# VatsalSy/gerris-fft-particles

Measured on AMD Instinct MI355X. Metric: Mcell-steps/s (projection+advection), 3D 256^3 uniform, higher is better.
Workload: dtype f64; 1 GPU; 3-D periodic Taylor-Green, 256^3 per GPU, default projection/advection parameters (SURVEY 8d config C); relax_mode=exact, parallelism=1 box, rccl_world_size=0

## Files before the change

### gerris-fft-particles_amd/csrc/domain.hip

```cpp
#include "gfship_internal.hpp"

namespace gfship {

static thread_local char g_error[1024] = "";

void set_error (const char * fmt, ...)
{
  va_list ap;
  va_start (ap, fmt);
  vsnprintf (g_error, sizeof (g_error), fmt, ap);
  va_end (ap);
}

int hip_fail (hipError_t e, const char * what, const char * file, int line)
{
  set_error ("HIP error %d (%s) in %s at %s:%d", (int) e, hipGetErrorString (e), what, file, line);
  return e == hipErrorOutOfMemory ? GFSHIP_ENOMEM : GFSHIP_EHIP;
}

Field * get_field (gfship_domain * dom, gfship_field f)
{
  if (!dom || f < 0 || (size_t) f >= dom->fields.size () || !dom->fields[f].used) {
    set_error ("invalid field handle %d", f);
    return nullptr;
  }
  return &dom->fields[f];
}

}

using namespace gfship;

extern "C" {

const char * gfship_last_error (void) { return g_error; }
int gfship_version (void) { return GFSHIP_VERSION; }

int gfship_device_count (void)
{
  int n = 0;
  if (hipGetDeviceCount (&n) != hipSuccess)
    return 0;
  return n;
}

int gfship_domain_create (gfship_domain ** out, int dim, int depth, const int side[6], int device)
{
  GFSHIP_CHECK (out != nullptr, GFSHIP_EINVAL, "null output pointer");
  *out = nullptr;
  GFSHIP_CHECK (dim == 2 || dim == 3, GFSHIP_EINVAL, "dim must be 2 or 3 (got %d)", dim);
  GFSHIP_CHECK (depth >= 0 && depth <= GFSHIP_MAXLEVEL, GFSHIP_EINVAL,
		"depth must be in [0,%d] (got %d)", GFSHIP_MAXLEVEL, depth);
  int ndev = gfship_device_count ();
  GFSHIP_CHECK (ndev > 0, GFSHIP_ENODEVICE,
		"no HIP device: libgfship has no CPU fallback");
  GFSHIP_CHECK (device >= 0 && device < ndev, GFSHIP_EINVAL, "device %d out of range (%d devices)",
		device, ndev);
  GFSHIP_HIP (hipSetDevice (device));
  gfship_domain * dom = new gfship_domain;
  dom->dim = dim;
  dom->depth = depth;
  dom->device = device;
  for (int d = 0; d < 6; d++) {
    dom->side[d] = side ? side[d] : GFSHIP_SIDE_BOUNDARY;
    if (d < 2*dim && (dom->side[d] < 0 || dom->side[d] > GFSHIP_SIDE_EXTERNAL)) {
      delete dom;
      set_error ("invalid side kind %d for direction %d", side[d], d);
      return GFSHIP_EINVAL;
    }
  }
  for (int d = 0; d < 2*dim; d += 2)
    if ((dom->side[d] == GFSHIP_SIDE_PERIODIC) != (dom->side[d + 1] == GFSHIP_SIDE_PERIODIC)) {
      delete dom;
      set_error ("periodic sides must come in pairs (directions %d,%d)", d, d + 1);
      return GFSHIP_EINVAL;
    }
  for (int d = 0; d < 2*dim; d++)
    if (dom->side[d] == GFSHIP_SIDE_EXTERNAL)
      dom->has_external = true;
  for (int l = 0; l <= depth; l++) {
    Layout & L = dom->lay[l];
    L.n = 1 << l;
    L.dim = dim;
    L.rows = L.n + 2;
    L.xo = 1;
    L.px = L.n + 4;
    L.sy = L.px;
    L.sz = dim == 3 ? (long) L.px*L.rows : 0;
    L.total = (size_t) L.px*L.rows*(dim == 3 ? L.rows : 1);
  }
  hipError_t e = hipStreamCreateWithFlags (&dom->stream, hipStreamNonBlocking);
  if (e == hipSuccess) e = hipEventCreate (&dom->ev0);
  if (e == hipSuccess) e = hipEventCreate (&dom->ev1);
  if (e == hipSuccess) e = hipStreamCreateWithFlags (&dom->side_stream, hipStreamNonBlocking);
  if (e == hipSuccess) e = hipEventCreateWithFlags (&dom->side_fork, hipEventDisableTiming);
  dom->scratch_doubles = 5*8192 + 64;
  if (e == hipSuccess) e = hipMalloc ((void **) &dom->d_scratch, dom->scratch_doubles*sizeof (double));
  if (e == hipSuccess) e = hipHostMalloc ((void **) &dom->h_pinned, 64*sizeof (double), hipHostMallocDefault);
  if (e == hipSuccess) memset (dom->h_pinned, 0, 64*sizeof (double));
  if (e != hipSuccess) {
    int r = hip_fail (e, "domain resources", __FILE__, __LINE__);
    gfship_domain_destroy (dom);
    return r;
  }
  dom->sw = read_switches ();
  *out = dom;
  return GFSHIP_OK;
}

void gfship_domain_destroy (gfship_domain * dom)
{
  if (!dom) return;
  (void) hipSetDevice (dom->device);
  if (dom->stream) (void) hipStreamSynchronize (dom->stream);
  if (dom->side_stream) (void) hipStreamSynchronize (dom->side_stream);
  for (size_t f = 0; f < dom->fields.size (); f++)
    if (dom->fields[f].used)
      gfship_field_free (dom, (gfship_field) f);
  comm_free (dom);
  mpi_order_free (dom);
  skew_free (dom);
  if (dom->d_scratch) (void) hipFree (dom->d_scratch);
  if (dom->cfl_partial) (void) hipFree (dom->cfl_partial);
  for (int d = 0; d < 6; d++) {
    if (dom->gfv_send[d]) (void) hipFree (dom->gfv_send[d]);
    if (dom->gfv_recv[d]) (void) hipFree (dom->gfv_recv[d]);
  }
  if (dom->lat_res) (void) hipFree (dom->lat_res);
  if (dom->lat_xch) (void) hipFree (dom->lat_xch);
  if (dom->lat_bar) (void) hipFree (dom->lat_bar);
  if (dom->h_pinned) (void) hipHostFree (dom->h_pinned);
  if (dom->ev0) (void) hipEventDestroy (dom->ev0);
  if (dom->ev1) (void) hipEventDestroy (dom->ev1);
  if (dom->side_fork) (void) hipEventDestroy (dom->side_fork);
  if (dom->side_stream) (void) hipStreamDestroy (dom->side_stream);
  if (dom->stream) (void) hipStreamDestroy (dom->stream);
  delete dom;
}

int gfship_domain_set_relax_mode (gfship_domain * dom, int mode)
{
  GFSHIP_CHECK (dom != nullptr, GFSHIP_EINVAL, "null domain");
  GFSHIP_CHECK (mode == GFSHIP_RELAX_EXACT || mode == GFSHIP_RELAX_REDBLACK ||
		mode == GFSHIP_RELAX_EXACT_HYPERPLANE || mode == GFSHIP_RELAX_EXACT_PER_SWEEP,
		GFSHIP_EINVAL, "unknown relax mode %d", mode);
  dom->force_hyperplane = (mode == GFSHIP_RELAX_EXACT_HYPERPLANE);
  dom->no_fused_loop = (mode == GFSHIP_RELAX_EXACT_PER_SWEEP);
  dom->no_fused_godunov = (mode == GFSHIP_RELAX_EXACT_PER_SWEEP);
  dom->relax_mode = mode == GFSHIP_RELAX_REDBLACK ? GFSHIP_RELAX_REDBLACK : GFSHIP_RELAX_EXACT;
  return GFSHIP_OK;
}

int gfship_domain_set_overlap (gfship_domain * dom, int overlap)
{
  GFSHIP_CHECK (dom != nullptr, GFSHIP_EINVAL, "null domain");
  dom->overlap = overlap != 0;
  return GFSHIP_OK;
}

int gfship_domain_set_exchange (gfship_domain * dom, gfship_exchange_fn fn, void * ctx)
{
  GFSHIP_CHECK (dom != nullptr, GFSHIP_EINVAL, "null domain");
  dom->exchange = fn;
  dom->exchange_ctx = ctx;
  return GFSHIP_OK;
}

int gfship_domain_set_reduce (gfship_domain * dom, gfship_reduce_fn fn, void * ctx)
{
  GFSHIP_CHECK (dom != nullptr, GFSHIP_EINVAL, "null domain");
  dom->reduce = fn;
  dom->reduce_ctx = ctx;
  return GFSHIP_OK;
}

int gfship_domain_set_gather (gfship_domain * dom, gfship_gather_fn fn, void * ctx, int rank,
			      int nboxes, const int lattice[3])
{
  GFSHIP_CHECK (dom && lattice, GFSHIP_EINVAL, "null argument");
  GFSHIP_CHECK (nboxes >= 1 && rank >= 0 && rank < nboxes &&
		(long) lattice[0]*lattice[1]*lattice[2] == nboxes, GFSHIP_EINVAL,
		"box %d of %d on a lattice of %d x %d x %d", rank, nboxes, lattice[0], lattice[1], lattice[2]);
  for (int d = 0; d < 2*dom->dim; d++)
    GFSHIP_CHECK (lattice[d/2] == 1 || dom->side[d] == GFSHIP_SIDE_EXTERNAL, GFSHIP_EINVAL,
		  "side %d faces another box of the lattice: it must be GFSHIP_SIDE_EXTERNAL", d);
  dom->gather = fn;
  dom->gather_ctx = ctx;
  dom->lat_rank = rank; dom->lat_n = nboxes;
  for (int c = 0; c < 3; c++) dom->lat_b[c] = lattice[c];
  return GFSHIP_OK;
}

int gfship_domain_path_counts (gfship_domain * dom, unsigned long long * lattice_cycles,
			       unsigned long long * fused_mpi_launches)
{
  GFSHIP_CHECK (dom != nullptr, GFSHIP_EINVAL, "null domain");
  if (lattice_cycles) *lattice_cycles = dom->n_lattice_cycles;
  if (fused_mpi_launches) *fused_mpi_launches = dom->n_fused_mpi;
  return GFSHIP_OK;
}

int gfship_domain_kernel_counts (gfship_domain * dom, unsigned long long * counts, int n)
{
  GFSHIP_CHECK (dom != nullptr && counts != nullptr && n >= 0, GFSHIP_EINVAL, "null argument");
  for (int k = 0; k < n && k < GFSHIP_KC_COUNT; k++)
    counts[k] = dom->kc[k];
  return GFSHIP_OK;
}

int gfship_domain_synchronize (gfship_domain * dom)
{
  GFSHIP_CHECK (dom != nullptr, GFSHIP_EINVAL, "null domain");
  GFSHIP_HIP (hipStreamSynchronize (dom->stream));
  return GFSHIP_OK;
}

void * gfship_domain_stream (gfship_domain * dom)
{
  return dom ? (void *) dom->stream : nullptr;
}

gfship_field gfship_field_alloc (gfship_domain * dom, int component)
{
  GFSHIP_CHECK (dom != nullptr, GFSHIP_EINVAL, "null domain");
  GFSHIP_CHECK (component >= -1 && component < dom->dim, GFSHIP_EINVAL,
		"component %d out of range", component);
  size_t slot = dom->fields.size ();
  for (size_t f = 0; f < dom->fields.size (); f++)
    if (!dom->fields[f].used) { slot = f; break; }
  if (slot == dom->fields.size ())
    dom->fields.emplace_back ();
  Field nf;
  nf.used = true;
  nf.component = component;
  size_t total = 0;
  for (int l = 0; l <= dom->depth; l++)
    total += (dom->lay[l].total + 31) & ~(size_t) 31;
  double * base = nullptr;
  GFSHIP_HIP (hipMalloc ((void **) &base, total*sizeof (double)));
  GFSHIP_HIP (hipMemsetAsync (base, 0, total*sizeof (double), dom->stream));
  size_t o = 0;
  for (int l = dom->depth; l >= 0; l--) {
    nf.lev[l] = base + o;
    nf.zero[l] = true;
    o += (dom->lay[l].total + 31) & ~(size_t) 31;
  }
  dom->fields[slot] = nf;
  return (gfship_field) slot;
}

int gfship_field_free (gfship_domain * dom, gfship_field f)
{
  Field * F = get_field (dom, f);
  if (!F) return GFSHIP_EINVAL;
  GFSHIP_HIP (hipStreamSynchronize (dom->stream));
  GFSHIP_HIP (hipFree (F->lev[dom->depth]));
  for (int d = 0; d < 6; d++)
    if (F->bcval[d]) GFSHIP_HIP (hipFree (F->bcval[d]));
  *F = Field ();
  return GFSHIP_OK;
}

int gfship_field_set_bc (gfship_domain * dom, gfship_field f, int d, int type, const double * val)
{
  Field * F = get_field (dom, f);
  if (!F) return GFSHIP_EINVAL;
  GFSHIP_CHECK (d >= 0 && d < 2*dom->dim, GFSHIP_EINVAL, "direction %d out of range", d);
  GFSHIP_CHECK (type >= GFSHIP_BC_SYMMETRY && type <= GFSHIP_BC_NEUMANN, GFSHIP_EINVAL,
		"unknown bc type %d", type);
  F->bc[d] = type;
  if (F->bcval[d]) {
    GFSHIP_HIP (hipStreamSynchronize (dom->stream));
    GFSHIP_HIP (hipFree (F->bcval[d]));
    F->bcval[d] = nullptr;
  }
  if (val) {
    int n = dom->lay[dom->depth].n;
    size_t m = dom->dim == 3 ? (size_t) n*n : (size_t) n;
    GFSHIP_HIP (hipMalloc ((void **) &F->bcval[d], m*sizeof (double)));
    GFSHIP_HIP (hipMemcpy (F->bcval[d], val, m*sizeof (double), hipMemcpyHostToDevice));
  }
  return GFSHIP_OK;
}

static int check_level (gfship_domain * dom, int level)
{
  GFSHIP_CHECK (level >= 0 && level <= dom->depth, GFSHIP_EINVAL, "level %d out of [0,%d]", level,
		dom->depth);
  return GFSHIP_OK;
}

}

namespace gfship {
int coarse_flush (gfship_domain * dom, Field * F, int level, bool leaf_write)
{
  if (!F->coarse_stale || (level >= dom->depth && !leaf_write)) return GFSHIP_OK;
  F->coarse_stale = false;
  Field * one[1] = { F };
  return launch_coarse_init (dom, one, 1);
}
}

extern "C" {

int gfship_field_upload (gfship_domain * dom, gfship_field f, int level, const double * host)
{
  Field * F = get_field (dom, f);
  if (!F) return GFSHIP_EINVAL;
  GFSHIP_CHECK (host != nullptr, GFSHIP_EINVAL, "null host pointer");
  int r = check_level (dom, level);
  if (r) return r;
  if ((r = before_write (dom))) return r;
  if ((r = coarse_flush (dom, F, level, true))) return r;
  const Layout & L = dom->lay[level];
  size_t rows = (size_t) L.rows*(dom->dim == 3 ? L.rows : 1);
  GFSHIP_HIP (hipMemcpy2DAsync (F->lev[level] + L.xo, L.px*sizeof (double),
				host, L.rows*sizeof (double),
				L.rows*sizeof (double), rows, hipMemcpyHostToDevice, dom->stream));
  GFSHIP_HIP (hipStreamSynchronize (dom->stream));
  F->zero[level] = false;
  if (level < dom->depth) F->coarse_valid = true;
  return GFSHIP_OK;
}

int gfship_field_download (gfship_domain * dom, gfship_field f, int level, double * host)
{
  Field * F = get_field (dom, f);
  if (!F) return GFSHIP_EINVAL;
  GFSHIP_CHECK (host != nullptr, GFSHIP_EINVAL, "null host pointer");
  int r = check_level (dom, level);
  if (r) return r;
  if ((r = coarse_flush (dom, F, level))) return r;
  const Layout & L = dom->lay[level];
  size_t rows = (size_t) L.rows*(dom->dim == 3 ? L.rows : 1);
  GFSHIP_HIP (hipMemcpy2DAsync (host, L.rows*sizeof (double),
				F->lev[level] + L.xo, L.px*sizeof (double),
				L.rows*sizeof (double), rows, hipMemcpyDeviceToHost, dom->stream));
  GFSHIP_HIP (hipStreamSynchronize (dom->stream));
  return GFSHIP_OK;
}

// ... 51 lines not shown
```

### gerris-fft-particles_amd/csrc/gfship_internal.hpp

```cpp
#pragma once

#include <hip/hip_runtime.h>
#include <cstdio>
#include <cstdarg>
#include <cstring>
#include <vector>
#include <deque>
#include <string>
#include <type_traits>
#include "gfship.h"
#include "switches.hpp"
#include "cell_update.hpp"

namespace gfship {

struct Layout {
  int n = 0;
  int px = 0;
  int xo = 1;
  int rows = 0;
  int dim = 3;
  long sy = 0;
  long sz = 0;
  size_t total = 0;
  __host__ __device__ inline long idx (int i, int j, int k) const {
    return xo + i + sy*j + sz*k;
  }
};

struct Field {
  bool used = false;
  int component = -1;
  double * lev[GFSHIP_MAXLEVEL + 1] = {};
  int bc[6] = {0, 0, 0, 0, 0, 0};
  double * bcval[6] = {};
  bool zero[GFSHIP_MAXLEVEL + 1] = {};
  bool coarse_stale = false;
  bool coarse_valid = false;
};

struct SkewPlan {
  int ntj = 0, RT = 0;
  size_t hb_words = 0;
  double * us = nullptr, * rs = nullptr, * ds = nullptr;
  double * ws[6] = {};
  unsigned long ws_stamp = 0;
  void * hb = nullptr;
  void * hbf = nullptr;
  bool rs_ready = false;
  int cur_set = 0;
  size_t armed[2] = { 0, 0 };
  unsigned * arm_cum = nullptr;
  hipEvent_t arm_ev = nullptr;
  bool arm_wait = false;
  bool loop_checked = false;
  void * stats_loop = nullptr;
  void * ctl = nullptr;
  unsigned long long * stats = nullptr;
  unsigned short * order = nullptr;
  unsigned short * xorder = nullptr;
};

struct RelaxOp {
  int kind = 0;
  double w = 1., h2 = 1.;
  const double * wf[6] = {};
};

inline W6 op_weights (const RelaxOp * op)
{
  W6 wf;
  for (int d = 0; d < 6; d++) wf.p[d] = op ? op->wf[d] : nullptr;
  return wf;
}

struct BcDesc {
  int side[6];
  int type[6];
  const double * val[6];
  int component;
  int homogeneous;
};

}

struct gfship_domain {
  int dim = 3, depth = 0, device = 0;
  int side[6] = {1, 1, 1, 1, 1, 1};
  int relax_mode = GFSHIP_RELAX_EXACT;
  gfship::Switches sw;
  gfship::Layout lay[GFSHIP_MAXLEVEL + 1];
  std::deque<gfship::Field> fields;
  hipStream_t stream = nullptr;
  hipEvent_t ev0 = nullptr, ev1 = nullptr;
  hipStream_t side_stream = nullptr;
  hipEvent_t side_fork = nullptr;
  int (* before_write) (void *) = nullptr;
  void * before_write_ctx = nullptr;
  double * d_scratch = nullptr;
  size_t scratch_doubles = 0;
  double * h_pinned = nullptr;
  gfship_exchange_fn exchange = nullptr; void * exchange_ctx = nullptr;
  gfship_reduce_fn reduce = nullptr;     void * reduce_ctx = nullptr;
  bool has_external = false;
  void * comm = nullptr;
  int overlap = 0;
  int lat_rank = -1, lat_n = 0, lat_b[3] = { 1, 1, 1 };
  gfship_gather_fn gather = nullptr; void * gather_ctx = nullptr;
  double * lat_res = nullptr, * lat_xch = nullptr;
  unsigned * lat_bar = nullptr;
  size_t lat_res_doubles = 0, lat_xch_doubles = 0;
  double * gfv_send[6] = {}, * gfv_recv[6] = {};
  double src[3] = { 0., 0., 0. };
  unsigned long long n_lattice_cycles = 0, n_fused_mpi = 0;
  unsigned long long kc[GFSHIP_KC_COUNT] = {};
  bool lattice_attr_set = false;
  void * mpi_plan[GFSHIP_MAXLEVEL + 1] = {};
  gfship_field dp_cache = -1;
  int skew_resident = -1;
  int patch_resident = 0;
  bool no_fused_godunov = false;
  bool no_fused_loop = false;
  bool force_hyperplane = false;
  bool unit_weights = false;
  bool weighted = false;
  unsigned long weights_stamp = 0;
  gfship_field wf[6] = {-1, -1, -1, -1, -1, -1};
  gfship::SkewPlan skew[GFSHIP_MAXLEVEL + 1];
  double diff_w[GFSHIP_MAXLEVEL + 1] = {};
  double * cfl_partial = nullptr;
  size_t cfl_nblocks = 0, cfl_used = 0;
  bool cfl_dirty = false;
  bool coarse_attr_set = false;
  gfship_field res_cache = -1;
  bool diff_ready = false;
  int diff_kind = 1;
  int patch_call = -1;
};

namespace gfship {

void set_error (const char * fmt, ...);
int  hip_fail (hipError_t e, const char * what, const char * file, int line);

inline int before_write (gfship_domain * dom)
{
  return dom->before_write ? dom->before_write (dom->before_write_ctx) : GFSHIP_OK;
}

#define GFSHIP_HIP(call) do { hipError_t e_ = (call); \
    if (e_ != hipSuccess) return gfship::hip_fail (e_, #call, __FILE__, __LINE__); } while (0)

inline hipError_t stream_wait_spin (hipStream_t st)
{
  hipError_t e;
  while ((e = hipStreamQuery (st)) == hipErrorNotReady)
    ;
  return e;
}

template <class F> inline void with_bools (F && f) { f (); }
template <class F, class... B> inline void with_bools (F && f, bool b0, B... rest)
{
  if (b0) with_bools ([&] (auto... r) { f (std::true_type {}, r...); }, rest...);
  else    with_bools ([&] (auto... r) { f (std::false_type {}, r...); }, rest...);
}

template <class F, class... B> inline void with_kind (F && f, int kind, B... bools)
{
  auto k = [&] (auto K) { with_bools ([&] (auto... r) { f (K, r...); }, bools...); };
  if (kind == 3)      k (std::integral_constant<int, 3> {});
  else if (kind == 2) k (std::integral_constant<int, 2> {});
  else if (kind)      k (std::integral_constant<int, 1> {});
  else                k (std::integral_constant<int, 0> {});
}

#define GFSHIP_CHECK(cond, code, ...) do { if (!(cond)) { \
    gfship::set_error (__VA_ARGS__); return (code); } } while (0)

Field * get_field (gfship_domain * dom, gfship_field f);
int coarse_flush (gfship_domain * dom, Field * F, int level, bool leaf_write = false);
inline long ncells (const Layout & L) {
  return L.dim == 3 ? (long) L.n*L.n*L.n : (long) L.n*L.n;
}

int launch_bc (gfship_domain * dom, Field * v, Field * v1, int level, int homogeneous);
bool all_sides_periodic (const gfship_domain * dom);

__device__ __forceinline__ void periodic_images (const Layout & L, double * __restrict__ a, int i, int j, int k,
						  double v)
{
  const int n = L.n;
  if (i == 1) a[L.idx (n + 1, j, k)] = v;
  if (i == n) a[L.idx (0, j, k)] = v;
  if (j == 1) a[L.idx (i, n + 1, k)] = v;
  if (j == n) a[L.idx (i, 0, k)] = v;
  if (k == 1) a[L.idx (i, j, n + 1)] = v;
  if (k == n) a[L.idx (i, j, 0)] = v;
}
int call_exchange (gfship_domain * dom, double * ptr, int level, int kind);
int bc_mpi_begin (gfship_domain * dom, Field * v1, int level);
int bc_mpi_end (gfship_domain * dom, Field * v, Field * v1, int level, int homogeneous);
int call_reduce (gfship_domain * dom, double * vals, int n, int op);
int call_reduce_norm (gfship_domain * dom, double * sums, int nsum, double * mx);
int comm_exchange (gfship_domain * dom, double * a, int level, int kind);
int comm_exchange_raw (gfship_domain * dom, double * const send[6], double * const recv[6], size_t count);
int comm_migrate (gfship_domain * dom, int rs, const int nsend[6], const double * const send[6],
		  int nrecv[6], std::vector<double> recv[6]);
int comm_allgather (gfship_domain * dom, const double * send, double * recv, size_t count);
int multi_buffers (gfship_domain * dom);
int launch_bc_multi (gfship_domain * dom, Field * const * v, int nf, int level, int homogeneous);
int call_gather (gfship_domain * dom, const double * send, double * recv, size_t count);
int comm_exchange_begin (gfship_domain * dom, double * a, int level);
int comm_exchange_end (gfship_domain * dom, double * a, int level);
int comm_reduce (gfship_domain * dom, double * sums, int nsum, double * maxs, int nmax,
		 double * mins, int nmin);
void comm_free (gfship_domain * dom);
int launch_relax_exact (gfship_domain * dom, unsigned dimension, int level, double omega,
			double * u, const double * rhs, const double * dia,
			const RelaxOp * op = nullptr);
int launch_relax_mpi_first (gfship_domain * dom, unsigned dimension, int level, double omega,
			    double * u, const double * rhs, const double * dia, const RelaxOp * op,
			    int (* after_shell) (void *), void * ctx);
void mpi_order_free (gfship_domain * dom);
int launch_relax_loop_small (gfship_domain * dom, unsigned dimension, int level, double omega,
			     Field * dp, Field * ubc, const double * rhs, const double * dia,
			     unsigned nrelax, bool * done, const RelaxOp * op = nullptr);
int coarse_cycle_top (gfship_domain * dom, int minlevel);
int lattice_cycle_top (gfship_domain * dom, int minlevel, Field * dia);
int lattice_check_error (gfship_domain * dom);
int launch_lattice_cycle (gfship_domain * dom, unsigned dimension, double omega, int lmin, int ltop,
			  const unsigned * nrelax, Field * dp, Field * ubc, Field * res);
int launch_coarse_cycle (gfship_domain * dom, unsigned dimension, double omega, int lmin, int ltop,
			 const unsigned * nrelax, Field * dp, Field * ubc, Field * res, Field * dia);
int launch_relax_redblack (gfship_domain * dom, unsigned dimension, int level, double omega,
			   double * u, const double * rhs, const double * dia);
int launch_residual (gfship_domain * dom, int level, const double * u, const double * rhs,
		     const double * dia, double * res);
int launch_residual_weighted (gfship_domain * dom, int level, const double * u, const double * rhs,
			      const double * dia, double * res);
int launch_poisson_weights (gfship_domain * dom, double * const alpha[3]);
int launch_diffusion_weights (gfship_domain * dom, double * const D[3], double cdt);
int alloc_weights (gfship_domain * dom);
RelaxOp weighted_op (gfship_domain * dom, int level);
int launch_restrict (gfship_domain * dom, unsigned dimension, int level_coarse, double * v_coarse,
		     const double * v_fine);
int launch_prolongate (gfship_domain * dom, int level_coarse, const double * v_coarse,
		       double * v_fine);
int launch_correct (gfship_domain * dom, int level, double * u, const double * dp);
int launch_fill (gfship_domain * dom, int level, double * a, double value);
int launch_residual_norm (gfship_domain * dom, int level, const double * u, const double * rhs,
			  const double * dia, double * res, double scale, double weight,
			  double * out , bool dia_zero = false);
int launch_norm_async (gfship_domain * dom, int level, const double * a, double scale, double weight);
int launch_norm (gfship_domain * dom, int level, const double * a, double scale, double weight,
		 double out[5] );

int launch_face_interp_un (gfship_domain * dom, double * const u[3], double * const un[3]);
int launch_divergence (gfship_domain * dom, double * const un[3], double * div, double dt);
int launch_correct_un (gfship_domain * dom, const double * p, double * const un[3], double dt);
int launch_centered_gradient (gfship_domain * dom, const double * p, double * const g[3]);
int launch_correct_centered (gfship_domain * dom, double * const u[3], double * const g[3], double dt);
int launch_correct_centered_coarse (gfship_domain * dom, double * const u[3], double * const g[3],
				    double dt, double * const uc[3]);
int launch_coarse_init_from (gfship_domain * dom, Field * const * v, int nf, int top);
int launch_coarse_init_levels (gfship_domain * dom, Field * const * v, int nf, int top, int bottom);
int launch_advected_face_values (gfship_domain * dom, const double * v, double * const u[3],
				 double * const un[3], double dt, int use_centered, int gradient,
				 double * const fv[6], int cmask, double visc = 0., double gsrc = 0.,
				 const double * msrc = nullptr );
int launch_variable_mac_source (gfship_domain * dom, const double * v, double * const D[3],
				const double * alpha, double * out);
int launch_mac_source_fields (gfship_domain * dom, int c, const double * F, bool add_out, double * out);
int launch_centered_source_fields (gfship_domain * dom, double * v, const double * F, double gsrc, double dt);
int launch_face_bc (gfship_domain * dom, Field * v, double * const fv[6], int cmask);
int launch_predict_un (gfship_domain * dom, int cc, const double * uc, double * const fv[6],
		       double * unc);
int launch_flux_update (gfship_domain * dom, bool velocity, double * v, double * const un[3],
			double * const fv[6], const double * gm, const double * gc, double dt,
			double gsrc = 0.);
int launch_cfl (gfship_domain * dom, double * const u[3], double * const un[3],
		const double visc[3], double * cfl2,
		double * const msrc[3] = nullptr );
int launch_coarse_init (gfship_domain * dom, Field * const * v, int nf);
int launch_velocity_divergence (gfship_domain * dom, double * const u[3], double * out);
bool godunov_fused_supported (const gfship_domain * dom);
bool godunov_fused_mpi_supported (const gfship_domain * dom);
int launch_project_correct (gfship_domain * dom, const double * p, double * const un[3],
			    double * const g[3], double * const u[3], double dt, bool want_max,
			    bool * ghosts_done = nullptr);
int launch_cfl_from_max (gfship_domain * dom, double * cfl2);
int launch_face_interp_div (gfship_domain * dom, double * const u[3], double * const un[3] ,
			    double * div, double dt);
int launch_project_correct_weighted (gfship_domain * dom, const double * p, double * const un[3],
				     double * const g[3], double * const u[3], double dt);
int launch_project_correct_lazy (gfship_domain * dom, const double * p, double * const u[3],
				 double * const g[3], double * const uo[3], double dt,
				 bool * ghosts_done = nullptr);
int launch_predict_un_fused (gfship_domain * dom, double * const u[3], double dt, int gradient,
			     const double visc[3], double * const un[3], double * div = nullptr,
			     double div_dt = 0., bool * div_done = nullptr);
int launch_advect3_fused (gfship_domain * dom, double * const v[3], double * const out[3],
			  double * const un[3], double * const gm[3], double * const gc[3],
			  double dt, int gradient, double corr_dt = 0., double * const uc[3] = nullptr);
int launch_advect_fused (gfship_domain * dom, bool velocity, const double * v, double * out,
			 double * const un[3], const double * gm, const double * gc, double dt,
			 int gradient, double visc, double gsrc = 0.);
int launch_advect_diffuse_fused (gfship_domain * dom, const double * v, double * out, double * const un[3],
				 double dt, int gradient, double D, double w, double beta);

bool skew_supported (const gfship_domain * dom, int level);
int  launch_relax_loop_skew (gfship_domain * dom, int level, Field * dp, Field * ubc,
			     const double * rhs, const double * dia, bool dia_zero,
			     unsigned nrelax, bool bc, double * correct_into = nullptr,
			     const double * prolong_from = nullptr, const RelaxOp * op = nullptr);
void skew_free (gfship_domain * dom);
bool skew_loop_supported (gfship_domain * dom, int level, unsigned nrelax, bool bc);
struct LoopGhosts;
int  skew_loop_run (gfship_domain * dom, int level, SkewPlan * S, double * u_nat, bool has_dia,
		    unsigned nrelax, float * ms = nullptr, const Field * ubc = nullptr,
		    const RelaxOp * op = nullptr, LoopGhosts * ghosts = nullptr);
int  skew_time_loop (gfship_domain * dom, int level, Field * u, const double * rhs,
		     const double * dia, bool dia_zero, unsigned nrelax, int reps,
		     double * ms_per_loop, int * fused, double * ms_inclusive = nullptr);
int  skew_check_error (gfship_domain * dom);
int  skew_arm_ahead (gfship_domain * dom, int level, unsigned nrelax);
int  patch_resident_per_cu (const gfship_domain * dom);
bool prolongation_fused (gfship_domain * dom, unsigned dimension, int level, unsigned nrelax);
bool prolongation_fusable (gfship_domain * dom, unsigned dimension, int level, unsigned nrelax);
bool line_prolongation_fused (gfship_domain * dom, unsigned dimension, int level, unsigned nrelax);
bool line_prolongation_fusable (gfship_domain * dom, unsigned dimension, int level, unsigned nrelax);
inline bool patch_level (const gfship_domain * dom, int level)
{
  const bool per_cell_weights = dom->patch_call < 0 ? dom->weighted : dom->patch_call == 0;
  return dom->sw.patch () && !per_cell_weights && dom->lay[level].n >= dom->sw.patch_min_n;
}
int  patch_pack (gfship_domain * dom, int level, SkewPlan * S, const double * u, const double * rhs,
		 const double * dia, const double * coarse = nullptr);
int  patch_unpack (gfship_domain * dom, int level, SkewPlan * S, double * u, double * add_into,
		   const LoopGhosts * ghosts = nullptr);
int  patch_restrict_pack (gfship_domain * dom, int level, SkewPlan * S, const double * res,
			  double * res_coarse, SkewPlan * Sc, unsigned dimension);
int  launch_restrict_pack (gfship_domain * dom, unsigned dimension, int level, Field * res,
			   bool coarse_fused);
void skew_dump_stats (gfship_domain * dom, int level);
int  skew_time_sweeps (gfship_domain * dom, int level, Field * u, const double * rhs,
		       const double * dia, bool dia_zero, int reps, double * ms_per_sweep);

}
```

### gerris-fft-particles_amd/csrc/poisson.hip

```cpp
#include "gfship_internal.hpp"
#include <cmath>
#include <cfloat>
#include <cstdlib>

using namespace gfship;

#define GFSHIP_CHECK_DIMENSION(dom, d) \
  GFSHIP_CHECK ((d) == (unsigned) (dom)->dim, GFSHIP_EUNSUPPORTED, \
		"dimension %u on a %d-D domain: only the dimension of the domain is implemented", (d), (dom)->dim)

namespace gfship {

static bool weighted_pipelinable (gfship_domain * dom, unsigned dimension, int level)
{
  return dom->relax_mode == GFSHIP_RELAX_EXACT && dimension == 3 && dom->dim == 3 &&
    skew_supported (dom, level) && !dom->force_hyperplane;
}

static bool weighted_pipelined (gfship_domain * dom, unsigned dimension, int level)
{
  return dom->sw.weighted_pipelined && weighted_pipelinable (dom, dimension, level);
}

static int relax_level (gfship_domain * dom, unsigned dimension, int level, double omega,
// ... 137 lines not shown
  int r;
  double w = (double) ncells (L);
  if (dom->has_external) {
    double sums[5] = { s[0], s[1], s[2], w, s[4] }, mx[1] = { s[3] };
    if ((r = call_reduce_norm (dom, sums, 5, mx))) return r;
    s[0] = sums[0]; s[1] = sums[1]; s[2] = sums[2]; w = sums[3]; s[3] = mx[0]; s[4] = sums[4];
  }
  gfship_norm n;
  n.bias = s[0]; n.first = s[1]; n.second = s[2]; n.infty = s[3]; n.w = w;
  if (n.w > 0.) {
    n.bias /= n.w;
    n.first /= n.w;
    n.second = sqrt (n.second/n.w);
  }
  else
    n.infty = 0.;
  dt *= dt;
  n.bias = s[4]*dt;
  n.first *= dt;
  n.second *= dt;
  n.infty *= dt;
  *out = n;
  return GFSHIP_OK;
}

}

extern "C" {

void gfship_multilevel_params_init (gfship_multilevel_params * par, int dim)
{
  memset (par, 0, sizeof (*par));
  par->tolerance = 1e-3;
  par->nrelax    = 4;
  par->erelax    = 1;
  par->minlevel  = 0;
  par->nitermax  = 100;
  par->nitermin  = 1;
  par->dimension = dim;
  par->weighted  = 0;
  par->beta      = 1.;
  par->omega     = 1.;
  par->function  = 0;
}

int gfship_poisson_coefficients_alpha (gfship_domain * dom, const gfship_field alpha[3])
{
  GFSHIP_CHECK (dom != nullptr, GFSHIP_EINVAL, "null domain");
  if (!alpha)
    return gfship_poisson_coefficients (dom);
  double * a[3] = { nullptr, nullptr, nullptr };
  for (int c = 0; c < dom->dim; c++) {
    Field * F = get_field (dom, alpha[c]);
    if (!F) return GFSHIP_EINVAL;
    a[c] = F->lev[dom->depth];
  }
  int r = alloc_weights (dom);
  if (r) return r;
  if ((r = launch_poisson_weights (dom, a))) return r;
  dom->weighted = true;
  dom->weights_stamp++;
  dom->unit_weights = true;
  return GFSHIP_OK;
}

int gfship_poisson_weights (gfship_domain * dom, int d, gfship_field * w)
{
  GFSHIP_CHECK (dom && w, GFSHIP_EINVAL, "null argument");
  GFSHIP_CHECK (d >= 0 && d < 2*dom->dim, GFSHIP_EINVAL, "direction %d out of range", d);
  GFSHIP_CHECK (dom->wf[d] >= 0 && (dom->weighted || (dom->diff_ready && dom->diff_kind == 3)), GFSHIP_EINVAL,
		"call gfship_poisson_coefficients_alpha or gfship_diffusion_coefficients_faces first");
  *w = dom->wf[d];
  return GFSHIP_OK;
}

int gfship_poisson_coefficients (gfship_domain * dom)
{
  GFSHIP_CHECK (dom != nullptr, GFSHIP_EINVAL, "null domain");
  dom->weighted = false;
  dom->unit_weights = true;
  return GFSHIP_OK;
}

int gfship_relax (gfship_domain * dom, unsigned d, int level, double omega,
		  gfship_field u, gfship_field rhs, gfship_field dia)
{
  Field * U = get_field (dom, u), * R = get_field (dom, rhs), * D = get_field (dom, dia);
  if (!U || !R || !D) return GFSHIP_EINVAL;
  GFSHIP_CHECK (level >= 0 && level <= dom->depth, GFSHIP_EINVAL, "level %d out of range", level);
  GFSHIP_CHECK (d == 2 || d == 3, GFSHIP_EINVAL, "dimension must be 2 or 3");
  GFSHIP_CHECK_DIMENSION (dom, d);
  GFSHIP_CHECK (dom->unit_weights, GFSHIP_EINVAL, "call gfship_poisson_coefficients first");
  { int r = before_write (dom); if (r) return r; }
  for (Field * F : { U, R, D })
    if (int r = coarse_flush (dom, F, level)) return r;
  return relax_level (dom, d, level, omega, U, R, D);
}

int gfship_residual (gfship_domain * dom, unsigned d, int level,
		     gfship_field u, gfship_field rhs, gfship_field dia, gfship_field res)
{
  Field * U = get_field (dom, u), * R = get_field (dom, rhs), * D = get_field (dom, dia),
    * S = get_field (dom, res);
  if (!U || !R || !D || !S) return GFSHIP_EINVAL;
  GFSHIP_CHECK (level >= 0 && level <= dom->depth, GFSHIP_EINVAL, "level %d out of range", level);
  GFSHIP_CHECK (d == 2 || d == 3, GFSHIP_EINVAL, "dimension must be 2 or 3");
  GFSHIP_CHECK_DIMENSION (dom, d);
  GFSHIP_CHECK (dom->unit_weights, GFSHIP_EINVAL, "call gfship_poisson_coefficients first");
  { int r = before_write (dom); if (r) return r; }
  for (Field * F : { U, R, D, S })
    if (int r = coarse_flush (dom, F, level)) return r;
  S->zero[level] = false;
  if (dom->weighted)
    return launch_residual_weighted (dom, level, U->lev[level], R->lev[level], D->lev[level],
				     S->lev[level]);
  return launch_residual (dom, level, U->lev[level], R->lev[level], D->lev[level], S->lev[level]);
}

int gfship_norm_residual (gfship_domain * dom, double dt, gfship_field res, gfship_norm * out)
{
  Field * S = get_field (dom, res);
  if (!S || !out) return GFSHIP_EINVAL;
  return norm_residual (dom, dt, S, out);
}

int gfship_norm_variable (gfship_domain * dom, gfship_field v, gfship_norm * out)
{
  Field * V = get_field (dom, v);
  if (!V || !out) return GFSHIP_EINVAL;
  const Layout & L = dom->lay[dom->depth];
  double size = 1./L.n;
  double vol = dom->dim == 3 ? size*size*size : size*size;
  double s[5];
  int r = launch_norm (dom, dom->depth, V->lev[dom->depth], 1., vol, s);
  if (r) return r;
  gfship_norm n;
  double wv = vol*(double) ncells (L);
  if (dom->has_external) {
    double sums[4] = { s[0], s[1], s[2], wv }, mx[1] = { s[3] };
    if ((r = call_reduce_norm (dom, sums, 4, mx))) return r;
    s[0] = sums[0]; s[1] = sums[1]; s[2] = sums[2]; wv = sums[3]; s[3] = mx[0];
  }
  n.bias = s[0]; n.first = s[1]; n.second = s[2]; n.infty = s[3];
  n.w = wv;
  if (n.w > 0.) {
    n.bias /= n.w;
    n.first /= n.w;
    n.second = sqrt (n.second/n.w);
  }
  else
    n.infty = 0.;
  *out = n;
  return GFSHIP_OK;
}

}

static int poisson_cycle (gfship_domain * dom, gfship_multilevel_params * p,
			  gfship_field u, gfship_field rhs, gfship_field dia, gfship_field res,
			  double dt, gfship_norm * norm)
{
  GFSHIP_CHECK (dom && p, GFSHIP_EINVAL, "null argument");
  GFSHIP_CHECK (p->dimension == 2 || p->dimension == 3, GFSHIP_EINVAL, "dimension must be 2 or 3");
  GFSHIP_CHECK_DIMENSION (dom, p->dimension);
  GFSHIP_CHECK (p->nrelax > 0 && p->erelax > 0, GFSHIP_EINVAL, "nrelax and erelax must be non zero");
  GFSHIP_CHECK (dom->unit_weights, GFSHIP_EINVAL, "call gfship_poisson_coefficients first");
  if (dom->dp_cache < 0)
    dom->dp_cache = gfship_field_alloc (dom, -1);
  gfship_field dpf = dom->dp_cache;
  if (dpf < 0) return dpf;
  Field * U = get_field (dom, u), * R = get_field (dom, rhs), * D = get_field (dom, dia),
    * S = get_field (dom, res), * DP = get_field (dom, dpf);
  int r = GFSHIP_OK;
  bool corrected = false;
  if (!U || !R || !D || !S) return GFSHIP_EINVAL;
  const int L = dom->depth;
  unsigned minlevel = p->minlevel;
  if (minlevel > (unsigned) L) minlevel = L;
  p->depth = L;

#define TRY(x) do { if ((r = (x)) != GFSHIP_OK) goto done; } while (0)
  for (int l = 0; l <= L; l++)
    S->zero[l] = U->zero[l] = false;
  {
    unsigned nrl[GFSHIP_MAXLEVEL + 1];
    {
      unsigned nr = p->nrelax;
      for (int l = L; l >= 0; l--) {
	nrl[l] = nr;
	if (l > (int) minlevel) nr *= p->erelax;
      }
    }
    for (int l = 0; l <= L; l++)
      DP->zero[l] = false;
    const int ctop = dom->weighted ? -1 : coarse_cycle_top (dom, (int) minlevel);
    const int ltop = ctop >= 0 ? -1 : lattice_cycle_top (dom, (int) minlevel, D);
    for (int l = L - 1; l >= (ctop >= 0 ? ctop + 1 : ltop >= 0 ? ltop : 0); l--) {
      if (dom->relax_mode == GFSHIP_RELAX_EXACT && p->dimension == 3 && !dom->weighted &&
	  !dom->force_hyperplane && skew_supported (dom, l + 1))
	TRY (skew_arm_ahead (dom, l + 1, nrl[l + 1]));
      const bool rp = !dom->skew[l + 1].rs_ready && prolongation_fused (dom, p->dimension, l + 1, nrl[l + 1]);
      if (rp) dom->kc[dom->sw.fused_restriction ? GFSHIP_KC_RESTRICTION_FUSED : GFSHIP_KC_RESTRICTION_DECLINED]++;
      if (dom->sw.fused_restriction && rp)
	TRY (launch_restrict_pack (dom, p->dimension, l + 1, S,
				   l > (int) minlevel && prolongation_fused (dom, p->dimension, l, nrl[l])));
      else
	TRY (launch_restrict (dom, p->dimension, l, S->lev[l], S->lev[l + 1]));
    }
    unsigned first = minlevel;
    if (ltop >= 0) {
      TRY (launch_lattice_cycle (dom, p->dimension, p->omega, (int) minlevel, ltop, nrl, DP, U, S));
      first = ltop + 1;
    }
    else if (ctop >= 0) {
      TRY (launch_coarse_cycle (dom, p->dimension, p->omega, (int) minlevel, ctop, nrl, DP, U, S, D));
      first = ctop + 1;
    }
    else {
      TRY (launch_fill (dom, minlevel, DP->lev[minlevel], 0.));
      TRY (relax_loop (dom, DP, U, p->dimension, minlevel, p->omega, S, D, nrl[minlevel]));
      first = minlevel + 1;
      dom->kc[GFSHIP_KC_COARSE_END_BY_LEVEL]++;
    }
    for (unsigned l = first; l <= p->depth; l++) {
      const bool fp = prolongation_fused (dom, p->dimension, (int) l, nrl[l]) ||
	line_prolongation_fused (dom, p->dimension, (int) l, nrl[l]);
      if (fp) dom->kc[GFSHIP_KC_PROLONGATION_FUSED]++;
      else if (prolongation_fusable (dom, p->dimension, (int) l, nrl[l]) ||
	       line_prolongation_fusable (dom, p->dimension, (int) l, nrl[l]))
	dom->kc[GFSHIP_KC_PROLONGATION_DECLINED]++;
      if (!fp)
	TRY (launch_prolongate (dom, l - 1, DP->lev[l - 1], DP->lev[l]));
      TRY (relax_loop (dom, DP, U, p->dimension, l, p->omega, S, D, nrl[l],
		       (int) l == L ? U->lev[L] : nullptr, &corrected, fp ? DP->lev[l - 1] : nullptr));
    }
  }
  if (!corrected)
    TRY (launch_correct (dom, L, U->lev[L], DP->lev[L]));
  if (!(corrected && all_sides_periodic (dom)))
    TRY (launch_bc (dom, U, U, L, 0));
  if (norm)
    TRY (residual_and_norm (dom, dt, U, R, D, S, norm));
  else if (dom->weighted)
    TRY (launch_residual_weighted (dom, L, U->lev[L], R->lev[L], D->lev[L], S->lev[L]));
  else
    TRY (launch_residual (dom, L, U->lev[L], R->lev[L], D->lev[L], S->lev[L]));
#undef TRY
 done:
  for (int l = 0; l <= L; l++)
    dom->skew[l].rs_ready = false;
  return r;
}

extern "C" {

int gfship_poisson_cycle (gfship_domain * dom, gfship_multilevel_params * p,
			  gfship_field u, gfship_field rhs, gfship_field dia, gfship_field res)
{
  GFSHIP_CHECK (dom != nullptr, GFSHIP_EINVAL, "null domain");
  int r = before_write (dom);
  if (r) return r;
  return poisson_cycle (dom, p, u, rhs, dia, res, 1., nullptr);
}

int gfship_poisson_solve (gfship_domain * dom, gfship_multilevel_params * par,
			  gfship_field lhs, gfship_field rhs, gfship_field res,
			  gfship_field dia, double dt)
{
  GFSHIP_CHECK (dom && par, GFSHIP_EINVAL, "null argument");
  Field * U = get_field (dom, lhs), * R = get_field (dom, rhs), * D = get_field (dom, dia),
    * S = get_field (dom, res);
  if (!U || !R || !D || !S) return GFSHIP_EINVAL;
  GFSHIP_CHECK (par->dimension == 2 || par->dimension == 3, GFSHIP_EINVAL, "dimension must be 2 or 3");
  GFSHIP_CHECK_DIMENSION (dom, par->dimension);
  GFSHIP_CHECK (dom->unit_weights, GFSHIP_EINVAL, "call gfship_poisson_coefficients first");
  { int r = before_write (dom); if (r) return r; }
  int r;
  const int L = dom->depth;
  if ((r = coarse_flush (dom, U, L, true))) return r;
  unsigned minlevel = par->minlevel;
  par->depth = L;
  par->niter = 0;

  bool deferred = par->nitermin >= 1 && par->nitermax >= 1;
  if (deferred) {
    const Layout & Ly = dom->lay[L];
    double size = 1./Ly.n;
    S->zero[L] = false;
    if (dom->weighted) {
      if ((r = launch_residual_weighted (dom, L, U->lev[L], R->lev[L], D->lev[L], S->lev[L]))) return r;
      if ((r = launch_norm_async (dom, L, S->lev[L], 1.*size*size, 1.))) return r;
    }
    else if ((r = launch_residual_norm (dom, L, U->lev[L], R->lev[L], D->lev[L], S->lev[L], 1.*size*size,
					1., nullptr, D->zero[L])))
      return r;
  }
  else {
    if ((r = residual_and_norm (dom, dt, U, R, D, S, &par->residual))) return r;
    par->residual_before = par->residual;
  }

  double res_max_before = par->residual.infty;

  while (par->niter < par->nitermin ||
	 (par->residual.infty > par->tolerance && par->niter < par->nitermax)) {
    if ((r = poisson_cycle (dom, par, lhs, rhs, dia, res, dt, &par->residual))) {
      if (deferred) {
	deferred = false;
	double s0[5];
	if (hipStreamSynchronize (dom->stream) == hipSuccess) {
	  memcpy (s0, dom->h_pinned + 8, sizeof (s0));
	  if (norm_residual_finish (dom, dt, s0, &par->residual_before) == GFSHIP_OK)
	    par->residual = par->residual_before;
	}
	else
	  memset (&par->residual_before, 0, sizeof (par->residual_before)),
	    memset (&par->residual, 0, sizeof (par->residual));
      }
      break;
    }
    if (deferred) {
      deferred = false;
      double s0[5];
      memcpy (s0, dom->h_pinned + 8, sizeof (s0));
      if ((r = norm_residual_finish (dom, dt, s0, &par->residual_before))) break;
      res_max_before = par->residual_before.infty;
    }
    if (par->residual.infty == res_max_before)
      break;
    if (par->residual.infty > res_max_before/1.1 && par->minlevel < par->depth)
      par->minlevel++;
    res_max_before = par->residual.infty;
    par->niter++;
  }

  par->minlevel = minlevel;
  if (r == GFSHIP_OK)
    r = skew_check_error (dom);
  if (r == GFSHIP_OK)
    r = lattice_check_error (dom);
  return r;
}

int gfship_time_relax (gfship_domain * dom, unsigned d, int level, gfship_field u,
		       gfship_field rhs, gfship_field dia, int reps, double * ms_per_sweep)
{
  Field * U = get_field (dom, u), * R = get_field (dom, rhs), * D = get_field (dom, dia);
  if (!U || !R || !D || !ms_per_sweep || reps <= 0) return GFSHIP_EINVAL;
  GFSHIP_CHECK (level >= 0 && level <= dom->depth, GFSHIP_EINVAL, "level %d out of range", level);
  int r;
  if (dom->relax_mode == GFSHIP_RELAX_EXACT && d == 3 && skew_supported (dom, level) &&
      !dom->force_hyperplane) {
    U->zero[level] = false;
    r = skew_time_sweeps (dom, level, U, R->lev[level], D->lev[level], D->zero[level], reps,
			  ms_per_sweep);
    if (r == GFSHIP_OK && dom->sw.skew_stats)
      skew_dump_stats (dom, level);
    return r;
  }
  if ((r = relax_level (dom, d, level, 1., U, R, D))) return r;
  GFSHIP_HIP (hipEventRecord (dom->ev0, dom->stream));
  for (int q = 0; q < reps; q++)
    if ((r = relax_level (dom, d, level, 1., U, R, D))) return r;
  GFSHIP_HIP (hipEventRecord (dom->ev1, dom->stream));
  GFSHIP_HIP (hipEventSynchronize (dom->ev1));
  float ms = 0.f;
  GFSHIP_HIP (hipEventElapsedTime (&ms, dom->ev0, dom->ev1));
  *ms_per_sweep = (double) ms/reps;
  if (dom->sw.skew_stats)
    skew_dump_stats (dom, level);
  return GFSHIP_OK;
}

int gfship_time_relax_loop (gfship_domain * dom, int level, gfship_field u, gfship_field rhs,
			    gfship_field dia, unsigned nrelax, int reps, double * ms_per_loop,
			    int * fused)
{
  return gfship_time_relax_loop_inclusive (dom, level, u, rhs, dia, nrelax, reps, ms_per_loop, fused,
					   nullptr);
}

int gfship_time_relax_loop_inclusive (gfship_domain * dom, int level, gfship_field u, gfship_field rhs,
				      gfship_field dia, unsigned nrelax, int reps,
				      double * ms_per_loop, int * fused, double * ms_inclusive)
{
  Field * U = get_field (dom, u), * R = get_field (dom, rhs), * D = get_field (dom, dia);
  if (!U || !R || !D || !ms_per_loop || !fused || reps <= 0 || nrelax == 0) return GFSHIP_EINVAL;
  GFSHIP_CHECK (level >= 0 && level <= dom->depth, GFSHIP_EINVAL, "level %d out of range", level);
  GFSHIP_CHECK (dom->relax_mode == GFSHIP_RELAX_EXACT && skew_supported (dom, level) &&
		!dom->force_hyperplane, GFSHIP_EUNSUPPORTED,
		"the pipelined sweep does not run on this level / in this mode");
  U->zero[level] = false;
  int r = skew_time_loop (dom, level, U, R->lev[level], D->lev[level], D->zero[level], nrelax,
			  reps, ms_per_loop, fused, ms_inclusive);
  if (r == GFSHIP_OK)
    r = skew_check_error (dom);
  return r;
}

}
```

### gerris-fft-particles_amd/csrc/relax_patch_loop.hip

```cpp
#include "relax_skew.hpp"
#include <cstdlib>
#include <vector>

#ifndef PK_D
#define PK_D 9
#endif
#ifndef PK_DH
#define PK_DH 3
#endif
#ifndef PK_KO
#define PK_KO 0
#endif
#define PK_NTHREADS 192
#define PK_SKEW 14

namespace gfship {

typedef double d2 __attribute__((ext_vector_type(2)));

__device__ __forceinline__ void patch_arm_other_set (const SkewLoopArgs & A, int tile, int tid, int nt)
{
  if (A.arm_pairs == 0) return;
  typedef unsigned long long ull2 __attribute__((ext_vector_type(2)));
  const unsigned long long W = A.arm_cum[A.ntj*A.ntj];
// ... 843 lines not shown
  __shared__ double cbuf[10][10][PR_W];
  const int Ilo = R0 - PK_SKEW > 0 ? R0 - PK_SKEW : 0;
  const int cx0 = Ilo >> 1;
  {
    const int jb = n/2 - 8*P - 8, kb = n/2 - 8*Q - 8;
    const int xmax = A.Lc.n + 1;
    for (int e = threadIdx.x; e < 100*PR_W; e += 64*PR_WAVES) {
      const int line = e / PR_W, ix = e % PR_W;
      const int jl = line % 10, kl = line / 10;
      int cx = cx0 + ix;
      if (cx > xmax) cx = xmax;
      cbuf[kl][jl][ix] = vc[A.Lc.idx (cx, jb + jl, kb + kl)];
    }
  }
  __syncthreads ();
  const double * const cl = &cbuf[8 - PB][8 - PA][0] - cx0;
  constexpr int lsy = PR_W, lsz = 10*PR_W;
#endif
  if (r0 >= n + PK_SKEW) return;
  const int j0 = n - (SK_T*P + 2*PA), k0 = n - (SK_T*Q + 2*PB);
  const bool side_j[2] = { j0 == n, j0 - 1 == 1 }, side_k[2] = { k0 == n, k0 - 1 == 1 };
  int cur_m = -1;
  double pv = 0., qx = 0., qy = 0., qz = 0.;
  const int r1 = r0 + PR_ROWS;
  for (int rho = r0; rho < r1; rho++) {
    const int I = rho - s;
    if ((unsigned) I >= (unsigned) n) continue;
    const int m = I >> 1;
    if (m != cur_m) {
      cur_m = m;
#if PR_LDS
      const double * const q = cl + (m + 1);
      pv = q[0];
      {
	const double g1 = q[1] - 1.*pv, g2 = q[-1] - 1.*pv;
	qx = 0.25*((g1 - g2)/2.);
      }
      {
	const double g1 = q[lsy] - 1.*pv, g2 = q[-lsy] - 1.*pv;
	qy = 0.25*((g1 - g2)/2.);
      }
      {
	const double g1 = q[lsz] - 1.*pv, g2 = q[-lsz] - 1.*pv;
	qz = 0.25*((g1 - g2)/2.);
      }
#else
      const long p = cline + (m + 1);
      pv = vc[p];
      {
	const double g1 = vc[p + 1] - 1.*pv, g2 = vc[p - 1] - 1.*pv;
	qx = 0.25*((g1 - g2)/2.);
      }
      {
	const double g1 = vc[p + csy] - 1.*pv, g2 = vc[p - csy] - 1.*pv;
	qy = 0.25*((g1 - g2)/2.);
      }
      {
	const double g1 = vc[p + csz] - 1.*pv, g2 = vc[p - csz] - 1.*pv;
	qz = 0.25*((g1 - g2)/2.);
      }
#endif
    }
    const double bx = pv + ((I & 1) ? qx : - qx);
    d2 o01, o23;
    {
      const double by0 = bx + qy, by1 = bx + (- qy);
      o01.x = by0 + qz;     o01.y = by1 + qz;
      o23.x = by0 + (- qz); o23.y = by1 + (- qz);
    }
    double * const row = dst + (long) rho*SK_NL;
    *(d2 *) row = o01;
    *(d2 *) (row + 128) = o23;
    if (__builtin_expect (I == 0 || I == n - 1 || side_j[0] || side_j[1] || side_k[0] || side_k[1], 0)) {
      const bool ends = I == 0 || I == n - 1;
      const double vv[4] = { o01.x, o01.y, o23.x, o23.y };
#pragma unroll
      for (int q = 0; q < 4; q++)
	if (ends || side_j[q & 1] || side_k[q >> 1]) {
	  A.nat[A.L.idx (I + 1, j0 - (q & 1), k0 - (q >> 1))] = vv[q];
	  if (A.periodic) periodic_images (A.L, A.nat, I + 1, j0 - (q & 1), k0 - (q >> 1), vv[q]);
	}
    }
  }
}

#ifndef PP_ROWS
#define PP_ROWS 16
#endif
#define PP_SPAN (PP_ROWS + 7)
#ifndef PPR_ROWS
#define PPR_ROWS 64
#endif
#define PPR_SPAN (PPR_ROWS + 7)
#ifndef PPU_ROWS
#define PPU_ROWS 64
#endif
#define PPU_SPAN (PPU_ROWS + 7)

__global__ void __launch_bounds__(256)
patch_pack_kernel (PatchPackArgs A)
{
  __shared__ double buf[3][32][PP_SPAN + 1];
  const int tid = threadIdx.x;
  const int tile = blockIdx.z, PB = blockIdx.y, r0 = blockIdx.x*PP_ROWS;
  const int P = tile % A.ntj, Q = tile / A.ntj;
  const int n = A.L.n;
  const long tbase = (long) tile*(A.RT + 2*SK_FP)*SK_NL + SK_FP*SK_NL;
  const int I0 = r0 - 7 - PB;
  for (int e = tid; e < 32*PP_SPAN; e += 256) {
    const int line = e / PP_SPAN, di = e % PP_SPAN;
    const int a = line & 15, db = line >> 4;
    const int I = I0 + di;
    if (I >= 0 && I < n) {
      const int j = n - (SK_T*P + a), k = n - (SK_T*Q + 2*PB + db);
      const long nidx = A.L.idx (I + 1, j, k);
      int q0 = 0;
      if (A.coarse) {
	const double v = patch_prolong (A.Lc, A.coarse, I + 1, j, k);
	buf[0][line][di] = v;
	if (I == 0 || I == n - 1 || j == 1 || j == n || k == 1 || k == n)
	  A.nat[nidx] = v;
	q0 = 1;
      }
      for (int q = q0; q < A.narr; q++)
	buf[q][line][di] = A.src[q][nidx];
    }
  }
  __syncthreads ();
  for (int e = tid; e < PP_ROWS*32; e += 256) {
    const int row = e / 32, col = e % 32;
    const int PA = col >> 2, p = col & 3;
    const int a = 2*PA + (p & 1), db = p >> 1;
    const int rho = r0 + row;
    const int I = rho - PA - PB;
    if (I >= 0 && I < n) {
      const long sidx = tbase + (long) rho*SK_NL + 128*(p >> 1) + 2*(PA + 8*PB) + (p & 1);
      for (int q = 0; q < A.narr; q++)
	A.dst[q][sidx] = buf[q][a + 16*db][I - I0];
    }
  }
}

struct PatchRestrictArgs {
  Layout L, Lc;
  int ntj, RT;
  const double * src;
  double * dst;
  double * cnat;
  double * cskew;
  int cntj, cRT;
  unsigned dimension;
};

__global__ void __launch_bounds__(256)
patch_restrict_pack_kernel (PatchRestrictArgs A)
{
  __shared__ double buf[32][PPR_SPAN + 2];
  const int tid = threadIdx.x;
  const int tile = blockIdx.z, PB = blockIdx.y, r0 = blockIdx.x*PPR_ROWS;
  const int P = tile % A.ntj, Q = tile / A.ntj;
  const int n = A.L.n;
  const long tbase = (long) tile*(A.RT + 2*SK_FP)*SK_NL + SK_FP*SK_NL;
  const int I0 = r0 - 7 - PB;
  for (int e = tid; e < 32*(PPR_SPAN + 1); e += 256) {
    const int line = e / (PPR_SPAN + 1), di = e % (PPR_SPAN + 1);
    const int a = line & 15, db = line >> 4;
    const int I = I0 + di;
    if (I >= 0 && I < n) {
      const int j = n - (SK_T*P + a), k = n - (SK_T*Q + 2*PB + db);
      buf[line][di] = A.src[A.L.idx (I + 1, j, k)];
    }
  }
  __syncthreads ();
  for (int e = tid; e < PPR_ROWS*32; e += 256) {
    const int row = e / 32, col = e % 32;
    const int PA = col >> 2, p = col & 3;
    const int a = 2*PA + (p & 1), db = p >> 1;
    const int rho = r0 + row;
    const int I = rho - PA - PB;
    if (I >= 0 && I < n)
      A.dst[tbase + (long) rho*SK_NL + 128*(p >> 1) + 2*(PA + 8*PB) + (p & 1)] = buf[a + 16*db][I - I0];
  }
  for (int e = tid; e < 8*(PPR_ROWS/2); e += 256) {
    const int PA = e / (PPR_ROWS/2), mi = e % (PPR_ROWS/2);
    const int par = (PA + PB + r0) & 1;
    const int row = 2*mi + par;
    const int I = r0 + row - PA - PB;
    if (I >= 0 && I < n) {
      const int di = I - I0;
      double val = 0.;
#pragma unroll
      for (int id = 0; id < 8; id++)
	val += buf[2*PA + ((id >> 1) & 1) + 16*(id >> 2)][di + (id & 1)];
      const double v = A.dimension == 2 ? val : val/2.;
      const int m = I >> 1;
      const int pj = (n - SK_T*P - 2*PA) >> 1, pk = (n - SK_T*Q - 2*PB) >> 1;
      A.cnat[A.Lc.idx (m + 1, pj, pk)] = v;
      if (A.cskew) {
	const int ca = 8*(P & 1) + PA, cb = 8*(Q & 1) + PB;
	const long ctile = (P >> 1) + (long) A.cntj*(Q >> 1);
	A.cskew[ctile*(A.cRT + 2*SK_FP)*SK_NL + SK_FP*SK_NL +
		(long) (m + (ca >> 1) + (cb >> 1))*SK_NL + 128*(cb & 1) + 2*((ca >> 1) + 8*(cb >> 1)) + (ca & 1)] = v;
      }
    }
  }
}

__global__ void __launch_bounds__(256)
patch_unpack_kernel (PatchPackArgs A, LoopGhosts G)
{
  if ((int) blockIdx.z >= A.ntj*A.ntj) {
    loop_ghost_blocks (G, A.ntj*A.ntj);
    return;
  }
  __shared__ double buf[32][PPU_SPAN + 1];
  const int tid = threadIdx.x;
  const int tile = blockIdx.z, PB = blockIdx.y, r0 = blockIdx.x*PPU_ROWS;
  const int P = tile % A.ntj, Q = tile / A.ntj;
  const int n = A.L.n;
  const long tbase = (long) tile*(A.RT + 2*SK_FP)*SK_NL + SK_FP*SK_NL;
  const int I0 = r0 - 7 - PB;
  for (int e = tid; e < PPU_ROWS*32; e += 256) {
    const int row = e / 32, col = e % 32;
    const int PA = col >> 2, p = col & 3;
    const int a = 2*PA + (p & 1), db = p >> 1;
    const int rho = r0 + row;
    const int I = rho - PA - PB;
    if (I >= 0 && I < n)
      buf[a + 16*db][I - I0] = A.src[0][tbase + (long) rho*SK_NL + 128*(p >> 1) + 2*(PA + 8*PB) + (p & 1)];
  }
  __syncthreads ();
  for (int e = tid; e < 32*PPU_SPAN; e += 256) {
    const int line = e / PPU_SPAN, di = e % PPU_SPAN;
    const int a = line & 15, db = line >> 4;
    const int I = I0 + di;
    const int rho = I + (a >> 1) + PB;
    if (I >= 0 && I < n && rho >= r0 && rho < r0 + PPU_ROWS) {
      const int j = n - (SK_T*P + a), k = n - (SK_T*Q + 2*PB + db);
      const long c = A.L.idx (I + 1, j, k);
      if (A.add) {
	const double v = A.add[c] + buf[line][di];
	A.add[c] = v;
	if (A.periodic && (I == 0 || I == n - 1 || j == 1 || j == n || k == 1 || k == n))
	  periodic_images (A.L, A.add, I + 1, j, k, v);
      }
      else
	A.dst[0][c] = buf[line][di];
    }
  }
}

int patch_resident_per_cu (const gfship_domain * dom)
{
  int per_cu = 0;
  hipError_t e = dom->sw.patch_regs ?
    hipOccupancyMaxActiveBlocksPerMultiprocessor (&per_cu, relax_patch_loop_kernel<true>, PK_NTHREADS, 0) :
    hipOccupancyMaxActiveBlocksPerMultiprocessor (&per_cu, relax_ring_loop_kernel<true, 0>, RK_NTHREADS, 0);
  int per_cu1 = 0;
  if (e == hipSuccess)
    e = hipOccupancyMaxActiveBlocksPerMultiprocessor (&per_cu1, relax_ring_loop_kernel<true, 1>, RK_NTHREADS, 0);
  if (per_cu1 < per_cu) per_cu = per_cu1;
  return e == hipSuccess ? per_cu : 0;
}

int patch_pack (gfship_domain * dom, int level, SkewPlan * S, const double * u, const double * rhs,
		const double * dia, const double * coarse)
{
  PatchPackArgs A;
  A.add = nullptr;
  A.coarse = coarse;
  A.periodic = all_sides_periodic (dom);
  A.nat = const_cast<double *> (u);
  A.Lc = dom->lay[level > 0 ? level - 1 : 0];
  A.L = dom->lay[level]; A.ntj = S->ntj; A.RT = S->RT;
  A.narr = 0;
  A.src[A.narr] = u;   A.dst[A.narr++] = S->us;
  if (rhs) { A.src[A.narr] = rhs; A.dst[A.narr++] = S->rs; }
  if (dia) { A.src[A.narr] = dia; A.dst[A.narr++] = S->ds; }
  const int rows = A.L.n + PK_SKEW + 1;
  const bool old_pack = coarse && dom->sw.old_prolong_pack;
  if (coarse) dom->kc[old_pack ? GFSHIP_KC_PROLONG_PACK_OLD : GFSHIP_KC_PROLONG_PACK_NEW]++;
  if (coarse && !old_pack) {
    PatchPackArgs Pr = A;
    Pr.narr = 1;
    dim3 pgrid ((rows + PR_ROWS*PR_WAVES - 1)/(PR_ROWS*PR_WAVES), S->ntj*S->ntj);
    hipLaunchKernelGGL (patch_prolong_kernel, pgrid, dim3 (64*PR_WAVES), 0, dom->stream, Pr);
    GFSHIP_HIP (hipGetLastError ());
    if (A.narr == 1)
      return GFSHIP_OK;
    for (int q = 1; q < A.narr; q++) { A.src[q - 1] = A.src[q]; A.dst[q - 1] = A.dst[q]; }
    A.narr--;
    A.coarse = nullptr;
  }
  dim3 grid ((rows + PP_ROWS - 1)/PP_ROWS, 8, S->ntj*S->ntj);
  hipLaunchKernelGGL (patch_pack_kernel, grid, dim3 (256), 0, dom->stream, A);
  GFSHIP_HIP (hipGetLastError ());
  return GFSHIP_OK;
}

int patch_restrict_pack (gfship_domain * dom, int level, SkewPlan * S, const double * res,
			 double * res_coarse, SkewPlan * Sc, unsigned dimension)
{
  PatchRestrictArgs A;
  A.L = dom->lay[level]; A.Lc = dom->lay[level - 1];
  A.ntj = S->ntj; A.RT = S->RT;
  A.src = res; A.dst = S->rs;
  A.cnat = res_coarse;
  A.cskew = Sc ? Sc->rs : nullptr;
  A.cntj = Sc ? Sc->ntj : 0; A.cRT = Sc ? Sc->RT : 0;
  A.dimension = dimension;
  const int rows = A.L.n + PK_SKEW + 1;
  dim3 grid ((rows + PPR_ROWS - 1)/PPR_ROWS, 8, S->ntj*S->ntj);
  hipLaunchKernelGGL (patch_restrict_pack_kernel, grid, dim3 (256), 0, dom->stream, A);
  GFSHIP_HIP (hipGetLastError ());
  return GFSHIP_OK;
}

int patch_unpack (gfship_domain * dom, int level, SkewPlan * S, double * u, double * add_into,
		  const LoopGhosts * ghosts)
{
  PatchPackArgs A;
  A.coarse = nullptr; A.nat = nullptr; A.Lc = dom->lay[level];
  A.periodic = all_sides_periodic (dom);
  A.L = dom->lay[level]; A.ntj = S->ntj; A.RT = S->RT;
  A.narr = 1;
  A.src[0] = S->us; A.dst[0] = u; A.add = add_into;
  const int rows = A.L.n + PK_SKEW + 1;
  dim3 grid ((rows + PPU_ROWS - 1)/PPU_ROWS, 8, S->ntj*S->ntj);
  const LoopGhosts G = ghosts ? *ghosts : LoopGhosts ();
  grid.z += loop_ghost_planes (G, grid.x, grid.y);
  hipLaunchKernelGGL (patch_unpack_kernel, grid, dim3 (256), 0, dom->stream, A, G);
  GFSHIP_HIP (hipGetLastError ());
  return GFSHIP_OK;
}

int patch_loop_launch (gfship_domain * dom, const SkewLoopArgs & A, int ntiles, bool has_dia,
		       unsigned nrelax, float * ms, LoopGhosts * ghosts)
{
  if (ms) GFSHIP_HIP (hipEventRecord (dom->ev0, dom->stream));
  if (A.op == 1)
    hipLaunchKernelGGL ((relax_ring_loop_kernel<true, 1>), dim3 (ntiles), dim3 (RK_NTHREADS), 0, dom->stream, A);
  else if (dom->sw.patch_regs) {
    if (has_dia)
      hipLaunchKernelGGL (relax_patch_loop_kernel<true>, dim3 (ntiles), dim3 (PK_NTHREADS), 0, dom->stream, A);
    else
      hipLaunchKernelGGL (relax_patch_loop_kernel<false>, dim3 (ntiles), dim3 (PK_NTHREADS), 0, dom->stream, A);
  }
  else if (has_dia)
    hipLaunchKernelGGL ((relax_ring_loop_kernel<true, 0>), dim3 (ntiles), dim3 (RK_NTHREADS), 0, dom->stream, A);
  else
    hipLaunchKernelGGL ((relax_ring_loop_kernel<false, 0>), dim3 (ntiles), dim3 (RK_NTHREADS), 0, dom->stream, A);
  GFSHIP_HIP (hipGetLastError ());
  if (ms) {
    GFSHIP_HIP (hipEventRecord (dom->ev1, dom->stream));
    GFSHIP_HIP (hipEventSynchronize (dom->ev1));
    GFSHIP_HIP (hipEventElapsedTime (ms, dom->ev0, dom->ev1));
  }
  if (nrelax >= 2 && ghosts)
    *ghosts = loop_ghosts_of (A, true);
  else if (nrelax >= 2) {
    const Layout & L = A.L;
    int block = L.n >= 256 ? 256 : L.n >= 128 ? 128 : 64;
    hipLaunchKernelGGL (patch_loop_ghosts_kernel, dim3 ((L.n + block - 1)/block, L.n, 4), dim3 (block),
			0, dom->stream, A);
    GFSHIP_HIP (hipGetLastError ());
  }
  return GFSHIP_OK;
}

}
```

### gerris-fft-particles_amd/csrc/relax_skew.hip

```cpp
#include "relax_skew.hpp"
#include <cstdlib>

namespace gfship {

template <bool HAS_DIA>
__global__ void __launch_bounds__(SK_NL)
relax_skew_kernel (SkewArgs A)
{
  constexpr int XS = SK_T + 1;
  __shared__ double X[2][XS*XS];
  __shared__ double Y[2][XS*XS];
  __shared__ unsigned s_tile;

  const int tid = threadIdx.x;
  const int a = tid & (SK_T - 1), b = tid >> 4;
  const int n = A.L.n;
  const int ntj = A.ntj;
  const long tstride = (long) (A.RT + 2*SK_FP)*SK_NL;
  const long hstride = (long) SK_HROWS (n)*SK_T;

  if (tid == 0)
    s_tile = A.order[atomicAdd (A.ticket, 1u)];
  __syncthreads ();
  const int tile = s_tile;
// ... 200 lines not shown
    const int di = m - lo;
    if (m <= 2*SK_T - 2 && di >= 0 && di < SK_T) {
      long sidx = tbase + (long) (I0 + m + b)*SK_NL + lo + SK_T*b;
      for (int q = 0; q < A.narr; q++)
	A.dst[q][sidx] = tile_[q][lo][di];
    }
  }
}

__global__ void __launch_bounds__(SK_NL)
skew_prolong_pack_kernel (PackArgs A)
{
  __shared__ double tile_[3][SK_T][SK_T + 1];
  const int tid = threadIdx.x;
  const int lo = tid & (SK_T - 1), hi = tid >> 4;
  const int tile = blockIdx.z;
  const int b = blockIdx.y;
  const int I0 = blockIdx.x*SK_T;
  const int P = tile % A.ntj, Q = tile / A.ntj;
  const int n = A.L.n;
  const int k = n - (SK_T*Q + b);
  const long tbase = (long) tile*(A.RT + 2*SK_FP)*SK_NL + SK_FP*SK_NL;
  {
    const int i = I0 + lo + 1, j = n - (SK_T*P + hi);
    const long nidx = A.L.idx (i, j, k);
    const double v = patch_prolong (A.Lc, A.coarse, i, j, k);
    tile_[0][hi][lo] = v;
    if (i == 1 || i == n || j == 1 || j == n || k == 1 || k == n) {
      A.nat[nidx] = v;
      periodic_images (A.L, A.nat, i, j, k, v);
    }
    for (int q = 1; q < A.narr; q++)
      tile_[q][hi][lo] = A.src[q][nidx];
  }
  __syncthreads ();
#pragma unroll
  for (int pass = 0; pass < 2; pass++) {
    const int m = hi + SK_T*pass;
    const int di = m - lo;
    if (m <= 2*SK_T - 2 && di >= 0 && di < SK_T) {
      long sidx = tbase + (long) (I0 + m + b)*SK_NL + lo + SK_T*b;
      for (int q = 0; q < A.narr; q++)
	A.dst[q][sidx] = tile_[q][lo][di];
    }
  }
}

__global__ void __launch_bounds__(SK_NL)
skew_unpack_kernel (PackArgs A, LoopGhosts G)
{
  if ((int) blockIdx.z >= A.ntj*A.ntj) {
    loop_ghost_blocks (G, A.ntj*A.ntj);
    return;
  }
  __shared__ double tile_[SK_T][SK_T + 1];
  const int tid = threadIdx.x;
  const int lo = tid & (SK_T - 1), hi = tid >> 4;
  const int tile = blockIdx.z;
  const int b = blockIdx.y;
  const int I0 = blockIdx.x*SK_T;
  const int P = tile % A.ntj, Q = tile / A.ntj;
  const int n = A.L.n;
  const int k = n - (SK_T*Q + b);
  const long tbase = (long) tile*(A.RT + 2*SK_FP)*SK_NL + SK_FP*SK_NL;
#pragma unroll
  for (int pass = 0; pass < 2; pass++) {
    const int m = hi + SK_T*pass;
    const int di = m - lo;
    if (m <= 2*SK_T - 2 && di >= 0 && di < SK_T)
      tile_[lo][di] = A.src[0][tbase + (long) (I0 + m + b)*SK_NL + lo + SK_T*b];
  }
  __syncthreads ();
  const int j = n - (SK_T*P + hi);
  const long c = A.L.idx (I0 + lo + 1, j, k);
  if (A.add) {
    const double v = A.add[c] + tile_[hi][lo];
    A.add[c] = v;
    if (A.periodic) periodic_images (A.L, A.add, I0 + lo + 1, j, k, v);
  }
  else
    A.dst[0][c] = tile_[hi][lo];
}

bool skew_supported (const gfship_domain * dom, int level)
{
  if (dom->dim != 3) return false;
  int n = dom->lay[level].n;
  if (n < 2*SK_T) return false;
  return true;
}

static unsigned * skew_err_word (gfship_domain * dom, int level)
{
  return (unsigned *) (dom->h_pinned + 32) + level;
}

static int skew_plan (gfship_domain * dom, int level, SkewPlan ** out)
{
  SkewPlan & S = dom->skew[level];
  if (!S.us) {
    const Layout & L = dom->lay[level];
    S.ntj = L.n/SK_T;
    S.RT = L.n + SK_PAD;
    int ntiles = S.ntj*S.ntj;
    size_t doubles = (size_t) ntiles*(S.RT + 2*SK_FP)*SK_NL + 64;
    S.hb_words = (size_t) ntiles*SK_HROWS (L.n)*SK_T;
    GFSHIP_HIP (hipMalloc ((void **) &S.us, doubles*sizeof (double)));
    GFSHIP_HIP (hipMalloc ((void **) &S.rs, doubles*sizeof (double)));
    GFSHIP_HIP (hipMalloc ((void **) &S.ds, doubles*sizeof (double)));
    GFSHIP_HIP (hipMalloc ((void **) &S.hb, 2*S.hb_words*sizeof (u64)));
    GFSHIP_HIP (hipMalloc ((void **) &S.ctl, 64));
    if (dom->sw.skew_stats)
      GFSHIP_HIP (hipMalloc ((void **) &S.stats, (size_t) ntiles*4*sizeof (u64)));
    std::vector<unsigned short> order;
    for (int d = 0; d <= 2*(S.ntj - 1); d++)
      for (int Q = 0; Q < S.ntj; Q++) {
	int P = d - Q;
	if (P >= 0 && P < S.ntj)
	  order.push_back ((unsigned short) (P + S.ntj*Q));
      }
    GFSHIP_HIP (hipMalloc ((void **) &S.order, order.size ()*sizeof (unsigned short)));
    GFSHIP_HIP (hipMemcpy (S.order, order.data (), order.size ()*sizeof (unsigned short),
			   hipMemcpyHostToDevice));
    if (ntiles >= 8 && S.ntj % 4 == 0) {
      int bw = S.ntj/2, bh = S.ntj/4;
      std::vector<unsigned short> xo;
      for (int x = 0; x < 8; x++)
	for (unsigned short t : order) {
	  int P = t % S.ntj, Q = t / S.ntj;
	  if ((P/bw) + 2*(Q/bh) == x) xo.push_back (t);
	}
      GFSHIP_HIP (hipMalloc ((void **) &S.xorder, xo.size ()*sizeof (unsigned short)));
      GFSHIP_HIP (hipMemcpy (S.xorder, xo.data (), xo.size ()*sizeof (unsigned short),
			     hipMemcpyHostToDevice));
    }
    GFSHIP_HIP (hipMemsetAsync (S.ctl, 0, 64, dom->stream));
  }
  *out = &S;
  return GFSHIP_OK;
}

void skew_free (gfship_domain * dom)
{
  for (int l = 0; l <= GFSHIP_MAXLEVEL; l++) {
    SkewPlan & S = dom->skew[l];
    if (S.us) (void) hipFree (S.us);
    if (S.rs) (void) hipFree (S.rs);
    if (S.ds) (void) hipFree (S.ds);
    for (int d = 0; d < 6; d++) if (S.ws[d]) (void) hipFree (S.ws[d]);
    if (S.hb) (void) hipFree (S.hb);
    if (S.hbf) (void) hipFree (S.hbf);
    if (S.arm_cum) (void) hipFree (S.arm_cum);
    if (S.arm_ev) (void) hipEventDestroy (S.arm_ev);
    if (S.stats_loop) (void) hipFree (S.stats_loop);
    if (S.ctl) (void) hipFree (S.ctl);
    if (S.stats) (void) hipFree (S.stats);
    if (S.order) (void) hipFree (S.order);
    if (S.xorder) (void) hipFree (S.xorder);
    S = SkewPlan ();
  }
}

static int skew_pack (gfship_domain * dom, int level, SkewPlan * S, const double * u,
		      const double * rhs, const double * dia, const double * coarse = nullptr)
{
  if (patch_level (dom, level))
    return patch_pack (dom, level, S, u, rhs, dia, coarse);
  PackArgs A;
  A.add = nullptr; A.periodic = false;
  A.coarse = coarse; A.nat = const_cast<double *> (u);
  A.Lc = dom->lay[level > 0 ? level - 1 : 0];
  A.L = dom->lay[level]; A.ntj = S->ntj; A.RT = S->RT;
  A.narr = 0;
  A.src[A.narr] = u;   A.dst[A.narr++] = S->us;
  A.src[A.narr] = rhs; A.dst[A.narr++] = S->rs;
  if (dia) { A.src[A.narr] = dia; A.dst[A.narr++] = S->ds; }
  dim3 grid (A.L.n/SK_T, SK_T, S->ntj*S->ntj);
  if (coarse)
    hipLaunchKernelGGL (skew_prolong_pack_kernel, grid, dim3 (SK_NL), 0, dom->stream, A);
  else
    hipLaunchKernelGGL (skew_pack_kernel, grid, dim3 (SK_NL), 0, dom->stream, A);
  GFSHIP_HIP (hipGetLastError ());
  return GFSHIP_OK;
}

static int skew_pack_weights (gfship_domain * dom, int level, SkewPlan * S, const RelaxOp * op)
{
  if (S->ws[0] && S->ws_stamp == dom->weights_stamp)
    return GFSHIP_OK;
  const size_t doubles = (size_t) S->ntj*S->ntj*(S->RT + 2*SK_FP)*SK_NL + 64;
  for (int d = 0; d < 6; d++)
    if (!S->ws[d]) {
      GFSHIP_HIP (hipMalloc ((void **) &S->ws[d], doubles*sizeof (double)));
      GFSHIP_HIP (hipMemsetAsync (S->ws[d], 0, doubles*sizeof (double), dom->stream));
    }
  for (int h = 0; h < 2; h++) {
    PackArgs A;
    A.add = nullptr; A.periodic = false;
    A.coarse = nullptr; A.nat = nullptr; A.Lc = dom->lay[level];
    A.L = dom->lay[level]; A.ntj = S->ntj; A.RT = S->RT;
    A.narr = 3;
    for (int q = 0; q < 3; q++) { A.src[q] = op->wf[3*h + q]; A.dst[q] = S->ws[3*h + q]; }
    dim3 grid (A.L.n/SK_T, SK_T, S->ntj*S->ntj);
    hipLaunchKernelGGL (skew_pack_kernel, grid, dim3 (SK_NL), 0, dom->stream, A);
    GFSHIP_HIP (hipGetLastError ());
  }
  S->ws_stamp = dom->weights_stamp;
  return GFSHIP_OK;
}

static int skew_unpack (gfship_domain * dom, int level, SkewPlan * S, double * u,
			double * add_into = nullptr, const LoopGhosts * ghosts = nullptr)
{
  if (patch_level (dom, level))
    return patch_unpack (dom, level, S, u, add_into, ghosts);
  PackArgs A;
  A.L = dom->lay[level]; A.ntj = S->ntj; A.RT = S->RT;
  A.narr = 1;
  A.src[0] = S->us; A.dst[0] = u; A.add = add_into;
  A.coarse = nullptr; A.nat = nullptr; A.Lc = dom->lay[level];
  A.periodic = all_sides_periodic (dom);
  dim3 grid (A.L.n/SK_T, SK_T, S->ntj*S->ntj);
  const LoopGhosts G = ghosts ? *ghosts : LoopGhosts ();
  grid.z += loop_ghost_planes (G, grid.x, grid.y);
  hipLaunchKernelGGL (skew_unpack_kernel, grid, dim3 (SK_NL), 0, dom->stream, A, G);
  GFSHIP_HIP (hipGetLastError ());
  return GFSHIP_OK;
}

static int skew_launch (gfship_domain * dom, int level, SkewPlan * S, double * u_nat, bool has_dia)
{
  SkewArgs A;
  A.L = dom->lay[level]; A.ntj = S->ntj; A.RT = S->RT;
  A.us = S->us; A.rs = S->rs; A.ds = has_dia ? S->ds : nullptr;
  A.un = u_nat;
  A.hbJ = (u64 *) S->hb; A.hbK = (u64 *) S->hb + S->hb_words;
  A.order = S->order;
  A.ticket = (unsigned *) S->ctl;
  A.err = skew_err_word (dom, level);
  A.dummy = (const u64 *) S->ctl + 2;
  A.stats = S->stats;
  int ntiles = S->ntj*S->ntj;
  if (has_dia)
    hipLaunchKernelGGL (relax_skew_kernel<true>, dim3 (ntiles), dim3 (SK_NL), 0, dom->stream, A);
  else
    hipLaunchKernelGGL (relax_skew_kernel<false>, dim3 (ntiles), dim3 (SK_NL), 0, dom->stream, A);
  GFSHIP_HIP (hipGetLastError ());
  return GFSHIP_OK;
}

static int skew_sweep (gfship_domain * dom, int level, SkewPlan * S, double * u_nat, bool has_dia,
		       const RelaxOp * op = nullptr)
{
  if (!dom->sw.skew_old || (op && op->kind))
    return skew_loop_run (dom, level, S, u_nat, has_dia, 1, nullptr, nullptr, op);
  GFSHIP_HIP (hipMemsetAsync (S->ctl, 0, sizeof (unsigned), dom->stream));
  if (S->ntj > 1)
    GFSHIP_HIP (hipMemsetAsync (S->hb, 0xFF, 2*S->hb_words*sizeof (u64), dom->stream));
  return skew_launch (dom, level, S, u_nat, has_dia);
}

static int skew_loop_trial (gfship_domain * dom, int level, SkewPlan * S, unsigned nrelax, bool bc)
{
  int r;
  if (!dom->no_fused_loop && !S->loop_checked && skew_loop_supported (dom, level, nrelax, bc)) {
    S->loop_checked = true;
    const Layout & L = dom->lay[level];
    size_t doubles = (size_t) S->ntj*S->ntj*(S->RT + 2*SK_FP)*SK_NL;
    double * zero_nat = nullptr;
    GFSHIP_HIP (hipMalloc ((void **) &zero_nat, L.total*sizeof (double)));
    GFSHIP_HIP (hipMemsetAsync (zero_nat, 0, L.total*sizeof (double), dom->stream));
    GFSHIP_HIP (hipMemsetAsync (S->us, 0, doubles*sizeof (double), dom->stream));
    GFSHIP_HIP (hipMemsetAsync (S->rs, 0, doubles*sizeof (double), dom->stream));
    r = skew_loop_run (dom, level, S, zero_nat, false, 2);
    if (r == GFSHIP_OK)
      GFSHIP_HIP (hipStreamSynchronize (dom->stream));
    (void) hipFree (zero_nat);
    if (r != GFSHIP_OK) return r;
    if (*skew_err_word (dom, level)) {
      dom->no_fused_loop = true;
      *skew_err_word (dom, level) = 0;
    }
  }
  return GFSHIP_OK;
}

bool prolongation_fused (gfship_domain * dom, unsigned dimension, int level, unsigned nrelax)
{
  return dom->sw.fused_prolongation && prolongation_fusable (dom, dimension, level, nrelax);
}

bool prolongation_fusable (gfship_domain * dom, unsigned dimension, int level, unsigned nrelax)
{
  if (dom->weighted || level < 1) return false;
  if (dom->relax_mode != GFSHIP_RELAX_EXACT || dimension != 3 || dom->force_hyperplane) return false;
  if (dom->has_external && dom->overlap && nrelax > 1) return false;
  return skew_supported (dom, level) && patch_level (dom, level);
}

bool line_prolongation_fusable (gfship_domain * dom, unsigned dimension, int level, unsigned nrelax)
{
  (void) nrelax;
  if (dom->weighted || level < 1) return false;
  if (dom->relax_mode != GFSHIP_RELAX_EXACT || dimension != 3 || dom->force_hyperplane) return false;
  return all_sides_periodic (dom) && skew_supported (dom, level) && !patch_level (dom, level);
}

bool line_prolongation_fused (gfship_domain * dom, unsigned dimension, int level, unsigned nrelax)
{
  return dom->sw.fused_prolongation && line_prolongation_fusable (dom, dimension, level, nrelax);
}

static bool prolong_images (gfship_domain * dom, int level)
{
  return all_sides_periodic (dom) && (!patch_level (dom, level) || !dom->sw.old_prolong_pack);
}

int launch_relax_loop_skew (gfship_domain * dom, int level, Field * dp, Field * ubc,
			    const double * rhs, const double * dia, bool dia_zero,
			    unsigned nrelax, bool bc, double * correct_into, const double * prolong_from,
			    const RelaxOp * op)
{
  SkewPlan * S;
  int r;
  if ((r = skew_plan (dom, level, &S))) return r;
  double * u = dp->lev[level];
  if ((r = skew_loop_trial (dom, level, S, nrelax, bc))) return r;
  if (op && op->kind >= 2) {
    if ((r = skew_pack_weights (dom, level, S, op))) return r;
    dia_zero = false;
  }
  const bool fusedp = prolong_from != nullptr && bc && (patch_level (dom, level) || all_sides_periodic (dom));
  const double * rhs_pack = S->rs_ready && patch_level (dom, level) ? nullptr : rhs;
  S->rs_ready = false;
  if (prolong_from && !fusedp)
    if ((r = launch_prolongate (dom, level - 1, prolong_from, u))) return r;
  if (fusedp && (r = skew_pack (dom, level, S, u, rhs_pack, dia_zero ? nullptr : dia, prolong_from))) return r;
  if (bc &&!(fusedp && prolong_images (dom, level)) && (r = launch_bc (dom, ubc, dp, level, 1))) return r;
  if (!fusedp && (r = skew_pack (dom, level, S, u, rhs_pack, dia_zero ? nullptr : dia))) return r;
  if (!dom->no_fused_loop && skew_loop_supported (dom, level, nrelax, bc)) {
    LoopGhosts G;
    const bool defer = all_sides_periodic (dom) && !op;
    if ((r = skew_loop_run (dom, level, S, u, !dia_zero, nrelax, nullptr, ubc, op, defer ? &G : nullptr))) return r;
    if (correct_into) G.active = false;
    return skew_unpack (dom, level, S, u, correct_into, &G);
  }
  for (unsigned q = 0; q < nrelax; q++) {
    if ((r = skew_sweep (dom, level, S, u, !dia_zero, op))) return r;
    if (bc && q + 1 < nrelax && (r = launch_bc (dom, ubc, dp, level, 1))) return r;
  }
  return skew_unpack (dom, level, S, u, correct_into);
}

int launch_restrict_pack (gfship_domain * dom, unsigned dimension, int level, Field * res, bool coarse_fused)
{
  SkewPlan * S, * Sc = nullptr;
  int r;
  if ((r = skew_plan (dom, level, &S))) return r;
  if ((r = skew_loop_trial (dom, level, S, 4, true))) return r;
  if (coarse_fused) {
    if ((r = skew_plan (dom, level - 1, &Sc))) return r;
    if ((r = skew_loop_trial (dom, level - 1, Sc, 4, true))) return r;
  }
  res->zero[level - 1] = false;
  if ((r = patch_restrict_pack (dom, level, S, res->lev[level], res->lev[level - 1], Sc, dimension))) return r;
  S->rs_ready = true;
  if (Sc) Sc->rs_ready = true;
  return GFSHIP_OK;
}

void skew_dump_stats (gfship_domain * dom, int level)
{
  SkewPlan & S = dom->skew[level];
  if (!S.stats) return;
  (void) hipStreamSynchronize (dom->stream);
  int nt = S.ntj*S.ntj;
  std::vector<u64> h (4*nt);
  (void) hipMemcpy (h.data (), S.stats, h.size ()*sizeof (u64), hipMemcpyDeviceToHost);
  u64 t0 = ~0ull;
  for (int q = 0; q < nt; q++) if (h[4*q] < t0) t0 = h[4*q];
  for (int Q = 0; Q < S.ntj; Q++)
    for (int P = 0; P < S.ntj; P++) {
      int q = P + S.ntj*Q;
      if (P == Q || P == 0 || Q == 0 || P == S.ntj - 1)
	fprintf (stderr, "tile (%2d,%2d) start %8.2f us  dur %8.2f us  spins %6llu slow %5llu\n", P, Q,
		 (h[4*q] - t0)/100., (h[4*q + 1] - h[4*q])/100., h[4*q + 2], h[4*q + 3]);
    }
}

int skew_time_sweeps (gfship_domain * dom, int level, Field * u, const double * rhs,
		      const double * dia, bool dia_zero, int reps, double * ms_per_sweep)
{
  SkewPlan * S;
  int r;
  if ((r = skew_plan (dom, level, &S))) return r;
  if ((r = skew_pack (dom, level, S, u->lev[level], rhs, dia_zero ? nullptr : dia))) return r;
  if ((r = skew_sweep (dom, level, S, u->lev[level], !dia_zero))) return r;
  float total = 0.f;
  for (int q = 0; q < reps; q++) {
    float ms = 0.f;
    if (!dom->sw.skew_old) {
      if ((r = skew_loop_run (dom, level, S, u->lev[level], !dia_zero, 1, &ms))) return r;
    }
    else {
      GFSHIP_HIP (hipMemsetAsync (S->ctl, 0, sizeof (unsigned), dom->stream));
      if (S->ntj > 1)
	GFSHIP_HIP (hipMemsetAsync (S->hb, 0xFF, 2*S->hb_words*sizeof (u64), dom->stream));
      GFSHIP_HIP (hipEventRecord (dom->ev0, dom->stream));
      if ((r = skew_launch (dom, level, S, u->lev[level], !dia_zero))) return r;
      GFSHIP_HIP (hipEventRecord (dom->ev1, dom->stream));
      GFSHIP_HIP (hipEventSynchronize (dom->ev1));
      GFSHIP_HIP (hipEventElapsedTime (&ms, dom->ev0, dom->ev1));
    }
    total += ms;
  }
  *ms_per_sweep = total/reps;
  return skew_unpack (dom, level, S, u->lev[level]);
}

int skew_time_loop (gfship_domain * dom, int level, Field * u, const double * rhs,
		    const double * dia, bool dia_zero, unsigned nrelax, int reps,
		    double * ms_per_loop, int * fused, double * ms_inclusive)
{
  SkewPlan * S;
  int r;
  if ((r = skew_plan (dom, level, &S))) return r;
  double * un = u->lev[level];
  bool fuse = !dom->no_fused_loop && skew_loop_supported (dom, level, nrelax, true);
  *fused = fuse;
  double total = 0., total_incl = 0.;
  hipEvent_t e0 = nullptr, e1 = nullptr;
  double * target = nullptr;
  const bool vcycle_like = ms_inclusive && fuse && level >= 1 && patch_level (dom, level);
  if (ms_inclusive) {
    GFSHIP_HIP (hipEventCreate (&e0));
    GFSHIP_HIP (hipEventCreate (&e1));
  }
  if (vcycle_like) {
    GFSHIP_HIP (hipMalloc ((void **) &target, dom->lay[level].total*sizeof (double)));
    GFSHIP_HIP (hipMemsetAsync (target, 0, dom->lay[level].total*sizeof (double), dom->stream));
    if ((r = skew_pack (dom, level, S, un, rhs, dia_zero ? nullptr : dia))) return r;
  }
  for (int q = -1; q < reps; q++) {
    float ms = 0.f;
    if (vcycle_like) {
      if (S->hbf) {
        if ((r = skew_arm_ahead (dom, level, nrelax))) return r;
        GFSHIP_HIP (hipStreamSynchronize (dom->side_stream));
      }
      GFSHIP_HIP (hipEventRecord (e0, dom->stream));
      if ((r = skew_pack (dom, level, S, un, nullptr, nullptr, u->lev[level - 1]))) return r;
      if ((r = launch_bc (dom, u, u, level, 1))) return r;
      if ((r = skew_loop_run (dom, level, S, un, !dia_zero, nrelax, &ms, u))) return r;
      if ((r = skew_unpack (dom, level, S, un, target))) return r;
    }
    else {
      if (e0) GFSHIP_HIP (hipEventRecord (e0, dom->stream));
      if ((r = launch_bc (dom, u, u, level, 1))) return r;
      if ((r = skew_pack (dom, level, S, un, rhs, dia_zero ? nullptr : dia))) return r;
      if (fuse) {
	if ((r = skew_loop_run (dom, level, S, un, !dia_zero, nrelax, &ms, u))) return r;
      }
      else
	for (unsigned w = 0; w < nrelax; w++) {
	  float m1 = 0.f;
	  if (!dom->sw.skew_old) {
	    if ((r = skew_loop_run (dom, level, S, un, !dia_zero, 1, &m1))) return r;
	  }
	  else {
	    GFSHIP_HIP (hipMemsetAsync (S->ctl, 0, sizeof (unsigned), dom->stream));
	    if (S->ntj > 1)
	      GFSHIP_HIP (hipMemsetAsync (S->hb, 0xFF, 2*S->hb_words*sizeof (u64), dom->stream));
	    GFSHIP_HIP (hipEventRecord (dom->ev0, dom->stream));
	    if ((r = skew_launch (dom, level, S, un, !dia_zero))) return r;
	    GFSHIP_HIP (hipEventRecord (dom->ev1, dom->stream));
	    GFSHIP_HIP (hipEventSynchronize (dom->ev1));
	    GFSHIP_HIP (hipEventElapsedTime (&m1, dom->ev0, dom->ev1));
	  }
	  ms += m1;
	  if (w + 1 < nrelax && (r = launch_bc (dom, u, u, level, 1))) return r;
	}
      if ((r = skew_unpack (dom, level, S, un))) return r;
    }
    if (e0) {
      float mi = 0.f;
      GFSHIP_HIP (hipEventRecord (e1, dom->stream));
      GFSHIP_HIP (hipEventSynchronize (e1));
      GFSHIP_HIP (hipEventElapsedTime (&mi, e0, e1));
      if (q >= 0) total_incl += mi;
    }
    if (q >= 0) total += ms;
  }
  *ms_per_loop = total/reps;
  if (ms_inclusive) {
    *ms_inclusive = total_incl/reps;
    (void) hipEventDestroy (e0);
    (void) hipEventDestroy (e1);
  }
  if (target) {
    GFSHIP_HIP (hipStreamSynchronize (dom->stream));
    (void) hipFree (target);
  }
  return GFSHIP_OK;
}

int skew_check_error (gfship_domain * dom)
{
  for (int l = 0; l <= dom->depth; l++)
    if (dom->skew[l].ctl && *skew_err_word (dom, l) != 0) {
      *skew_err_word (dom, l) = 0;
      dom->skew[l].armed[0] = dom->skew[l].armed[1] = 0;
      dom->no_fused_loop = true;
      set_error ("relax_skew_kernel: a hand-off wait timed out on level %d (CUs held by another "
		 "process or stream?); this solve failed, the domain falls back to one launch "
		 "per sweep", l);
      return GFSHIP_EHIP;
    }
  return GFSHIP_OK;
}

// ... 2 lines not shown
```

### gerris-fft-particles_amd/csrc/simulation.hip

```cpp
#include "gfship_internal.hpp"
#include <cmath>
#include <cfloat>
#include <cstdlib>

using namespace gfship;

#define G_MAXINT 2147483647

struct gfship_sim {
  gfship_domain * dom = nullptr;
  gfship_field p = -1, pmac = -1, u[3] = {-1, -1, -1}, g[3] = {-1, -1, -1}, gmac[3] = {-1, -1, -1};
  std::vector<gfship_field> tracers;
  std::vector<int> tracer_gradient;
  std::vector<int> tracer_scheme;
  std::vector<double> tracer_D;
  std::deque<gfship_multilevel_params> tracer_diffusion_params;
  bool tracer_diffusion_fused = true;
  unsigned long long tracer_diffusion_counts[2] = { 0, 0 };
  gfship_field un[3] = {-1, -1, -1};
  gfship_field fv[6] = {-1, -1, -1, -1, -1, -1};
  gfship_field dia = -1, div = -1, res = -1, tmp = -1;
  gfship_multilevel_params projection_params, approx_projection_params;
  gfship_advection_params advection_params;
  double t = 0., end = DBL_MAX, dtmax = DBL_MAX, tnext = 0.;
// ... 800 lines not shown
      TRY (variable_sources (s, t, s->drhs, gradient, false, dt, nullptr, nullptr, D));
    TRY (gfship_diffusion_rhs (dom, t, s->drhs, s->rhoc, par->beta));
    s->tracer_diffusion_counts[1]++;
  }
  TRY (gfship_diffusion (dom, par, t, s->drhs, s->rhoc));
  return GFSHIP_OK;
}

int gfship_sim_set_tracer_diffusion (gfship_sim * s, int t, double D)
{
  GFSHIP_CHECK (s != nullptr, GFSHIP_EINVAL, "null simulation");
  GFSHIP_CHECK (t >= 0 && (size_t) t < s->tracers.size (), GFSHIP_EINVAL, "no tracer %d", t);
  GFSHIP_CHECK (D >= 0., GFSHIP_EINVAL, "the diffusion coefficient must be positive");
  GFSHIP_CHECK (D == 0. || !s->dom->has_external, GFSHIP_EUNSUPPORTED,
		"GfsSourceDiffusion on a tracer on a box with GfsBoundaryMpi sides is not supported");
  s->tracer_D[t] = D;
  return GFSHIP_OK;
}

gfship_multilevel_params * gfship_sim_tracer_diffusion_params (gfship_sim * s, int t)
{ return (s && t >= 0 && (size_t) t < s->tracers.size ()) ? &s->tracer_diffusion_params[t] : nullptr; }

int gfship_sim_set_tracer_scheme (gfship_sim * s, int t, int scheme)
{
  GFSHIP_CHECK (s != nullptr, GFSHIP_EINVAL, "null simulation");
  GFSHIP_CHECK (t >= 0 && (size_t) t < s->tracers.size (), GFSHIP_EINVAL, "no tracer %d", t);
  GFSHIP_CHECK (scheme == GFSHIP_SCHEME_GODUNOV || scheme == GFSHIP_SCHEME_NONE, GFSHIP_EINVAL,
		"scheme: GFSHIP_SCHEME_GODUNOV or GFSHIP_SCHEME_NONE");
  s->tracer_scheme[t] = scheme;
  return GFSHIP_OK;
}

int gfship_sim_tracer_diffusion_path (gfship_sim * s, int fused)
{
  GFSHIP_CHECK (s != nullptr, GFSHIP_EINVAL, "null simulation");
  GFSHIP_CHECK (fused == 0 || fused == 1, GFSHIP_EINVAL, "path: 1 the fused pass where it applies, 0 composed");
  s->tracer_diffusion_fused = fused != 0;
  return GFSHIP_OK;
}

int gfship_sim_tracer_diffusion_counts (gfship_sim * s, unsigned long long counts[2])
{
  GFSHIP_CHECK (s && counts, GFSHIP_EINVAL, "null argument");
  counts[0] = s->tracer_diffusion_counts[0];
  counts[1] = s->tracer_diffusion_counts[1];
  return GFSHIP_OK;
}

static int cfl_full (gfship_sim * s, double * const u[3], double * const un[3], double * c2)
{
  double * msrc[3] = { nullptr, nullptr, nullptr };
  for (int c = 0; c < s->dom->dim; c++) {
    const double * m;
    TRY (mac_source_array (s, c, &m));
    msrc[c] = const_cast<double *> (m);
  }
  return launch_cfl (s->dom, u, un, s->visc, c2, msrc);
}

static int domain_cfl (gfship_sim * s, double * cfl, bool cached)
{
  double * u[3], * un[3];
  ptrs3 (s, s->u, u);
  ptrs3 (s, s->un, un);
  double c2;
  if (cached && s->cfl_ready)
    TRY (launch_cfl_from_max (s->dom, &c2));
  else {
    TRY (materialize_un (s));
    TRY (cfl_full (s, u, un, &c2));
  }
  s->cfl_ready = false;
  *cfl = sqrt (c2);
  return GFSHIP_OK;
}

int gfship_domain_cfl (gfship_sim * s, double * cfl)
{
  GFSHIP_CHECK (s && cfl, GFSHIP_EINVAL, "null argument");
  double * u[3], * un[3];
  ptrs3 (s, s->u, u);
  ptrs3 (s, s->un, un);
  double c2;
  s->cfl_ready = false;
  TRY (materialize_un (s));
  TRY (cfl_full (s, u, un, &c2));
  *cfl = sqrt (c2);
  return GFSHIP_OK;
}

static int set_timestep (gfship_sim * s, bool cached)
{
  double t = s->t;
  double cfl = s->advection_params.cfl;
  if (cfl < DBL_MAX) {
    double dcfl;
    TRY (domain_cfl (s, &dcfl, cached));
    s->advection_params.dt = cfl*dcfl;
  }
  else
    s->advection_params.dt = G_MAXINT;
  if (s->advection_params.dt > s->dtmax)
    s->advection_params.dt = s->dtmax;

  double tnext = G_MAXINT;
  if (s->next_event)
    tnext = s->next_event (s->next_event_ctx, t, s->i);
  if (s->end < tnext)
    tnext = s->end;

  double n = ceil ((tnext - t)/s->advection_params.dt);
  if (n > 0. && n < G_MAXINT) {
    s->advection_params.dt = (tnext - t)/n;
    if (n == 1.)
      s->tnext = tnext;
    else
      s->tnext = t + s->advection_params.dt;
  }
  else
    s->tnext = t + s->advection_params.dt;

  if (s->advection_params.dt < 1e-9)
    s->advection_params.dt = 1e-9;
  return GFSHIP_OK;
}

int gfship_set_timestep (gfship_sim * s)
{
  GFSHIP_CHECK (s != nullptr, GFSHIP_EINVAL, "null simulation");
  return set_timestep (s, false);
}

static void sim_variables (gfship_sim * s, std::vector<Field *> & v)
{
  gfship_domain * dom = s->dom;
  v.push_back (get_field (dom, s->p));
  v.push_back (get_field (dom, s->pmac));
  for (int c = 0; c < dom->dim; c++)
    v.push_back (get_field (dom, s->u[c]));
  for (gfship_field t : s->tracers)
    v.push_back (get_field (dom, t));
}

int gfship_sim_set_tracer_gradient (gfship_sim * s, int t, int gradient)
{
  GFSHIP_CHECK (s != nullptr, GFSHIP_EINVAL, "null simulation");
  GFSHIP_CHECK (t >= 0 && (size_t) t < s->tracers.size (), GFSHIP_EINVAL, "no tracer %d", t);
  GFSHIP_CHECK (gradient >= 0 && gradient <= 4, GFSHIP_EINVAL,
		"gradient: 0 centred, 1 van Leer, 2 minmod, 3 superbee, 4 sweby");
  s->tracer_gradient[t] = gradient;
  return GFSHIP_OK;
}

static int coarse_init (gfship_sim * s, bool u_done);

int gfship_coarse_init (gfship_sim * s)
{
  GFSHIP_CHECK (s != nullptr, GFSHIP_EINVAL, "null simulation");
  return coarse_init (s, false);
}

static int coarse_init (gfship_sim * s, bool u_done)
{
  std::vector<Field *> v;
  sim_variables (s, v);
  Field * pmac = get_field (s->dom, s->pmac);
  std::vector<Field *> now, vel;
  for (Field * F : v) {
    bool is_u = false;
    for (int c = 0; c < s->dom->dim; c++)
      if (F == get_field (s->dom, s->u[c])) is_u = true;
    if (F == pmac) F->coarse_stale = true;
    else {
      F->coarse_stale = false;
      F->coarse_valid = true;
      if (u_done && is_u) vel.push_back (F); else now.push_back (F);
    }
  }
  if (vel.empty ())
    return launch_coarse_init (s->dom, now.data (), (int) now.size ());
  TRY (launch_coarse_init_levels (s->dom, now.data (), (int) now.size (), s->dom->depth - 1, s->dom->depth - 1));
  now.insert (now.end (), vel.begin (), vel.end ());
  if (s->dom->depth >= 2)
    TRY (launch_coarse_init_levels (s->dom, now.data (), (int) now.size (), s->dom->depth - 2, 0));
  return GFSHIP_OK;
}

int gfship_sim_start (gfship_sim * s)
{
  GFSHIP_CHECK (s != nullptr, GFSHIP_EINVAL, "null simulation");
  GFSHIP_CHECK (s->advection_params.gc, GFSHIP_EUNSUPPORTED, "gc = 0 is not supported");
  TRY (bc_leaf (s, s->p));
  TRY (bc_leaf (s, s->pmac));
  for (int c = 0; c < s->dom->dim; c++)
    TRY (bc_leaf (s, s->u[c]));
  for (gfship_field t : s->tracers)
    TRY (bc_leaf (s, t));
  TRY (gfship_coarse_init (s));

  TRY (gfship_set_timestep (s));
  if (s->i == 0) {
    TRY (gfship_approximate_projection (s, &s->approx_projection_params, s->advection_params.dt,
					s->p, s->g));
    TRY (set_timestep (s, true));
    TRY (advance_tracers (s, s->advection_params.dt/2.));
  }
  else {
    double * gp[3];
    ptrs3 (s, s->g, gp);
    if (s->has_alpha) {
      TRY (gfship_poisson_coefficients_alpha (s->dom, s->alpha));
      TRY (launch_project_correct_weighted (s->dom, leaf (s, s->p), nullptr, gp, nullptr, 0.));
    }
    else {
      TRY (gfship_poisson_coefficients (s->dom));
      TRY (launch_centered_gradient (s->dom, leaf (s, s->p), gp));
    }
    for (int c = 0; c < s->dom->dim; c++)
      TRY (bc_leaf (s, s->g[c]));
  }
  return GFSHIP_OK;
}

int gfship_sim_restart (gfship_sim * s, double t, unsigned i)
{
  GFSHIP_CHECK (s != nullptr, GFSHIP_EINVAL, "null simulation");
  s->t = s->tnext = t;
  s->i = i;
  return GFSHIP_OK;
}

int gfship_sim_advection_step (gfship_sim * s)
{
  GFSHIP_CHECK (s != nullptr, GFSHIP_EINVAL, "null simulation");
  TRY (materialize_un (s));
  TRY (gfship_coarse_init (s));
  TRY (set_timestep (s, false));
  TRY (advance_tracers (s, s->advection_params.dt));
  s->t = s->tnext;
  s->i++;
  return GFSHIP_OK;
}

int gfship_sim_step (gfship_sim * s)
{
  GFSHIP_CHECK (s != nullptr, GFSHIP_EINVAL, "null simulation");
  gfship_domain * dom = s->dom;
  const gfship_field * gc = s->g;

  TRY (predicted_face_velocities (s, s->advection_params.dt/2.));

  {
    Field * P = get_field (dom, s->p), * PM = get_field (dom, s->pmac);
    std::swap (P->lev, PM->lev);
    int r = mac_projection (s, &s->projection_params, s->advection_params.dt/2., s->p, s->gmac);
    std::swap (P->lev, PM->lev);
    if (r != GFSHIP_OK) return r;
  }

  bool u_coarse = false, corrected = false;
  TRY (centered_velocity_advection (s, s->gmac, s->i > 0 ? gc : s->gmac, - s->advection_params.dt,
				    &corrected, &u_coarse));
  if (!corrected)
    TRY (correct_centered_velocities (s, s->i > 0 ? gc : s->gmac, - s->advection_params.dt, &u_coarse));

  TRY (coarse_init (s, u_coarse));

  TRY (mac_projection (s, &s->approx_projection_params, s->advection_params.dt, s->p, s->g, true, true));
  s->t = s->tnext;
  s->i++;

  TRY (set_timestep (s, true));
  TRY (advance_tracers (s, s->advection_params.dt));
  return GFSHIP_OK;
}

int gfship_divergence_norm (gfship_sim * s, gfship_norm * out)
{
  GFSHIP_CHECK (s && out, GFSHIP_EINVAL, "null argument");
  double * u[3];
  ptrs3 (s, s->u, u);
  TRY (launch_velocity_divergence (s->dom, u, leaf (s, s->div)));
  return gfship_norm_variable (s->dom, s->div, out);
}

int gfship_sim_download_un (gfship_sim * s, int c, double * host)
{
  GFSHIP_CHECK (s && host, GFSHIP_EINVAL, "null argument");
  GFSHIP_CHECK (c >= 0 && c < s->dom->dim, GFSHIP_EINVAL, "component %d out of range", c);
  TRY (materialize_un (s));
  return gfship_field_download (s->dom, s->un[c], s->dom->depth, host);
}

}
```

### gerris-fft-particles_amd/csrc/timestep_kernels.hip

```cpp
#include "gfship_internal.hpp"
#include "cell_loop.hpp"
#include <cfloat>

namespace gfship {

#define EXT_PROLOGUE(L)							\
  int i = blockIdx.x*blockDim.x + threadIdx.x;				\
  int j = blockIdx.y;							\
  int k = (L).dim == 3 ? blockIdx.z : 0;				\
  if (i > (L).n) return;						\
  long c = (L).idx (i, j, k)

static inline void ext_grid (const Layout & L, dim3 * grid, dim3 * block)
{
  int b = L.n >= 256 ? 256 : L.n >= 128 ? 128 : 64;
  *block = dim3 (b);
  *grid = dim3 ((L.n + 1 + b - 1)/b, L.n + 1, L.dim == 3 ? L.n + 1 : 1);
}

struct Ptr3  { double * p[3]; };
struct CPtr3 { const double * p[3]; };
struct Ptr6  { double * p[6]; };
struct CPtr6 { const double * p[6]; };
struct Visc3 { double d[3]; double g[3]; };
// ... 2509 lines not shown
    vn[q] = u.p[q][col + plane (kb + 1)];
  }
  for (int p = kb; p <= kb + SWZ + 1; p++) {
#pragma unroll
    for (int q = 0; q < 3; q++) {
      vm[q] = v0[q]; v0[q] = vp[q]; vp[q] = vn[q];
      vn[q] = u.p[q][col + plane (p + 2)];
      S_.V[q][ty + 1][tx + 1] = v0[q];
    }
    __syncthreads ();
    const int rp = p & 1, ro = rp ^ 1;
    FacePair F[3];
    double uxpn, uypn;
    {
      Stencil7 W;
      W.v0 = v0[0];
      W.m[0] = S_.V[0][ty + 1][tx];  W.p[0] = S_.V[0][ty + 1][tx + 2];
      W.m[1] = S_.V[0][ty][tx + 1];  W.p[1] = S_.V[0][ty + 2][tx + 1];
      W.m[2] = vm[0];                W.p[2] = vp[0];
      uxpn = W.p[0];
      F[0] = cen_face_values_s<0, VL, VS> (W, v0, dt, n, visc.d[0], visc.g[0]);
      S_.FRx[rp][ty][tx] = F[0].r;
      W.v0 = v0[1];
      W.m[0] = S_.V[1][ty + 1][tx];  W.p[0] = S_.V[1][ty + 1][tx + 2];
      W.m[1] = S_.V[1][ty][tx + 1];  W.p[1] = S_.V[1][ty + 2][tx + 1];
      W.m[2] = vm[1];                W.p[2] = vp[1];
      uypn = W.p[1];
      F[1] = cen_face_values_s<1, VL, VS> (W, v0, dt, n, visc.d[1], visc.g[1]);
      S_.FRy[rp][ty][tx] = F[1].r;
      W.v0 = v0[2];
      W.m[0] = S_.V[2][ty + 1][tx];  W.p[0] = S_.V[2][ty + 1][tx + 2];
      W.m[1] = S_.V[2][ty][tx + 1];  W.p[1] = S_.V[2][ty + 2][tx + 1];
      W.m[2] = vm[2];                W.p[2] = vp[2];
      F[2] = cen_face_values_s<2, VL, VS> (W, v0, dt, n, visc.d[2], visc.g[2]);
      if (MPI) {
	if (zlo && p == 0) F[2].l = G.r[5][fpos];
	if (zhi && p == n + 1) F[2].r = G.r[4][fpos];
      }
    }
    double unv[3] = { 0., 0., 0. };
    if (p > kb) {
      const int o = p - 1, co = col + plane (o);
      unv[0] = upwinded (face_interp (vm[0], uxp), flo[0], S_.FRx[ro][ty][tx + 1]);
      unv[1] = upwinded (face_interp (vm[1], uyp), flo[1], S_.FRy[ro][ty + 1][tx]);
      unv[2] = upwinded (face_interp (vm[2], v0[2]), flo[2], F[2].r);
      if (o >= 1 && o <= n) {
	un.p[0][co] = unv[0];
	un.p[1][co] = unv[1];
	un.p[2][co] = unv[2];
	if (i == n && !xmpi) un.p[0][co - n] = unv[0];
	if (j == n && !ympi) un.p[1][co - n*sy] = unv[1];
	if (o == n && !zlo) un.p[2][co - n*sz] = unv[2];
      }
      else if (MPI && zlo && o == 0)
	un.p[2][co] = unv[2];
      if (DIV) {
	S_.UOx[ty][tx + 1] = unv[0];
	S_.UOy[ty + 1][tx] = unv[1];
      }
    }
    __syncthreads ();
    if (p > kb) {
      if (DIV && p > kb + 1) {
	const int co = col + plane (p - 1);
	const double h = 1./n;
	double d_ = 0.;
	d_ += 1.*unv[0]*1.;
	d_ += -1.*S_.UOx[ty][tx]*1.;
	d_ += 1.*unv[1]*1.;
	d_ += -1.*S_.UOy[ty][tx]*1.;
	d_ += 1.*unv[2]*1.;
	d_ += -1.*unzo*1.;
	const double w_ = d_*h;
	div[co] = w_/div_dt;
      }
      unzo = unv[2];
    }
#pragma unroll
    for (int d = 0; d < 3; d++)
      flo[d] = F[d].l;
    uxp = uxpn; uyp = uypn;
  }
}

template <int DIM>
__global__ void __launch_bounds__(256)
cfl_partial_kernel (Layout L, CPtr3 u, CPtr3 un, Visc3 visc, CPtr3 msrc, double * __restrict__ partial)
{
  const int n = L.n;
  const double length = 1./n;
  const long r = n + 1;
  const long next = DIM == 3 ? r*r*r : r*r;
  const long off[3] = { 1, L.sy, L.sz };
  double m = DBL_MAX;
  for (long q = (long) blockIdx.x*blockDim.x + threadIdx.x; q < next;
       q += (long) gridDim.x*blockDim.x) {
    int i = q % r, j = (q / r) % r, k = DIM == 3 ? q / (r*r) : 0;
    long c = L.idx (i, j, k);
#pragma unroll
    for (int cc = 0; cc < DIM; cc++)
      if (face_valid<DIM> (n, cc, i, j, k)) {
	double unf = un.p[cc][c];
	if (unf != 0.) {
	  double cflu = length/fabs (unf);
	  m = fmin (m, cflu*cflu);
	}
      }
    if (i >= 1 && j >= 1 && (DIM == 2 || k >= 1)) {
#pragma unroll
      for (int cc = 0; cc < DIM; cc++) {
	double uv = u.p[cc][c];
	if (uv != 0.) {
	  double cflu = length/fabs (1.*uv);
	  m = fmin (m, cflu*cflu);
	}
	if ((visc.d[cc] != 0. || visc.g[cc] != 0. || msrc.p[cc]) && i <= n && j <= n && (DIM == 2 || k <= n)) {
	  double g = 0.;
	  if (msrc.p[cc]) g += msrc.p[cc][c];
	  else if (visc.d[cc] != 0.) g += source_diffusion_value<DIM> (u.p[cc], c, off, visc.d[cc], n);
	  if (visc.g[cc] != 0.) g += visc.g[cc];
	  if (g != 0.) {
	    double cflg = 2.*length/fabs (1.*g);
	    m = fmin (m, cflg);
	  }
	}
      }
    }
  }
  __shared__ double sh[4];
  m = wave_min (m);
  if ((threadIdx.x & 63) == 0) sh[threadIdx.x >> 6] = m;
  __syncthreads ();
  if (threadIdx.x == 0) {
    double rmin = sh[0];
    for (int q = 1; q < (int) (blockDim.x >> 6); q++) rmin = fmin (rmin, sh[q]);
    partial[blockIdx.x] = rmin;
  }
}

__global__ void __launch_bounds__(256)
min_final_kernel (const double * __restrict__ partial, int nblocks, double * __restrict__ out)
{
  double m = DBL_MAX;
  for (int q = threadIdx.x; q < nblocks; q += blockDim.x)
    m = fmin (m, partial[q]);
  __shared__ double sh[4];
  m = wave_min (m);
  if ((threadIdx.x & 63) == 0) sh[threadIdx.x >> 6] = m;
  __syncthreads ();
  if (threadIdx.x == 0)
    out[0] = fmin (fmin (sh[0], sh[1]), fmin (sh[2], sh[3]));
}

struct CoarseArgs { double * vc[8]; const double * vf[8]; int nf; };

template <int DIM>
__global__ void __launch_bounds__(256)
coarse_init_kernel (Layout Lc, Layout Lf, CoarseArgs A)
{
  CELL_LOOP_PROLOGUE (Lc);
  for (int f = 0; f < A.nf; f++) {
    double val = 0., sa = 0.;
#pragma unroll
    for (int id = 0; id < (1 << DIM); id++) {
      int ci = 2*i - 1 + (id & 1);
      int cj = 2*j - 1 + ((id & 2) ? 0 : 1);
      int ck = DIM == 3 ? 2*k - 1 + ((id & 4) ? 0 : 1) : 0;
      double a = 1.;
      val += A.vf[f][Lf.idx (ci, cj, ck)]*a;
      sa += a;
    }
    A.vc[f][c] = val/sa;
  }
}

template <int DIM>
__global__ void __launch_bounds__(256)
velocity_divergence_kernel (Layout L, CPtr3 u, double * __restrict__ out)
{
  CELL_LOOP_PROLOGUE (L);
  const long off[3] = { 1, L.sy, L.sz };
  double h = 1./L.n;
  double div = 0.;
#pragma unroll
  for (int cc = 0; cc < DIM; cc++) {
    div += 1.*1.*face_interp (u.p[cc][c], u.p[cc][c + off[cc]]);
    div += 1.*-1.*face_interp (u.p[cc][c], u.p[cc][c - off[cc]]);
  }
  out[c] = div/(1.*h);
}

#define DISPATCH(dom, kern, grid, block, ...)				\
  do {									\
    if ((dom)->dim == 3)						\
      hipLaunchKernelGGL (kern<3>, grid, block, 0, (dom)->stream, __VA_ARGS__); \
    else								\
      hipLaunchKernelGGL (kern<2>, grid, block, 0, (dom)->stream, __VA_ARGS__); \
    GFSHIP_HIP (hipGetLastError ());					\
  } while (0)

static CPtr3 c3 (double * const p[3]) { CPtr3 r; for (int q = 0; q < 3; q++) r.p[q] = p[q]; return r; }
static Ptr3  m3 (double * const p[3]) { Ptr3 r; for (int q = 0; q < 3; q++) r.p[q] = p[q]; return r; }
static CPtr6 c6 (double * const p[6]) { CPtr6 r; for (int q = 0; q < 6; q++) r.p[q] = p[q]; return r; }
static Ptr6  m6 (double * const p[6]) { Ptr6 r; for (int q = 0; q < 6; q++) r.p[q] = p[q]; return r; }

int launch_face_interp_un (gfship_domain * dom, double * const u[3], double * const un[3])
{
  const Layout & L = dom->lay[dom->depth];
  dim3 grid, block;
  ext_grid (L, &grid, &block);
  DISPATCH (dom, face_interp_un_kernel, grid, block, L, c3 (u), m3 (un));
  return GFSHIP_OK;
}

int launch_divergence (gfship_domain * dom, double * const un[3], double * div, double dt)
{
  const Layout & L = dom->lay[dom->depth];
  dim3 grid, block;
  cell_grid (L, &grid, &block);
  DISPATCH (dom, divergence_kernel, grid, block, L, c3 (un), div, dt);
  return GFSHIP_OK;
}

int launch_correct_un (gfship_domain * dom, const double * p, double * const un[3], double dt)
{
  const Layout & L = dom->lay[dom->depth];
  dim3 grid, block;
  ext_grid (L, &grid, &block);
  DISPATCH (dom, correct_un_kernel, grid, block, L, p, m3 (un), dt);
  return GFSHIP_OK;
}

int launch_centered_gradient (gfship_domain * dom, const double * p, double * const g[3])
{
  const Layout & L = dom->lay[dom->depth];
  dim3 grid, block;
  cell_grid (L, &grid, &block);
  DISPATCH (dom, centered_gradient_kernel, grid, block, L, p, m3 (g));
  return GFSHIP_OK;
}

int launch_correct_centered (gfship_domain * dom, double * const u[3], double * const g[3], double dt)
{
  const Layout & L = dom->lay[dom->depth];
  dim3 grid, block;
  cell_grid (L, &grid, &block);
  DISPATCH (dom, correct_centered_kernel, grid, block, L, m3 (u), c3 (g), dt);
  return GFSHIP_OK;
}

int launch_correct_centered_coarse (gfship_domain * dom, double * const u[3], double * const g[3],
				    double dt, double * const uc[3])
{
  const Layout & L = dom->lay[dom->depth], & Lc = dom->lay[dom->depth - 1];
  dim3 grid, block;
  cell_grid (Lc, &grid, &block);
  hipLaunchKernelGGL (correct_centered_coarse_kernel, grid, block, 0, dom->stream, L, Lc, m3 (u), c3 (g), dt,
		      m3 (uc));
  GFSHIP_HIP (hipGetLastError ());
  return GFSHIP_OK;
}

int launch_advected_face_values (gfship_domain * dom, const double * v, double * const u[3],
				 double * const un[3], double dt, int use_centered, int gradient,
				 double * const fv[6], int cmask, double visc, double gsrc, const double * msrc)
{
  const Layout & L = dom->lay[dom->depth];
  dim3 grid, block;
  cell_grid (L, &grid, &block);
  DISPATCH (dom, advected_face_values_kernel, grid, block, L, v, c3 (u), c3 (un), dt,
	    use_centered, gradient, m6 (fv), cmask, visc, gsrc, msrc);
  return GFSHIP_OK;
}

int launch_variable_mac_source (gfship_domain * dom, const double * v, double * const D[3],
				const double * alpha, double * out)
{
  const Layout & L = dom->lay[dom->depth];
  dim3 grid, block;
  cell_grid (L, &grid, &block);
  DISPATCH (dom, variable_mac_source_kernel, grid, block, L, v, c3 (D), alpha, out);
  return GFSHIP_OK;
}

int launch_face_bc (gfship_domain * dom, Field * v, double * const fv[6], int cmask)
{
  const Layout & L = dom->lay[dom->depth];
  BcDesc bc;
  for (int d = 0; d < 6; d++) {
    bc.side[d] = dom->side[d];
    bc.type[d] = v->bc[d];
    bc.val[d] = v->bcval[d];
  }
  bc.component = v->component;
  bc.homogeneous = 0;
  int nface = dom->dim == 3 ? L.n*L.n : L.n;
  int block = nface >= 256 ? 256 : 64;
  dim3 grid ((nface + block - 1)/block, 2*dom->dim);
  DISPATCH (dom, face_bc_kernel, grid, dim3 (block), L, bc, (const double *) v->lev[dom->depth],
	    m6 (fv), cmask);
  if (dom->has_external)
    for (int e = 0; e < 2*dom->dim; e++)
      if (dom->side[e ^ 1] == GFSHIP_SIDE_EXTERNAL && (cmask & (1 << (e/2)))) {
	int r = call_exchange (dom, fv[e], dom->depth, 1 + e);
	if (r) return r;
      }
  return GFSHIP_OK;
// ... 235 lines not shown
    if (r) return r;
    const dim3 bgrid ((L.n*L.n + 255)/256, 6);
    CPtr3 none = { { nullptr, nullptr, nullptr } };
    with_bools ([&] (auto VL, auto VS) {
      hipLaunchKernelGGL ((boundary_face_values_kernel<true, decltype (VL)::value, decltype (VS)::value>), bgrid, dim3 (256), 0,
			  dom->stream, L, c3 (u), none, dt, vs, G);
    }, gradient != 0, anyv);
    GFSHIP_HIP (hipGetLastError ());
    if ((r = comm_exchange_raw (dom, dom->gfv_send, dom->gfv_recv, (size_t) L.n*L.n))) return r;
    dom->n_fused_mpi++;
  }
  const bool sweep_fits = dom->sw.advect_sweep && L.n % SWX == 0 && L.n % SWY == 0 && L.n % SWZ == 0;
  if (sweep_fits && (!mpi || dom->sw.mpi_sweep)) {
    const dim3 sgrid (L.n/SWX, L.n/SWY, L.n/SWZ);
    const bool dv = div != nullptr && div_dt != 0.;
    with_bools ([&] (auto VL, auto VS, auto DV, auto MPI) {
      hipLaunchKernelGGL ((predict_un_sweep_kernel<decltype (VL)::value, decltype (VS)::value, decltype (DV)::value, decltype (MPI)::value>),
			  sgrid, dim3 (SWN + SW_RING), 0, dom->stream, L, c3 (u), m3 (un), dt, vs, div, div_dt, G);
    }, gradient != 0, anyv, dv, mpi);
    GFSHIP_HIP (hipGetLastError ());
    dom->kc[mpi ? GFSHIP_KC_PREDICT_SWEEP_MPI : GFSHIP_KC_PREDICT_SWEEP]++;
    if (div_done) *div_done = dv;
    return GFSHIP_OK;
  }
  const dim3 grid (L.n/GX, L.n/GY, L.n/GZ);
  with_bools ([&] (auto VL, auto VS, auto MPI) {
    hipLaunchKernelGGL ((predict_un_tiled_kernel<decltype (VL)::value, decltype (VS)::value, decltype (MPI)::value>), grid, dim3 (GN), 0,
			dom->stream, L, c3 (u), m3 (un), dt, vs, G);
  }, gradient != 0, anyv, mpi);
  GFSHIP_HIP (hipGetLastError ());
  dom->kc[mpi ? GFSHIP_KC_PREDICT_TILED_MPI : GFSHIP_KC_PREDICT_TILED]++;
  return GFSHIP_OK;
}

int launch_advect_fused (gfship_domain * dom, bool velocity, const double * v, double * out,
			 double * const un[3], const double * gm, const double * gc, double dt,
			 int gradient, double visc, double gsrc)
{
  const Layout & L = dom->lay[dom->depth];
  dim3 grid (L.n/GX, L.n/GY, L.n/GZ);
  with_bools ([&] (auto VE, auto VL, auto VS) {
    hipLaunchKernelGGL ((advect_tiled_kernel<decltype (VE)::value, decltype (VL)::value, decltype (VS)::value>), grid, dim3 (GN), 0,
			dom->stream, L, v, out, c3 (un), gm, gc, dt, visc, gsrc);
  }, velocity, gradient != 0, visc != 0. || gsrc != 0.);
  GFSHIP_HIP (hipGetLastError ());
  dom->kc[velocity ? GFSHIP_KC_ADVECT1_TILED_VELOCITY : GFSHIP_KC_ADVECT1_TILED_TRACER]++;
  return GFSHIP_OK;
}

int launch_advect_diffuse_fused (gfship_domain * dom, const double * v, double * out, double * const un[3],
				 double dt, int gradient, double D, double w, double beta)
{
  const Layout & L = dom->lay[dom->depth];
  dim3 grid (L.n/GX, L.n/GY, L.n/GZ);
  with_bools ([&] (auto VL) {
    hipLaunchKernelGGL ((advect_diffuse_tiled_kernel<decltype (VL)::value>), grid, dim3 (GN), 0,
			dom->stream, L, v, out, c3 (un), dt, D, w, (1. - beta)/beta);
  }, gradient != 0);
  GFSHIP_HIP (hipGetLastError ());
  return GFSHIP_OK;
}

int launch_advect3_fused (gfship_domain * dom, double * const v[3], double * const out[3],
			  double * const un[3], double * const gm[3], double * const gc[3],
			  double dt, int gradient, double corr_dt, double * const uc[3])
{
  const Layout & L = dom->lay[dom->depth];
  dim3 grid (L.n/GX, L.n/GY, L.n/GZ);
  CPtr3 gcp;
  for (int c = 0; c < 3; c++) gcp.p[c] = gc ? gc[c] : nullptr;
  GhostFv G;
  for (int d = 0; d < 6; d++) { G.r[d] = nullptr; G.s[d] = nullptr; }
  Visc3 vs = { { 0., 0., 0. }, { dom->src[0], dom->src[1], dom->src[2] } };
  AdvCorr K;
  K.dt = corr_dt;
  for (int c = 0; c < 3; c++) K.uc[c] = uc ? uc[c] : nullptr;
  K.Lc = dom->lay[dom->depth > 0 ? dom->depth - 1 : 0];
  const bool corr = corr_dt != 0.;
  GFSHIP_CHECK (!corr || gc, GFSHIP_EINVAL, "the fused correction needs the centred gradient");
  const bool srcs = dom->src[0] != 0. || dom->src[1] != 0. || dom->src[2] != 0.;
  const bool mpi = dom->has_external;
  if (mpi) {
    int r = ghost_fv (dom, &G);
    if (r) return r;
    const dim3 bgrid ((L.n*L.n + 255)/256, 6);
    with_bools ([&] (auto VL, auto VS) {
      hipLaunchKernelGGL ((boundary_face_values_kernel<false, decltype (VL)::value, decltype (VS)::value>), bgrid, dim3 (256), 0,
			  dom->stream, L, c3 (v), c3 (un), dt, vs, G);
    }, gradient != 0, srcs);
    GFSHIP_HIP (hipGetLastError ());
    if ((r = comm_exchange_raw (dom, dom->gfv_send, dom->gfv_recv, (size_t) 3*L.n*L.n))) return r;
    dom->n_fused_mpi++;
  }
  const bool sweep_fits = dom->sw.advect_sweep && L.n % SWX == 0 && L.n % SWY == 0 && L.n % SWZ == 0;
  if (sweep_fits && (!mpi || dom->sw.mpi_sweep)) {
    const dim3 sgrid (L.n/SWX, L.n/SWY, L.n/SWZ);
    const bool sweep1 = !mpi && dom->sw.advect_sweep1;
    if (sweep1)
      with_bools ([&] (auto VL, auto SRC, auto CORR) {
	hipLaunchKernelGGL ((advect3_sweep_kernel<decltype (VL)::value, decltype (SRC)::value, decltype (CORR)::value>),
			    sgrid, dim3 (SWN + SW_RING), 0, dom->stream, L, c3 (v), m3 (out), c3 (un), c3 (gm), gcp, dt, vs, K);
      }, gradient != 0, srcs, corr);
    else
      with_bools ([&] (auto VL, auto SRC, auto CORR, auto MPI) {
	hipLaunchKernelGGL ((advect3_sweep2_kernel<decltype (VL)::value, decltype (SRC)::value, decltype (CORR)::value, decltype (MPI)::value>),
			    sgrid, dim3 (SWN + SW_RING), 0, dom->stream, L, c3 (v), m3 (out), c3 (un), c3 (gm), gcp, dt, vs, K, G);
      }, gradient != 0, srcs, corr, mpi);
    GFSHIP_HIP (hipGetLastError ());
    dom->kc[mpi ? GFSHIP_KC_ADVECT3_SWEEP2_MPI : sweep1 ? GFSHIP_KC_ADVECT3_SWEEP1 : GFSHIP_KC_ADVECT3_SWEEP2]++;
    return GFSHIP_OK;
  }
  with_bools ([&] (auto VL, auto MPI, auto SRC, auto CORR) {
    hipLaunchKernelGGL ((advect3_tiled_kernel<decltype (VL)::value, decltype (MPI)::value, decltype (SRC)::value, ADV3_WPE, decltype (CORR)::value>),
			grid, dim3 (GN), 0, dom->stream, L, c3 (v), m3 (out), c3 (un), c3 (gm), gcp, dt, G, vs, K);
  }, gradient != 0, mpi, srcs, corr);
  GFSHIP_HIP (hipGetLastError ());
  dom->kc[mpi ? GFSHIP_KC_ADVECT3_TILED_MPI : GFSHIP_KC_ADVECT3_TILED]++;
  return GFSHIP_OK;
}

int launch_cfl (gfship_domain * dom, double * const u[3], double * const un[3],
		const double visc[3], double * cfl2, double * const msrc[3])
{
  double * const none[3] = { nullptr, nullptr, nullptr };
  Visc3 vs;
  for (int c = 0; c < 3; c++) { vs.d[c] = visc ? visc[c] : 0.; vs.g[c] = dom->src[c]; }
  const Layout & L = dom->lay[dom->depth];
  long r = L.n + 1;
  long next = dom->dim == 3 ? r*r*r : r*r;
  int block = 256;
  int nblocks = (int) ((next + block - 1)/block);
  if (nblocks > 1024) nblocks = 1024;
  double * partial = dom->d_scratch;
  double * result = dom->h_pinned;
  DISPATCH (dom, cfl_partial_kernel, dim3 (nblocks), dim3 (block), L, c3 (u), c3 (un), vs, c3 (msrc ? msrc : none),
	    partial);
  hipLaunchKernelGGL (min_final_kernel, dim3 (1), dim3 (256), 0, dom->stream, partial, nblocks, result);
  GFSHIP_HIP (hipGetLastError ());
  GFSHIP_HIP (stream_wait_spin (dom->stream));
  *cfl2 = dom->h_pinned[0];
  return call_reduce (dom, cfl2, 1, 2);
}

int launch_coarse_init (gfship_domain * dom, Field * const * v, int nf)
{
  return launch_coarse_init_from (dom, v, nf, dom->depth - 1);
}

int launch_coarse_init_from (gfship_domain * dom, Field * const * v, int nf, int top)
{
  return launch_coarse_init_levels (dom, v, nf, top, 0);
}

int launch_coarse_init_levels (gfship_domain * dom, Field * const * v, int nf, int top, int bottom)
{
  for (int f0 = 0; f0 < nf; f0 += 8) {
    int m = nf - f0 < 8 ? nf - f0 : 8;
    for (int l = top; l >= bottom; l--) {
      const Layout & Lc = dom->lay[l], & Lf = dom->lay[l + 1];
      CoarseArgs A;
      A.nf = m;
      for (int f = 0; f < m; f++) {
	A.vc[f] = v[f0 + f]->lev[l];
	A.vf[f] = v[f0 + f]->lev[l + 1];
	v[f0 + f]->zero[l] = false;
	v[f0 + f]->coarse_valid = true;
      }
      dim3 grid, block;
      cell_grid (Lc, &grid, &block);
      DISPATCH (dom, coarse_init_kernel, grid, block, Lc, Lf, A);
    }
  }
  return GFSHIP_OK;
}

int launch_velocity_divergence (gfship_domain * dom, double * const u[3], double * out)
{
  const Layout & L = dom->lay[dom->depth];
  dim3 grid, block;
  cell_grid (L, &grid, &block);
  DISPATCH (dom, velocity_divergence_kernel, grid, block, L, c3 (u), out);
  return GFSHIP_OK;
}

}
```

### gerris-fft-particles_amd/gfship/__init__.py

```python
import ctypes as C
import os
import sys

import numpy as np

_PKG = os.path.dirname(os.path.dirname(os.path.abspath(__file__)))
LIB_PATH = os.environ.get("GFSHIP_LIB", os.path.join(_PKG, "lib", "libgfship.so"))

SIDE_PERIODIC, SIDE_BOUNDARY, SIDE_EXTERNAL = 0, 1, 2
BC_SYMMETRY, BC_DIRICHLET, BC_NEUMANN = 0, 1, 2
SCHEME_GODUNOV, SCHEME_NONE = 0, 1
RELAX_EXACT, RELAX_REDBLACK, RELAX_EXACT_HYPERPLANE, RELAX_EXACT_PER_SWEEP = 0, 1, 2, 3


class GfshipError(RuntimeError):
    pass


class Norm(C.Structure):
    _fields_ = [("bias", C.c_double), ("first", C.c_double), ("second", C.c_double),
                ("infty", C.c_double), ("w", C.c_double)]


class MultilevelParams(C.Structure):
    _fields_ = [("tolerance", C.c_double), ("nrelax", C.c_uint), ("erelax", C.c_uint),
                ("minlevel", C.c_uint), ("nitermax", C.c_uint), ("nitermin", C.c_uint),
                ("dimension", C.c_uint), ("niter", C.c_uint), ("depth", C.c_uint),
                ("weighted", C.c_int), ("function", C.c_int),
                ("beta", C.c_double), ("omega", C.c_double),
                ("residual_before", Norm), ("residual", Norm)]


class AdvectionParams(C.Structure):
    _fields_ = [("cfl", C.c_double), ("dt", C.c_double), ("gradient", C.c_int), ("gc", C.c_int)]


_lib = None

_vp, _i, _d, _u = C.c_void_p, C.c_int, C.c_double, C.c_uint
_pd = C.POINTER(C.c_double)
_pi = C.POINTER(C.c_int)
SIGNATURES = {
    "gfship_last_error": (C.c_char_p, []),
    "gfship_version": (_i, []),
    "gfship_device_count": (_i, []),
    "gfship_domain_create": (_i, [C.POINTER(_vp), _i, _i, _pi, _i]),
    "gfship_domain_destroy": (None, [_vp]),
    "gfship_domain_set_relax_mode": (_i, [_vp, _i]),
    "gfship_domain_synchronize": (_i, [_vp]),
    "gfship_domain_stream": (_vp, [_vp]),
    "gfship_field_alloc": (_i, [_vp, _i]),
    "gfship_field_free": (_i, [_vp, _i]),
    "gfship_field_set_bc": (_i, [_vp, _i, _i, _i, _pd]),
    "gfship_field_upload": (_i, [_vp, _i, _i, _pd]),
    "gfship_field_download": (_i, [_vp, _i, _i, _pd]),
    "gfship_field_fill": (_i, [_vp, _i, _i, _d]),
    "gfship_field_device_ptr": (_vp, [_vp, _i, _i, _pi, _pi]),
    "gfship_bc": (_i, [_vp, _i, _i, _i]),
    "gfship_homogeneous_bc": (_i, [_vp, _i, _i, _i]),
    "gfship_multilevel_params_init": (None, [C.POINTER(MultilevelParams), _i]),
    "gfship_poisson_coefficients": (_i, [_vp]),
    "gfship_poisson_coefficients_alpha": (_i, [_vp, _pi]),
    "gfship_poisson_weights": (_i, [_vp, _i, _pi]),
    "gfship_relax": (_i, [_vp, _u, _i, _d, _i, _i, _i]),
    "gfship_residual": (_i, [_vp, _u, _i, _i, _i, _i, _i]),
    "gfship_norm_residual": (_i, [_vp, _d, _i, C.POINTER(Norm)]),
    "gfship_norm_variable": (_i, [_vp, _i, C.POINTER(Norm)]),
    "gfship_poisson_cycle": (_i, [_vp, C.POINTER(MultilevelParams), _i, _i, _i, _i]),
    "gfship_poisson_solve": (_i, [_vp, C.POINTER(MultilevelParams), _i, _i, _i, _i, _d]),
    "gfship_diffusion_coefficients": (_i, [_vp, _d, _d, _i, _d]),
    "gfship_diffusion_coefficients_faces": (_i, [_vp, _pi, _d, _i, _i, _d]),
    "gfship_diffusion_rhs": (_i, [_vp, _i, _i, _i, _d]),
    "gfship_diffusion_residual": (_i, [_vp, _i, _i, _i, _i]),
    "gfship_diffusion_cycle": (_i, [_vp, _u, _u, _u, _i, _i, _i, _i]),
    "gfship_diffusion": (_i, [_vp, C.POINTER(MultilevelParams), _i, _i, _i]),
    "gfship_time_relax": (_i, [_vp, _u, _i, _i, _i, _i, _i, _pd]),
    "gfship_time_relax_loop": (_i, [_vp, _i, _i, _i, _i, _u, _i, _pd, _pi]),
    "gfship_time_relax_loop_inclusive": (_i, [_vp, _i, _i, _i, _i, _u, _i, _pd, _pi, _pd]),
    "gfship_sim_create": (_i, [C.POINTER(_vp), _vp]),
    "gfship_sim_destroy": (None, [_vp]),
    "gfship_sim_variable": (_i, [_vp, _i, _i]),
    "gfship_sim_projection_params": (C.POINTER(MultilevelParams), [_vp]),
    "gfship_sim_approx_projection_params": (C.POINTER(MultilevelParams), [_vp]),
    "gfship_sim_advection_params": (C.POINTER(AdvectionParams), [_vp]),
    "gfship_sim_set_time": (_i, [_vp, _d, _d]),
    "gfship_sim_set_next_event": (_i, [_vp, _vp, _vp]),
    "gfship_sim_time": (_d, [_vp]),
    "gfship_sim_iter": (_u, [_vp]),
    "gfship_sim_add_tracer": (_i, [_vp]),
    "gfship_sim_set_viscosity": (_i, [_vp, _i, _d]),
    "gfship_sim_set_viscosity_faces": (_i, [_vp, _i, _pi]),
    "gfship_sim_set_alpha_cell": (_i, [_vp, _i]),
    "gfship_sim_set_viscosity_cell": (_i, [_vp, _i]),
    "gfship_variable_mac_source": (_i, [_vp, _i, _i]),
    "gfship_sim_set_alpha": (_i, [_vp, _pi]),
    "gfship_sim_set_source": (_i, [_vp, _i, _d]),
    "gfship_sim_diffusion_params": (C.POINTER(MultilevelParams), [_vp, _i]),
    "gfship_sim_start": (_i, [_vp]),
    "gfship_sim_step": (_i, [_vp]),
    "gfship_sim_advection_step": (_i, [_vp]),
    "gfship_sim_set_tracer_gradient": (_i, [_vp, _i, _i]),
    "gfship_sim_set_tracer_scheme": (_i, [_vp, _i, _i]),
    "gfship_sim_set_tracer_diffusion": (_i, [_vp, _i, _d]),
    "gfship_sim_tracer_diffusion_params": (C.POINTER(MultilevelParams), [_vp, _i]),
    "gfship_sim_tracer_diffusion_path": (_i, [_vp, _i]),
    "gfship_sim_tracer_diffusion_counts": (_i, [_vp, C.POINTER(C.c_ulonglong)]),
    "gfship_predicted_face_velocities": (_i, [_vp]),
    "gfship_mac_projection": (_i, [_vp, C.POINTER(MultilevelParams), _d, _i, _pi]),
    "gfship_approximate_projection": (_i, [_vp, C.POINTER(MultilevelParams), _d, _i, _pi]),
    "gfship_centered_velocity_advection": (_i, [_vp, _pi, _pi]),
    "gfship_correct_centered_velocities": (_i, [_vp, _pi, _d]),
    "gfship_sim_advance_time": (_i, [_vp]),
    "gfship_tracer_advection": (_i, [_vp, _i, _d]),
    "gfship_domain_cfl": (_i, [_vp, _pd]),
    "gfship_set_timestep": (_i, [_vp]),
    "gfship_coarse_init": (_i, [_vp]),
    "gfship_divergence_norm": (_i, [_vp, C.POINTER(Norm)]),
    "gfship_sim_download_un": (_i, [_vp, _i, _pd]),
    "gfship_domain_set_overlap": (_i, [_vp, _i]),
    "gfship_domain_set_exchange": (_i, [_vp, _vp, _vp]),
    "gfship_domain_set_reduce": (_i, [_vp, _vp, _vp]),
    "gfship_domain_set_gather": (_i, [_vp, _vp, _vp, _i, _i, C.POINTER(C.c_int)]),
    "gfship_domain_path_counts": (_i, [_vp, C.POINTER(C.c_ulonglong), C.POINTER(C.c_ulonglong)]),
    "gfship_domain_kernel_counts": (_i, [_vp, C.POINTER(C.c_ulonglong), _i]),
    "gfship_sim_restart": (_i, [_vp, _d, _u]),
    "gfship_snapshot_tree_bytes": (C.c_size_t, [_vp, _i]),
    "gfship_snapshot_tree_write": (_i, [_vp, _i, _pi, _vp, C.c_size_t]),
    "gfship_snapshot_tree_read": (_i, [_vp, _i, _pi, _vp, C.c_size_t]),
    "gfship_comm_available": (_i, []),
    "gfship_comm_unique_id": (_i, [_vp]),
    "gfship_domain_comm_init": (_i, [_vp, _vp, _i, _i, _pi]),
    "gfship_domain_comm_size": (_i, [_vp]),
    "gfship_domain_comm_stats": (_i, [_vp, C.POINTER(C.c_ulonglong), C.POINTER(C.c_ulonglong)]),
    "gfship_domain_comm_destroy": (_i, [_vp]),
    "gfship_halo_pack": (_i, [_vp, _vp, _i, _i, _vp]),
    "gfship_halo_unpack": (_i, [_vp, _vp, _i, _i, _vp]),
    "gfship_halo_pack_sides": (_i, [_vp, _vp, _i, _i, _pi, C.POINTER(_vp)]),
    "gfship_halo_unpack_sides": (_i, [_vp, _vp, _i, _i, _pi, C.POINTER(_vp)]),
    "gfship_field_interpolate": (_i, [_vp, _i, _i, _pd, _pd, C.POINTER(C.c_ubyte)]),
    "gfship_particles_create": (_i, [C.POINTER(_vp), _vp, _i, _pd, C.POINTER(C.c_uint)]),
    "gfship_particles_destroy": (None, [_vp]),
    "gfship_particle_list_event": (_i, [_vp]),
    "gfship_particles_count": (_i, [_vp]),
    "gfship_particles_set_migrate": (_i, [_vp, _vp, _vp]),
    "gfship_particles_slots": (_i, [_vp]),
    "gfship_particles_record_size": (_i, [_vp]),
    "gfship_particles_sort": (_i, [_vp]),
    "gfship_particles_set_sort_interval": (_i, [_vp, _i]),
    "gfship_particles_download": (_i, [_vp, _pd, C.POINTER(C.c_uint)]),
    "gfship_particles_download_old": (_i, [_vp, _pd]),
    "gfship_energy_spectra_bins": (_i, [_vp]),
    "gfship_energy_spectra": (_i, [_vp, _i, C.POINTER(_i), _pd, C.POINTER(C.c_double),
                                   C.POINTER(C.c_double)]),
    "gfship_init_spectra": (_i, [_vp, _vp, C.POINTER(_i)]),
    "gfship_output_spectra_side": (_i, [_vp]),
    "gfship_output_spectra": (_i, [_vp, _i, _pd, C.POINTER(C.c_double)]),
    "gfship_output_spectra_plane": (_i, [_vp, _i, _i, _d, _pd, _pd]),
    "gfship_turbulent_viscosity": (_i, [_vp, C.POINTER(_i), C.c_double, _i, _i]),
    "gfship_particles_set_particulate": (_i, [_vp, _pd, _pd, _pd]),
    "gfship_particles_set_forces": (_i, [_vp, _i, C.POINTER(_i), _pd]),
    "gfship_particles_set_force_coefficient": (_i, [_vp, _i, C.c_char_p]),
    "gfship_particles_download_particulate": (_i, [_vp, _pd, _pd, _pd]),
    "gfship_particulate_field": (_i, [_vp, _i]),
    "gfship_particles_forces_on_fluid": (_i, [_vp]),
    "gfship_particles_set_kernel": (_i, [_vp, C.c_double, C.c_char_p]),
    "gfship_source_particulate_event": (_i, [_vp, C.POINTER(_i)]),
    "gfship_particles_spread_forces": (_i, [_vp, C.POINTER(_i)]),
    "gfship_sim_set_source_fields": (_i, [_vp, C.POINTER(_i)]),
    "gfship_particles_time_spreading": (_i, [_vp, C.POINTER(_i), _pd]),
    "gfship_tree_create": (_i, [C.POINTER(_vp), _i, C.c_void_p, _vp, _i]),
    "gfship_tree_create_sides": (_i, [C.POINTER(_vp), _i, C.c_void_p, _vp, _pi, _i]),
    "gfship_tree_set_bc": (_i, [_vp, _i, _i]),
    "gfship_tree_poisson_solve": (_i, [_vp, C.POINTER(MultilevelParams), _d]),
    "gfship_tree_destroy": (None, [_vp]),
    "gfship_tree_depth": (_i, [_vp]),
    "gfship_tree_dim": (_i, [_vp]),
    "gfship_tree_flags": (_i, [_vp, _i, C.POINTER(C.c_ubyte)]),
    "gfship_tree_upload": (_i, [_vp, _i, _i, _pd]),
    "gfship_tree_download": (_i, [_vp, _i, _i, _pd]),
    "gfship_tree_projection_params": (C.POINTER(MultilevelParams), [_vp, _i]),
    "gfship_tree_set_time": (_i, [_vp, _d, _d]),
    "gfship_tree_set_next_event": (_i, [_vp, _vp, _vp]),
    "gfship_tree_time": (_d, [_vp]),
    "gfship_tree_dt": (_d, [_vp]),
    "gfship_tree_iter": (_u, [_vp]),
    "gfship_tree_add_tracer": (_i, [_vp, _i]),
    "gfship_tree_set_bc_u": (_i, [_vp, _i, _i, _i]),
    "gfship_tree_set_viscosity": (_i, [_vp, _i, _d]),
    "gfship_tree_set_source": (_i, [_vp, _i, _d]),
    "gfship_tree_diffusion_params": (C.POINTER(MultilevelParams), [_vp, _i]),
    "gfship_tree_start": (_i, [_vp]),
    "gfship_tree_step": (_i, [_vp]),
    "gfship_tree_snapshot_bytes": (C.c_size_t, [_vp, _i]),
    "gfship_tree_snapshot_write": (_i, [_vp, _i, _pi, _vp, C.c_size_t]),
    "gfship_tree_snapshot_read": (_i, [_vp, _i, _pi, _vp, C.c_size_t]),
    "gfship_tree_restart": (_i, [_vp, _d, _u]),
    "gfship_tree_sweep_levels": (_i, [_vp, _i, _pi, _pi]),
    "gfship_tree_divergence": (_i, [_vp]),
    "gfship_tree_host_check": (_i, [_i, C.c_void_p, _vp, _pi, _u, C.POINTER(C.c_longlong)]),
    "gfship_tree_host_check_diffusion": (_i, [_i, C.c_void_p, _vp, _pi, _u, _d, C.POINTER(C.c_longlong)]),
    "gfship_tree_interpolate": (_i, [_vp, _i, _i, _pd, _pd, C.POINTER(C.c_ubyte)]),
    "gfship_tree_sampler_stats": (_i, [_vp, C.POINTER(C.c_longlong)]),
    "gfship_particles_create_tree": (_i, [C.POINTER(_vp), _vp, _i, _pd, C.POINTER(C.c_uint)]),
    "gfship_particulates_create_tree": (_i, [C.POINTER(_vp), _vp, _i, _pd, C.POINTER(C.c_uint), _pd, _pd, _pd]),
    "gfship_tree_particulate_field": (_i, [_vp, _i]),
    "gfship_tree_particles_forces_on_fluid": (_i, [_vp]),
    "gfship_tree_particles_set_kernel": (_i, [_vp, C.c_double, C.c_char_p]),
    "gfship_tree_particles_spread_forces": (_i, [_vp]),
    "gfship_tree_source_particulate_event": (_i, [_vp]),
    "gfship_tree_set_source_fields": (_i, [_vp, _i]),
    "gfship_tree_mac_source": (_i, [_vp, _i, _i]),
}


UNIQUE_ID_BYTES = 128

KERNEL_COUNT_NAMES = (
    "PREDICT_SWEEP", "PREDICT_SWEEP_MPI", "PREDICT_TILED", "PREDICT_TILED_MPI", "PREDICT_GENERAL",
    "ADVECT3_SWEEP2", "ADVECT3_SWEEP2_MPI", "ADVECT3_SWEEP1", "ADVECT3_TILED", "ADVECT3_TILED_MPI",
    "ADVECT1_TILED_VELOCITY", "ADVECT1_TILED_TRACER", "ADVECT_GENERAL", "CORRECTION_FUSED",
    "CORRECTION_DECLINED", "DIVERGENCE_FUSED", "DIVERGENCE_DECLINED", "DIVERGENCE_SEPARATE",
    "PROJECT_PAIRS", "PROJECT_SCALAR", "RESIDUAL_PAIRS", "RESIDUAL_SCALAR", "RN_BLOCKS_LIMIT",
    "RN_BLOCKS_MAX", "ROWS2D", "HYPERPLANES_2D", "DIFFUSION_PIPELINED", "DIFFUSION_HYPERPLANES",
    "WEIGHTED_PIPELINED", "WEIGHTED_HYPERPLANES", "PROLONGATION_FUSED", "PROLONGATION_DECLINED",
    "RESTRICTION_FUSED", "RESTRICTION_DECLINED", "PROLONG_PACK_NEW", "PROLONG_PACK_OLD",
    "ARM_AHEAD", "ARM_AHEAD_DECLINED", "ARM_INLINE", "PATCH_LOOP_KERNEL_ARMS",
    "PATCH_LOOP_HOST_ARMS", "XCD_SCOPE_ON", "XCD_SCOPE_OFF", "XCD_NEAR_MODE", "XCD_PLACE_ON",
    "XCD_PLACE_OFF", "COARSE_CYCLES", "COARSE_THREADS", "COARSE_END_BY_LEVEL",
    "DIFFUSION_FACES_PIPELINED", "DIFFUSION_FACES_HYPERPLANES",
)
KERNEL_COUNT_VALUES = ("RN_BLOCKS_LIMIT", "RN_BLOCKS_MAX", "XCD_NEAR_MODE", "COARSE_THREADS")


def comm_available():
    _check(lib().gfship_comm_available())


def comm_unique_id():
    buf = C.create_string_buffer(UNIQUE_ID_BYTES)
    _check(lib().gfship_comm_unique_id(buf))
    return buf.raw


def lib():
    global _lib
    if _lib is None:
        if not os.path.exists(LIB_PATH):
            raise GfshipError("%s not found: run __graft_entry__.build() "
                              "(gerris-fft-particles_amd/csrc/build.sh)" % LIB_PATH)
        if "torch" not in sys.modules and os.environ.get("GFSHIP_NO_TORCH") is None:
            try:
                import torch
            except ImportError:
                pass
        L = C.CDLL(LIB_PATH)
        for name, (res, args) in SIGNATURES.items():
            f = getattr(L, name)
            f.restype, f.argtypes = res, args
        _lib = L
    return _lib


def _check(rc):
    if rc < 0:
        raise GfshipError("gfship error %d: %s" % (rc, lib().gfship_last_error().decode()))
    return rc


class Variable:

    def __init__(self, dom, component=-1):
        self.dom = dom
        self.h = _check(lib().gfship_field_alloc(dom.ptr, component))

    def _shape(self, level):
        return ((1 << level) + 2,) * self.dom.dim

    def upload(self, a, level=None):
        level = self.dom.depth if level is None else level
        a = np.ascontiguousarray(a, dtype=np.float64)
        assert a.shape == self._shape(level), (a.shape, self._shape(level))
        _check(lib().gfship_field_upload(self.dom.ptr, self.h, level, a.ctypes.data_as(_pd)))

    def download(self, level=None):
        level = self.dom.depth if level is None else level
        a = np.empty(self._shape(level), dtype=np.float64)
        _check(lib().gfship_field_download(self.dom.ptr, self.h, level, a.ctypes.data_as(_pd)))
        return a

    def fill(self, value, level=None):
        level = self.dom.depth if level is None else level
        _check(lib().gfship_field_fill(self.dom.ptr, self.h, level, value))

    def set_bc(self, d, kind, val=None):
        if val is not None:
            val = np.ascontiguousarray(val, dtype=np.float64).ravel()
            p = val.ctypes.data_as(_pd)
        else:
            p = None
        _check(lib().gfship_field_set_bc(self.dom.ptr, self.h, d, kind, p))

    def free(self):
        if self.h is not None and self.dom.ptr:
            lib().gfship_field_free(self.dom.ptr, self.h)
            self.h = None


class Domain:

    def __init__(self, dim, depth, side=None, device=0):
        self.dim, self.depth = dim, depth
        s = (C.c_int * 6)(*(side if side is not None else [SIDE_BOUNDARY] * 6))
        p = _vp()
        _check(lib().gfship_domain_create(C.byref(p), dim, depth, s, device))
        self.ptr = p

    def variable(self, component=-1):
        return Variable(self, component)

    def params(self):
        par = MultilevelParams()
        lib().gfship_multilevel_params_init(C.byref(par), self.dim)
        return par

    def comm_init(self, unique_id, rank, nranks, lattice):
        buf = C.create_string_buffer(bytes(unique_id), UNIQUE_ID_BYTES)
        _check(lib().gfship_domain_comm_init(self.ptr, buf, rank, nranks, (C.c_int * 3)(*lattice)))

    def comm_size(self):
        return _check(lib().gfship_domain_comm_size(self.ptr))

    def comm_stats(self):
        m, b = C.c_ulonglong(), C.c_ulonglong()
        _check(lib().gfship_domain_comm_stats(self.ptr, C.byref(m), C.byref(b)))
        return int(m.value), int(b.value)

    def path_counts(self):
        a, b = C.c_ulonglong(), C.c_ulonglong()
        _check(lib().gfship_domain_path_counts(self.ptr, C.byref(a), C.byref(b)))
        return int(a.value), int(b.value)

    def kernel_counts(self):
        n = len(KERNEL_COUNT_NAMES)
        a = (C.c_ulonglong * n)()
        _check(lib().gfship_domain_kernel_counts(self.ptr, a, n))
        return {name: int(a[k]) for k, name in enumerate(KERNEL_COUNT_NAMES)}

    def snapshot_tree(self, variables):
        n = len(variables)
        h = (C.c_int * n)(*[v.h for v in variables])
        size = lib().gfship_snapshot_tree_bytes(self.ptr, n)
        buf = C.create_string_buffer(size)
        _check(lib().gfship_snapshot_tree_write(self.ptr, n, h, buf, size))
        return buf.raw

    def snapshot_tree_read(self, variables, data):
        n = len(variables)
        h = (C.c_int * n)(*[v.h for v in variables])
        buf = C.create_string_buffer(bytes(data), len(data))
        _check(lib().gfship_snapshot_tree_read(self.ptr, n, h, buf, len(data)))

    def set_overlap(self, overlap):
        _check(lib().gfship_domain_set_overlap(self.ptr, int(overlap)))

    def set_relax_mode(self, mode):
        _check(lib().gfship_domain_set_relax_mode(self.ptr, mode))

    def synchronize(self):
        _check(lib().gfship_domain_synchronize(self.ptr))

    def bc(self, v, v1=None, level=None):
        level = self.depth if level is None else level
        _check(lib().gfship_bc(self.ptr, v.h, (v1 or v).h, level))

    def homogeneous_bc(self, ov, v, level=None):
        level = self.depth if level is None else level
        _check(lib().gfship_homogeneous_bc(self.ptr, ov.h, v.h, level))

    def poisson_coefficients(self):
        _check(lib().gfship_poisson_coefficients(self.ptr))

    def poisson_coefficients_alpha(self, alpha):
        h = (C.c_int * 3)(*([v.h for v in alpha] + [-1] * (3 - len(alpha))))
        _check(lib().gfship_poisson_coefficients_alpha(self.ptr, h))

    def poisson_weight(self, d, level=None):
        w = C.c_int()
        _check(lib().gfship_poisson_weights(self.ptr, d, C.byref(w)))
        v = Variable.__new__(Variable)
        v.dom, v.h = self, w.value
        a = v.download(level)
        v.h = None
        return a

    def relax(self, u, rhs, dia, level=None, omega=1., d=None):
        level = self.depth if level is None else level
        _check(lib().gfship_relax(self.ptr, d or self.dim, level, omega, u.h, rhs.h, dia.h))

    def residual(self, u, rhs, dia, res, level=None, d=None):
        level = self.depth if level is None else level
        _check(lib().gfship_residual(self.ptr, d or self.dim, level, u.h, rhs.h, dia.h, res.h))

    def norm_residual(self, res, dt=1.):
        n = Norm()
        _check(lib().gfship_norm_residual(self.ptr, dt, res.h, C.byref(n)))
        return n

    def norm_variable(self, v):
        n = Norm()
        _check(lib().gfship_norm_variable(self.ptr, v.h, C.byref(n)))
        return n

    def poisson_cycle(self, par, u, rhs, dia, res):
        _check(lib().gfship_poisson_cycle(self.ptr, C.byref(par), u.h, rhs.h, dia.h, res.h))

    def poisson_solve(self, par, lhs, rhs, res, dia, dt=1.):
        _check(lib().gfship_poisson_solve(self.ptr, C.byref(par), lhs.h, rhs.h, res.h, dia.h, dt))

    def diffusion_coefficients(self, D, dt, rhoc, beta=1.):
        _check(lib().gfship_diffusion_coefficients(self.ptr, D, dt, rhoc.h, beta))

    def diffusion_coefficients_faces(self, D, dt, rhoc, alpha_cell=None, beta=1.):
        h = (C.c_int * 3)(*([v.h for v in D] + [-1] * (3 - len(D))))
        _check(lib().gfship_diffusion_coefficients_faces(self.ptr, h, dt, rhoc.h,
                                                         -1 if alpha_cell is None else alpha_cell.h, beta))

    def diffusion_rhs(self, v, rhs, rhoc, beta=1.):
        _check(lib().gfship_diffusion_rhs(self.ptr, v.h, rhs.h, rhoc.h, beta))

    def diffusion_residual(self, u, rhs, rhoc, res):
        _check(lib().gfship_diffusion_residual(self.ptr, u.h, rhs.h, rhoc.h, res.h))

    def diffusion_cycle(self, levelmin, nrelax, u, rhs, rhoc, res):
        _check(lib().gfship_diffusion_cycle(self.ptr, levelmin, self.depth, nrelax,
                                            u.h, rhs.h, rhoc.h, res.h))

    def diffusion(self, par, v, rhs, rhoc):
        _check(lib().gfship_diffusion(self.ptr, C.byref(par), v.h, rhs.h, rhoc.h))

    def time_relax_loop(self, u, rhs, dia, nrelax=4, level=None, reps=5):
        level = self.depth if level is None else level
        ms, fused = C.c_double(), C.c_int()
        _check(lib().gfship_time_relax_loop(self.ptr, level, u.h, rhs.h, dia.h, nrelax, reps,
                                            C.byref(ms), C.byref(fused)))
        return ms.value, bool(fused.value)

    def time_relax_loop_inclusive(self, u, rhs, dia, nrelax=4, level=None, reps=5):
        level = self.depth if level is None else level
        ms, fused, incl = C.c_double(), C.c_int(), C.c_double()
        _check(lib().gfship_time_relax_loop_inclusive(self.ptr, level, u.h, rhs.h, dia.h, nrelax, reps,
                                                      C.byref(ms), C.byref(fused), C.byref(incl)))
        return ms.value, bool(fused.value), incl.value

    def energy_spectra(self, comps):
        nk = _check(lib().gfship_energy_spectra_bins(self.ptr))
        Ek = np.empty(nk)
        etot, dk = C.c_double(), C.c_double()
        h = (_i * len(comps))(*[c.h for c in comps])
        _check(lib().gfship_energy_spectra(self.ptr, len(comps), h, Ek.ctypes.data_as(_pd),
                                           C.byref(etot), C.byref(dk)))
        i = np.arange(1, nk)
        return dk.value * np.sqrt(i.astype(float)), Ek[1:].copy(), etot.value

    def output_spectra(self, v):
        N = _check(lib().gfship_output_spectra_side(self.ptr))
        out = np.empty((N, N, N // 2 + 1), dtype=np.complex128)
        ks = C.c_double()
        _check(lib().gfship_output_spectra(self.ptr, v.h, out.ctypes.data_as(_pd), C.byref(ks)))
        return out, ks.value

    def output_spectra_plane(self, v, normal, pos):
        N = _check(lib().gfship_output_spectra_side(self.ptr))
        out = np.empty((N, N), dtype=np.complex128)
        ks = C.c_double()
        _check(lib().gfship_output_spectra_plane(self.ptr, v.h, int(normal), float(pos),
                                                 out.ctypes.data_as(_pd), C.byref(ks)))
        return out, ks.value

    def turbulent_viscosity(self, u, Cs, out, model=1):
        h = (_i * 3)(*([c.h for c in u] + [u[-1].h] * (3 - len(u))))
        _check(lib().gfship_turbulent_viscosity(self.ptr, h, float(Cs), int(model), out.h))

    def init_spectra(self, par, fields):
        p = InitSpectraParams()
        for k, v in par.items():
            setattr(p, k, v)
        h = (_i * 3)(*[f.h for f in fields])
        _check(lib().gfship_init_spectra(self.ptr, C.byref(p), h))

    def interpolate(self, v, points):
        pts = np.ascontiguousarray(points, dtype=np.float64).reshape(-1, 3)
        out = np.empty(len(pts))
        inside = np.empty(len(pts), dtype=np.uint8)
        _check(lib().gfship_field_interpolate(self.ptr, v.h, len(pts), pts.ctypes.data_as(_pd),
# ... 522 lines not shown
```

### include/gfship.h

```cpp
#ifndef GFSHIP_H
#define GFSHIP_H

#include <stddef.h>

#ifdef __cplusplus
extern "C" {
#endif

#define GFSHIP_VERSION   1
#define GFSHIP_MAXLEVEL  12

enum { GFSHIP_OK = 0, GFSHIP_EINVAL = -1, GFSHIP_ENODEVICE = -2, GFSHIP_ENOMEM = -3,
       GFSHIP_EHIP = -4, GFSHIP_EUNSUPPORTED = -5 };

enum { GFSHIP_SIDE_PERIODIC = 0,
       GFSHIP_SIDE_BOUNDARY = 1,
       GFSHIP_SIDE_EXTERNAL = 2 };

enum { GFSHIP_BC_SYMMETRY = 0, GFSHIP_BC_DIRICHLET = 1, GFSHIP_BC_NEUMANN = 2 };

enum { GFSHIP_RELAX_EXACT = 0, GFSHIP_RELAX_REDBLACK = 1, GFSHIP_RELAX_EXACT_HYPERPLANE = 2,
       GFSHIP_RELAX_EXACT_PER_SWEEP = 3 };

typedef struct gfship_domain gfship_domain;
// ... 117 lines not shown
int  gfship_sim_restart (gfship_sim * sim, double t, unsigned i);
int  gfship_sim_step (gfship_sim * sim);
int  gfship_sim_advection_step (gfship_sim * sim);
int  gfship_predicted_face_velocities (gfship_sim * sim);
int  gfship_mac_projection (gfship_sim * sim, gfship_multilevel_params * par, double dt,
			    gfship_field p, const gfship_field g[3]);
int  gfship_approximate_projection (gfship_sim * sim, gfship_multilevel_params * par, double dt,
				    gfship_field p, const gfship_field g[3]);
int  gfship_centered_velocity_advection (gfship_sim * sim, const gfship_field gmac[3],
					 const gfship_field g[3]);
int  gfship_correct_centered_velocities (gfship_sim * sim, const gfship_field g[3], double dt);
int  gfship_tracer_advection (gfship_sim * sim, gfship_field t, double dt);
int  gfship_domain_cfl (gfship_sim * sim, double * cfl);
int  gfship_set_timestep (gfship_sim * sim);
int  gfship_coarse_init (gfship_sim * sim);
int  gfship_sim_advance_time (gfship_sim * sim);
int  gfship_divergence_norm (gfship_sim * sim, gfship_norm * out);
int  gfship_sim_download_un (gfship_sim * sim, int c, double * host);

int  gfship_field_interpolate (gfship_domain * dom, gfship_field v, int np, const double * pos,
			       double * out, unsigned char * inside);


size_t gfship_snapshot_tree_bytes (gfship_domain * dom, int nvars);
int  gfship_snapshot_tree_write (gfship_domain * dom, int nvars, const gfship_field * vars,
				 void * host_buf, size_t bytes);
int  gfship_snapshot_tree_read (gfship_domain * dom, int nvars, const gfship_field * vars,
				const void * host_buf, size_t bytes);


int  gfship_energy_spectra_bins (gfship_domain * dom);
int  gfship_energy_spectra (gfship_domain * dom, int ncomp, const gfship_field * comps, double * Ek,
			    double * Etot, double * deltak);

int  gfship_output_spectra_side (gfship_domain * dom);
int  gfship_output_spectra (gfship_domain * dom, gfship_field v, double * out, double * kstep);
int  gfship_output_spectra_plane (gfship_domain * dom, gfship_field v, int normal, double pos, double * out,
				  double * kstep);

int  gfship_turbulent_viscosity (gfship_domain * dom, const gfship_field u[3], double Cs, int model,
				 gfship_field out);

typedef struct {
  double x0, y0, z0, L, E;
  double alpha, epsilon, c1, c2, c3, ReL, kmax, seed;
  int level;
} gfship_init_spectra_params;
int  gfship_init_spectra (gfship_domain * dom, const gfship_init_spectra_params * par,
			  const gfship_field v[3]);


typedef struct gfship_particles gfship_particles;

int  gfship_particles_create (gfship_particles ** pl, gfship_sim * sim, int np,
			      const double * pos, const unsigned * id);
void gfship_particles_destroy (gfship_particles * pl);
int  gfship_particle_list_event (gfship_particles * pl);
int  gfship_particles_sort (gfship_particles * pl);
int  gfship_particles_set_sort_interval (gfship_particles * pl, int every);
typedef int (* gfship_particle_migrate_fn) (void * ctx, const int nsend[6],
					    const double * const send[6], int nrecv[6],
					    const double * recv[6]);
int  gfship_particles_set_migrate (gfship_particles * pl, gfship_particle_migrate_fn fn, void * ctx);
int  gfship_particles_record_size (gfship_particles * pl);
int  gfship_particles_slots (gfship_particles * pl);
int  gfship_particles_count (gfship_particles * pl);
int  gfship_particles_download (gfship_particles * pl, double * pos, unsigned * id);
int  gfship_particles_download_old (gfship_particles * pl, double * old);

enum { GFSHIP_FORCE_INERTIAL = 1, GFSHIP_FORCE_ADDEDMASS = 2, GFSHIP_FORCE_LIFT = 3,
       GFSHIP_FORCE_DRAG = 4, GFSHIP_FORCE_BUOY = 5 };
int  gfship_particles_set_particulate (gfship_particles * pl, const double * vel, const double * mass,
				       const double * volume);
int  gfship_particles_set_forces (gfship_particles * pl, int nforces, const int * kinds,
				  const double gravity[3]);
int  gfship_particles_set_force_coefficient (gfship_particles * pl, int force, const char * function);
int  gfship_particles_download_particulate (gfship_particles * pl, double * vel, double * mass,
					    double * force);

int  gfship_particulate_field (gfship_particles * pl, gfship_field v);
int  gfship_particles_forces_on_fluid (gfship_particles * pl);
int  gfship_particles_set_kernel (gfship_particles * pl, double rkernel, const char * function);
int  gfship_source_particulate_event (gfship_particles * pl, const gfship_field F[3]);
int  gfship_particles_spread_forces (gfship_particles * pl, const gfship_field F[3]);
int  gfship_particles_time_spreading (gfship_particles * pl, const gfship_field F[3], double info[5]);
int  gfship_sim_set_source_fields (gfship_sim * sim, const gfship_field F[3]);


int  gfship_domain_set_overlap (gfship_domain * dom, int overlap);
typedef int (* gfship_exchange_fn) (void * ctx, void * dev_ptr, int level, int kind);
typedef int (* gfship_reduce_fn) (void * ctx, double * vals, int n, int op);
int  gfship_domain_set_exchange (gfship_domain * dom, gfship_exchange_fn fn, void * ctx);
int  gfship_domain_set_reduce (gfship_domain * dom, gfship_reduce_fn fn, void * ctx);
typedef int (* gfship_gather_fn) (void * ctx, const void * dev_send, void * dev_recv, size_t bytes);
int  gfship_domain_set_gather (gfship_domain * dom, gfship_gather_fn fn, void * ctx, int rank,
			       int nboxes, const int lattice[3]);
int  gfship_domain_path_counts (gfship_domain * dom, unsigned long long * lattice_cycles,
				unsigned long long * fused_mpi_launches);
enum {
  GFSHIP_KC_PREDICT_SWEEP = 0,
  GFSHIP_KC_PREDICT_SWEEP_MPI,
  GFSHIP_KC_PREDICT_TILED,
  GFSHIP_KC_PREDICT_TILED_MPI,
  GFSHIP_KC_PREDICT_GENERAL,
  GFSHIP_KC_ADVECT3_SWEEP2,
  GFSHIP_KC_ADVECT3_SWEEP2_MPI,
  GFSHIP_KC_ADVECT3_SWEEP1,
  GFSHIP_KC_ADVECT3_TILED,
  GFSHIP_KC_ADVECT3_TILED_MPI,
  GFSHIP_KC_ADVECT1_TILED_VELOCITY,
  GFSHIP_KC_ADVECT1_TILED_TRACER,
  GFSHIP_KC_ADVECT_GENERAL,
  GFSHIP_KC_CORRECTION_FUSED,
  GFSHIP_KC_CORRECTION_DECLINED,
  GFSHIP_KC_DIVERGENCE_FUSED,
  GFSHIP_KC_DIVERGENCE_DECLINED,
  GFSHIP_KC_DIVERGENCE_SEPARATE,
  GFSHIP_KC_PROJECT_PAIRS,
  GFSHIP_KC_PROJECT_SCALAR,
  GFSHIP_KC_RESIDUAL_PAIRS,
  GFSHIP_KC_RESIDUAL_SCALAR,
  GFSHIP_KC_RN_BLOCKS_LIMIT,
  GFSHIP_KC_RN_BLOCKS_MAX,
  GFSHIP_KC_ROWS2D,
  GFSHIP_KC_HYPERPLANES_2D,
  GFSHIP_KC_DIFFUSION_PIPELINED,
  GFSHIP_KC_DIFFUSION_HYPERPLANES,
  GFSHIP_KC_WEIGHTED_PIPELINED,
  GFSHIP_KC_WEIGHTED_HYPERPLANES,
  GFSHIP_KC_PROLONGATION_FUSED,
  GFSHIP_KC_PROLONGATION_DECLINED,
  GFSHIP_KC_RESTRICTION_FUSED,
  GFSHIP_KC_RESTRICTION_DECLINED,
  GFSHIP_KC_PROLONG_PACK_NEW,
  GFSHIP_KC_PROLONG_PACK_OLD,
  GFSHIP_KC_ARM_AHEAD,
  GFSHIP_KC_ARM_AHEAD_DECLINED,
  GFSHIP_KC_ARM_INLINE,
  GFSHIP_KC_PATCH_LOOP_KERNEL_ARMS,
  GFSHIP_KC_PATCH_LOOP_HOST_ARMS,
  GFSHIP_KC_XCD_SCOPE_ON,
  GFSHIP_KC_XCD_SCOPE_OFF,
  GFSHIP_KC_XCD_NEAR_MODE,
  GFSHIP_KC_XCD_PLACE_ON,
  GFSHIP_KC_XCD_PLACE_OFF,
  GFSHIP_KC_COARSE_CYCLES,
  GFSHIP_KC_COARSE_THREADS,
  GFSHIP_KC_COARSE_END_BY_LEVEL,
  GFSHIP_KC_DIFFUSION_FACES_PIPELINED,
  GFSHIP_KC_DIFFUSION_FACES_HYPERPLANES,
  GFSHIP_KC_COUNT
};
int  gfship_domain_kernel_counts (gfship_domain * dom, unsigned long long * counts, int n);
#define GFSHIP_UNIQUE_ID_BYTES 128
int  gfship_comm_available (void);
int  gfship_comm_unique_id (void * id);
int  gfship_domain_comm_init (gfship_domain * dom, const void * unique_id, int rank, int nranks,
			      const int lattice[3]);
int  gfship_domain_comm_size (gfship_domain * dom);
int  gfship_domain_comm_stats (gfship_domain * dom, unsigned long long * messages,
			       unsigned long long * bytes);
int  gfship_domain_comm_destroy (gfship_domain * dom);

int  gfship_halo_pack (gfship_domain * dom, const void * dev_ptr, int level, int side, void * dev_buf);
int  gfship_halo_unpack (gfship_domain * dom, void * dev_ptr, int level, int side, const void * dev_buf);
int  gfship_halo_pack_sides (gfship_domain * dom, const void * dev_ptr, int level, int nsides,
			     const int * sides, void * const * dev_bufs);
int  gfship_halo_unpack_sides (gfship_domain * dom, void * dev_ptr, int level, int nsides,
			       const int * sides, void * const * dev_bufs);


typedef struct gfship_tree gfship_tree;
typedef double (* gfship_refine_fn) (double x, double y, double z, void * ctx);
enum { GFSHIP_TREE_P = 0, GFSHIP_TREE_PMAC, GFSHIP_TREE_U, GFSHIP_TREE_V, GFSHIP_TREE_GX, GFSHIP_TREE_GY,
       GFSHIP_TREE_GMACX, GFSHIP_TREE_GMACY, GFSHIP_TREE_UN0, GFSHIP_TREE_UN1, GFSHIP_TREE_UN2,
       GFSHIP_TREE_UN3, GFSHIP_TREE_W, GFSHIP_TREE_GZ, GFSHIP_TREE_GMACZ, GFSHIP_TREE_UN4,
       GFSHIP_TREE_UN5, GFSHIP_TREE_DIV, GFSHIP_TREE_BCVAL, GFSHIP_TREE_RES,
       GFSHIP_TREE_T0, GFSHIP_TREE_T1, GFSHIP_TREE_BCU, GFSHIP_TREE_BCV, GFSHIP_TREE_BCW,
       GFSHIP_TREE_UPREV, GFSHIP_TREE_VPREV, GFSHIP_TREE_WPREV };
enum { GFSHIP_TREE_VF = GFSHIP_TREE_WPREV + 1, GFSHIP_TREE_FX, GFSHIP_TREE_FY, GFSHIP_TREE_FZ };
int  gfship_tree_create (gfship_tree ** tree, int dim, gfship_refine_fn refine, void * ctx, int device);
int  gfship_tree_create_sides (gfship_tree ** tree, int dim, gfship_refine_fn refine, void * ctx,
			       const int * side, int device);
int  gfship_tree_set_bc (gfship_tree * tree, int d, int kind);
int  gfship_tree_poisson_solve (gfship_tree * tree, gfship_multilevel_params * par, double dt);
void gfship_tree_destroy (gfship_tree * tree);
int  gfship_tree_depth (const gfship_tree * tree);
int  gfship_tree_dim (const gfship_tree * tree);
int  gfship_tree_flags (const gfship_tree * tree, int level, unsigned char * out );
int  gfship_tree_upload (gfship_tree * tree, int var, int level, const double * in );
int  gfship_tree_download (gfship_tree * tree, int var, int level, double * out);
gfship_multilevel_params * gfship_tree_projection_params (gfship_tree * tree, int approx);
int  gfship_tree_set_time (gfship_tree * tree, double end, double cfl);
int  gfship_tree_set_next_event (gfship_tree * tree, gfship_next_event_fn fn, void * ctx);
double   gfship_tree_time (const gfship_tree * tree);
double   gfship_tree_dt (const gfship_tree * tree);
unsigned gfship_tree_iter (const gfship_tree * tree);
int  gfship_tree_add_tracer (gfship_tree * tree, int gradient);
int  gfship_tree_set_bc_u (gfship_tree * tree, int c, int d, int kind);
int  gfship_tree_set_viscosity (gfship_tree * tree, int c, double nu);
int  gfship_tree_set_source (gfship_tree * tree, int c, double g);
gfship_multilevel_params * gfship_tree_diffusion_params (gfship_tree * tree, int c);
int  gfship_tree_start (gfship_tree * tree);
int  gfship_tree_step (gfship_tree * tree);
size_t gfship_tree_snapshot_bytes (const gfship_tree * tree, int nvars);
int  gfship_tree_snapshot_write (gfship_tree * tree, int nvars, const int * vars, void * host_buf, size_t bytes);
int  gfship_tree_snapshot_read (gfship_tree * tree, int nvars, const int * vars, const void * host_buf, size_t bytes);
int  gfship_tree_restart (gfship_tree * tree, double t, unsigned i);
int  gfship_tree_divergence (gfship_tree * tree);
int  gfship_tree_host_check (int dim, gfship_refine_fn refine, void * ctx, const int * side,
			     unsigned nrelax, long long stats[4]);
int  gfship_tree_host_check_diffusion (int dim, gfship_refine_fn refine, void * ctx, const int * side,
				       unsigned nrelax, double w, long long stats[6]);
int  gfship_tree_sweep_levels (const gfship_tree * tree, int level, int * ncells, int * nlevels);


int  gfship_tree_interpolate (gfship_tree * tree, int var, int np, const double * pos,
			      double * out, unsigned char * inside);
int  gfship_tree_sampler_stats (gfship_tree * tree, long long stats[5]);
int  gfship_particles_create_tree (gfship_particles ** pl, gfship_tree * tree, int np,
				   const double * pos, const unsigned * id);
int  gfship_particulates_create_tree (gfship_particles ** pl, gfship_tree * tree, int np,
				      const double * pos, const unsigned * id,
				      const double * vel, const double * mass, const double * volume);


int  gfship_tree_particulate_field (gfship_particles * pl, int var);
int  gfship_tree_particles_forces_on_fluid (gfship_particles * pl);
int  gfship_tree_particles_set_kernel (gfship_particles * pl, double rkernel, const char * function);
int  gfship_tree_particles_spread_forces (gfship_particles * pl);
int  gfship_tree_source_particulate_event (gfship_particles * pl);
int  gfship_tree_set_source_fields (gfship_tree * tree, int on);
int  gfship_tree_mac_source (gfship_tree * tree, int c, int var_out);


int  gfship_time_relax (gfship_domain * dom, unsigned d, int level, gfship_field u,
			gfship_field rhs, gfship_field dia, int reps, double * ms_per_sweep);

int  gfship_time_relax_loop (gfship_domain * dom, int level, gfship_field u, gfship_field rhs,
			     gfship_field dia, unsigned nrelax, int reps, double * ms_per_loop,
			     int * fused);

int  gfship_time_relax_loop_inclusive (gfship_domain * dom, int level, gfship_field u, gfship_field rhs,
				       gfship_field dia, unsigned nrelax, int reps,
				       double * ms_per_loop, int * fused, double * ms_inclusive);

#ifdef __cplusplus
}
#endif
#endif
```

Measured before the change: 2872 Mcell-steps/s.

## Overlap coarse-init and restricted RHS packing on side stream during multigrid cycle

Defers the coarse_init kernels into a job list and launches them on the side stream after restriction, joining the main stream only before the finest-level prolongation. The restricted residual's RHS packing is also split out of the fused restrict_pack kernel and issued on the side stream, with an event join before the relax loop needs it. The aim is to hide these memory-bound kernels behind coarse-level multigrid work, which underuses the GPU. In exchange the code gains cross-stream events and more complex ordering, and the side kernels compete for bandwidth and CUs with the main stream.

Result: no change. 2898 Mcell-steps/s, median of 6 (+0.9%).

```diff
diff --git a/gerris-fft-particles_amd/csrc/domain.hip b/gerris-fft-particles_amd/csrc/domain.hip
--- a/gerris-fft-particles_amd/csrc/domain.hip
+++ b/gerris-fft-particles_amd/csrc/domain.hip
@@ -94,6 +94,7 @@
   if (e == hipSuccess) e = hipEventCreate (&dom->ev1);
   if (e == hipSuccess) e = hipStreamCreateWithFlags (&dom->side_stream, hipStreamNonBlocking);
   if (e == hipSuccess) e = hipEventCreateWithFlags (&dom->side_fork, hipEventDisableTiming);
+  if (e == hipSuccess) e = hipEventCreateWithFlags (&dom->side_join, hipEventDisableTiming);
   dom->scratch_doubles = 5*8192 + 64;
   if (e == hipSuccess) e = hipMalloc ((void **) &dom->d_scratch, dom->scratch_doubles*sizeof (double));
   if (e == hipSuccess) e = hipHostMalloc ((void **) &dom->h_pinned, 64*sizeof (double), hipHostMallocDefault);
@@ -133,6 +134,7 @@
   if (dom->ev0) (void) hipEventDestroy (dom->ev0);
   if (dom->ev1) (void) hipEventDestroy (dom->ev1);
   if (dom->side_fork) (void) hipEventDestroy (dom->side_fork);
+  if (dom->side_join) (void) hipEventDestroy (dom->side_join);
   if (dom->side_stream) (void) hipStreamDestroy (dom->side_stream);
   if (dom->stream) (void) hipStreamDestroy (dom->stream);
   delete dom;
@@ -188,6 +190,15 @@
   dom->gather_ctx = ctx;
   dom->lat_rank = rank; dom->lat_n = nboxes;
   for (int c = 0; c < 3; c++) dom->lat_b[c] = lattice[c];
+  return GFSHIP_OK;
+}
+
+int gfship_domain_side_counts (gfship_domain * dom, unsigned long long * rhs_copies,
+			       unsigned long long * coarse_init_jobs)
+{
+  GFSHIP_CHECK (dom != nullptr, GFSHIP_EINVAL, "null domain");
+  if (rhs_copies) *rhs_copies = dom->n_rhs_copy_side;
+  if (coarse_init_jobs) *coarse_init_jobs = dom->n_coarse_init_side;
   return GFSHIP_OK;
 }
 
diff --git a/gerris-fft-particles_amd/csrc/gfship_internal.hpp b/gerris-fft-particles_amd/csrc/gfship_internal.hpp
--- a/gerris-fft-particles_amd/csrc/gfship_internal.hpp
+++ b/gerris-fft-particles_amd/csrc/gfship_internal.hpp
@@ -54,6 +54,9 @@
   hipEvent_t arm_ev = nullptr;
   bool arm_wait = false;
   bool loop_checked = false;
+  bool rs_side = false, rs_wait = false;
+  const double * rs_src = nullptr;
+  hipEvent_t rs_ev = nullptr;
   void * stats_loop = nullptr;
   void * ctl = nullptr;
   unsigned long long * stats = nullptr;
@@ -73,6 +76,9 @@
   for (int d = 0; d < 6; d++) wf.p[d] = op ? op->wf[d] : nullptr;
   return wf;
 }
+
+struct CoarseArgs { double * vc[8]; const double * vf[8]; int nf; };
+struct CoarseLaunch { int level; CoarseArgs A; };
 
 struct BcDesc {
   int side[6];
@@ -95,6 +101,9 @@
   hipEvent_t ev0 = nullptr, ev1 = nullptr;
   hipStream_t side_stream = nullptr;
   hipEvent_t side_fork = nullptr;
+  std::vector<gfship::CoarseLaunch> side_job;
+  hipEvent_t side_join = nullptr;
+  bool side_join_wait = false;
   int (* before_write) (void *) = nullptr;
   void * before_write_ctx = nullptr;
   double * d_scratch = nullptr;
@@ -114,6 +123,7 @@
   double src[3] = { 0., 0., 0. };
   unsigned long long n_lattice_cycles = 0, n_fused_mpi = 0;
   unsigned long long kc[GFSHIP_KC_COUNT] = {};
+  unsigned long long n_rhs_copy_side = 0, n_coarse_init_side = 0;
   bool lattice_attr_set = false;
   void * mpi_plan[GFSHIP_MAXLEVEL + 1] = {};
   gfship_field dp_cache = -1;
@@ -264,7 +274,11 @@
 int launch_correct_centered_coarse (gfship_domain * dom, double * const u[3], double * const g[3],
 				    double dt, double * const uc[3]);
 int launch_coarse_init_from (gfship_domain * dom, Field * const * v, int nf, int top);
-int launch_coarse_init_levels (gfship_domain * dom, Field * const * v, int nf, int top, int bottom);
+int launch_coarse_init_levels (gfship_domain * dom, Field * const * v, int nf, int top, int bottom,
+			       hipStream_t stream = nullptr, bool job = false);
+int launch_side_job (gfship_domain * dom, hipStream_t stream);
+bool side_window (gfship_domain * dom, const gfship_multilevel_params * p);
+int side_job_flush (gfship_domain * dom);
 int launch_advected_face_values (gfship_domain * dom, const double * v, double * const u[3],
 				 double * const un[3], double dt, int use_centered, int gradient,
 				 double * const fv[6], int cmask, double visc = 0., double gsrc = 0.,
@@ -325,6 +339,8 @@
 		     double * ms_per_loop, int * fused, double * ms_inclusive = nullptr);
 int  skew_check_error (gfship_domain * dom);
 int  skew_arm_ahead (gfship_domain * dom, int level, unsigned nrelax);
+int  skew_side_copies (gfship_domain * dom, bool * forked);
+int  skew_rs_join (gfship_domain * dom, int level);
 int  patch_resident_per_cu (const gfship_domain * dom);
 bool prolongation_fused (gfship_domain * dom, unsigned dimension, int level, unsigned nrelax);
 bool prolongation_fusable (gfship_domain * dom, unsigned dimension, int level, unsigned nrelax);
@@ -336,11 +352,12 @@
   return dom->sw.patch () && !per_cell_weights && dom->lay[level].n >= dom->sw.patch_min_n;
 }
 int  patch_pack (gfship_domain * dom, int level, SkewPlan * S, const double * u, const double * rhs,
-		 const double * dia, const double * coarse = nullptr);
+		 const double * dia, const double * coarse, hipStream_t stream);
+int  patch_pack_rhs (gfship_domain * dom, int level, SkewPlan * S, const double * rhs, hipStream_t stream);
 int  patch_unpack (gfship_domain * dom, int level, SkewPlan * S, double * u, double * add_into,
 		   const LoopGhosts * ghosts = nullptr);
 int  patch_restrict_pack (gfship_domain * dom, int level, SkewPlan * S, const double * res,
-			  double * res_coarse, SkewPlan * Sc, unsigned dimension);
+			  double * res_coarse, SkewPlan * Sc, unsigned dimension, bool pack, hipStream_t stream);
 int  launch_restrict_pack (gfship_domain * dom, unsigned dimension, int level, Field * res,
 			   bool coarse_fused);
 void skew_dump_stats (gfship_domain * dom, int level);
diff --git a/gerris-fft-particles_amd/csrc/poisson.hip b/gerris-fft-particles_amd/csrc/poisson.hip
--- a/gerris-fft-particles_amd/csrc/poisson.hip
+++ b/gerris-fft-particles_amd/csrc/poisson.hip
@@ -313,6 +313,60 @@
     n.infty = 0.;
   *out = n;
   return GFSHIP_OK;
+}
+
+}
+
+namespace gfship {
+
+bool side_window (gfship_domain * dom, const gfship_multilevel_params * p)
+{
+  const int L = dom->depth;
+#ifdef GFSHIP_LAB_NO_SIDE_JOB
+  return false;
+#endif
+  if (!dom->side_stream || !dom->sw.arm_ahead) return false;
+  if (dom->dim != 3 || p->dimension != 3 || dom->relax_mode != GFSHIP_RELAX_EXACT || dom->force_hyperplane)
+    return false;
+  for (int d = 0; d < 6; d++)
+    if (dom->side[d] == GFSHIP_SIDE_EXTERNAL) return false;
+  return L >= 1 && (int) p->minlevel <= L - 1 && skew_supported (dom, L - 1);
+}
+
+static int side_join_main (gfship_domain * dom)
+{
+  if (dom->side_join_wait) {
+    GFSHIP_HIP (hipStreamWaitEvent (dom->stream, dom->side_join, 0));
+    dom->side_join_wait = false;
+  }
+  return GFSHIP_OK;
+}
+
+static int side_issue (gfship_domain * dom, const gfship_multilevel_params * p)
+{
+  bool forked = false;
+  int r;
+  if ((r = skew_side_copies (dom, &forked))) return r;
+  if (dom->side_job.empty ())
+    return GFSHIP_OK;
+  if (dom->weighted || !side_window (dom, p))
+    return launch_side_job (dom, dom->stream);
+  if (!forked) {
+    GFSHIP_HIP (hipEventRecord (dom->side_fork, dom->stream));
+    GFSHIP_HIP (hipStreamWaitEvent (dom->side_stream, dom->side_fork, 0));
+  }
+  if ((r = launch_side_job (dom, dom->side_stream))) return r;
+  GFSHIP_HIP (hipEventRecord (dom->side_join, dom->side_stream));
+  dom->side_join_wait = true;
+  dom->n_coarse_init_side++;
+  return GFSHIP_OK;
+}
+
+int side_job_flush (gfship_domain * dom)
+{
+  if (!dom->side_job.empty ())
+    if (int r = launch_side_job (dom, dom->stream)) return r;
+  return side_join_main (dom);
 }
 
 }
@@ -368,6 +422,7 @@
       else
 	TRY (launch_restrict (dom, p->dimension, l, S->lev[l], S->lev[l + 1]));
     }
+    TRY (side_issue (dom, p));
     unsigned first = minlevel;
     if (ltop >= 0) {
       TRY (launch_lattice_cycle (dom, p->dimension, p->omega, (int) minlevel, ltop, nrl, DP, U, S));
@@ -390,6 +445,8 @@
       else if (prolongation_fusable (dom, p->dimension, (int) l, nrl[l]) ||
 	       line_prolongation_fusable (dom, p->dimension, (int) l, nrl[l]))
 	dom->kc[GFSHIP_KC_PROLONGATION_DECLINED]++;
+      if ((int) l == L)
+	TRY (side_join_main (dom));
       if (!fp)
 	TRY (launch_prolongate (dom, l - 1, DP->lev[l - 1], DP->lev[l]));
       TRY (relax_loop (dom, DP, U, p->dimension, l, p->omega, S, D, nrl[l],
@@ -408,8 +465,12 @@
     TRY (launch_residual (dom, L, U->lev[L], R->lev[L], D->lev[L], S->lev[L]));
 #undef TRY
  done:
-  for (int l = 0; l <= L; l++)
+  for (int l = 0; l <= L; l++) {
     dom->skew[l].rs_ready = false;
+    dom->skew[l].rs_side = false;
+    if (int rj = skew_rs_join (dom, l)) { if (r == GFSHIP_OK) r = rj; }
+  }
+  if (int rj = side_join_main (dom)) { if (r == GFSHIP_OK) r = rj; }
   return r;
 }
 
@@ -424,7 +485,23 @@
   return poisson_cycle (dom, p, u, rhs, dia, res, 1., nullptr);
 }
 
+static int poisson_solve (gfship_domain * dom, gfship_multilevel_params * par,
+			  gfship_field lhs, gfship_field rhs, gfship_field res,
+			  gfship_field dia, double dt);
+
 int gfship_poisson_solve (gfship_domain * dom, gfship_multilevel_params * par,
+			  gfship_field lhs, gfship_field rhs, gfship_field res,
+			  gfship_field dia, double dt)
+{
+  int r = poisson_solve (dom, par, lhs, rhs, res, dia, dt);
+  if (dom) {
+    int rf = side_job_flush (dom);
+    if (r == GFSHIP_OK) r = rf;
+  }
+  return r;
+}
+
+static int poisson_solve (gfship_domain * dom, gfship_multilevel_params * par,
 			  gfship_field lhs, gfship_field rhs, gfship_field res,
 			  gfship_field dia, double dt)
 {
diff --git a/gerris-fft-particles_amd/csrc/relax_patch_loop.hip b/gerris-fft-particles_amd/csrc/relax_patch_loop.hip
--- a/gerris-fft-particles_amd/csrc/relax_patch_loop.hip
+++ b/gerris-fft-particles_amd/csrc/relax_patch_loop.hip
@@ -1019,6 +1019,7 @@
   unsigned dimension;
 };
 
+template <bool PACK>
 __global__ void __launch_bounds__(256)
 patch_restrict_pack_kernel (PatchRestrictArgs A)
 {
@@ -1039,15 +1040,16 @@
     }
   }
   __syncthreads ();
-  for (int e = tid; e < PPR_ROWS*32; e += 256) {
-    const int row = e / 32, col = e % 32;
-    const int PA = col >> 2, p = col & 3;
-    const int a = 2*PA + (p & 1), db = p >> 1;
-    const int rho = r0 + row;
-    const int I = rho - PA - PB;
-    if (I >= 0 && I < n)
-      A.dst[tbase + (long) rho*SK_NL + 128*(p >> 1) + 2*(PA + 8*PB) + (p & 1)] = buf[a + 16*db][I - I0];
-  }
+  if (PACK)
+    for (int e = tid; e < PPR_ROWS*32; e += 256) {
+      const int row = e / 32, col = e % 32;
+      const int PA = col >> 2, p = col & 3;
+      const int a = 2*PA + (p & 1), db = p >> 1;
+      const int rho = r0 + row;
+      const int I = rho - PA - PB;
+      if (I >= 0 && I < n)
+	A.dst[tbase + (long) rho*SK_NL + 128*(p >> 1) + 2*(PA + 8*PB) + (p & 1)] = buf[a + 16*db][I - I0];
+    }
   for (int e = tid; e < 8*(PPR_ROWS/2); e += 256) {
     const int PA = e / (PPR_ROWS/2), mi = e % (PPR_ROWS/2);
     const int par = (PA + PB + r0) & 1;
@@ -1131,7 +1133,7 @@
 }
 
 int patch_pack (gfship_domain * dom, int level, SkewPlan * S, const double * u, const double * rhs,
-		const double * dia, const double * coarse)
+		const double * dia, const double * coarse, hipStream_t stream)
 {
   PatchPackArgs A;
   A.add = nullptr;
@@ -1151,7 +1153,7 @@
     PatchPackArgs Pr = A;
     Pr.narr = 1;
     dim3 pgrid ((rows + PR_ROWS*PR_WAVES - 1)/(PR_ROWS*PR_WAVES), S->ntj*S->ntj);
-    hipLaunchKernelGGL (patch_prolong_kernel, pgrid, dim3 (64*PR_WAVES), 0, dom->stream, Pr);
+    hipLaunchKernelGGL (patch_prolong_kernel, pgrid, dim3 (64*PR_WAVES), 0, stream, Pr);
     GFSHIP_HIP (hipGetLastError ());
     if (A.narr == 1)
       return GFSHIP_OK;
@@ -1160,13 +1162,29 @@
     A.coarse = nullptr;
   }
   dim3 grid ((rows + PP_ROWS - 1)/PP_ROWS, 8, S->ntj*S->ntj);
-  hipLaunchKernelGGL (patch_pack_kernel, grid, dim3 (256), 0, dom->stream, A);
+  hipLaunchKernelGGL (patch_pack_kernel, grid, dim3 (256), 0, stream, A);
   GFSHIP_HIP (hipGetLastError ());
   return GFSHIP_OK;
 }
 
+int patch_pack_rhs (gfship_domain * dom, int level, SkewPlan * S, const double * rhs, hipStream_t stream)
+{
+  PatchPackArgs A;
+  A.add = nullptr; A.coarse = nullptr; A.nat = nullptr;
+  A.periodic = all_sides_periodic (dom);
+  A.Lc = dom->lay[level > 0 ? level - 1 : 0];
+  A.L = dom->lay[level]; A.ntj = S->ntj; A.RT = S->RT;
+  A.narr = 1;
+  A.src[0] = rhs; A.dst[0] = S->rs;
+  const int rows = A.L.n + PK_SKEW + 1;
+  dim3 grid ((rows + PP_ROWS - 1)/PP_ROWS, 8, S->ntj*S->ntj);
+  hipLaunchKernelGGL (patch_pack_kernel, grid, dim3 (256), 0, stream, A);
+  GFSHIP_HIP (hipGetLastError ());
+  return GFSHIP_OK;
+}
+
 int patch_restrict_pack (gfship_domain * dom, int level, SkewPlan * S, const double * res,
-			 double * res_coarse, SkewPlan * Sc, unsigned dimension)
+			 double * res_coarse, SkewPlan * Sc, unsigned dimension, bool pack, hipStream_t stream)
 {
   PatchRestrictArgs A;
   A.L = dom->lay[level]; A.Lc = dom->lay[level - 1];
@@ -1178,7 +1196,9 @@
   A.dimension = dimension;
   const int rows = A.L.n + PK_SKEW + 1;
   dim3 grid ((rows + PPR_ROWS - 1)/PPR_ROWS, 8, S->ntj*S->ntj);
-  hipLaunchKernelGGL (patch_restrict_pack_kernel, grid, dim3 (256), 0, dom->stream, A);
+  with_bools ([&] (auto PACK) {
+    hipLaunchKernelGGL (patch_restrict_pack_kernel<decltype (PACK)::value>, grid, dim3 (256), 0, stream, A);
+  }, pack);
   GFSHIP_HIP (hipGetLastError ());
   return GFSHIP_OK;
 }
diff --git a/gerris-fft-particles_amd/csrc/relax_skew.hip b/gerris-fft-particles_amd/csrc/relax_skew.hip
--- a/gerris-fft-particles_amd/csrc/relax_skew.hip
+++ b/gerris-fft-particles_amd/csrc/relax_skew.hip
@@ -376,6 +376,7 @@
     if (S.hbf) (void) hipFree (S.hbf);
     if (S.arm_cum) (void) hipFree (S.arm_cum);
     if (S.arm_ev) (void) hipEventDestroy (S.arm_ev);
+    if (S.rs_ev) (void) hipEventDestroy (S.rs_ev);
     if (S.stats_loop) (void) hipFree (S.stats_loop);
     if (S.ctl) (void) hipFree (S.ctl);
     if (S.stats) (void) hipFree (S.stats);
@@ -389,7 +390,7 @@
 		      const double * rhs, const double * dia, const double * coarse = nullptr)
 {
   if (patch_level (dom, level))
-    return patch_pack (dom, level, S, u, rhs, dia, coarse);
+    return patch_pack (dom, level, S, u, rhs, dia, coarse, dom->stream);
   PackArgs A;
   A.add = nullptr; A.periodic = false;
   A.coarse = coarse; A.nat = const_cast<double *> (u);
@@ -557,11 +558,13 @@
   const bool fusedp = prolong_from != nullptr && bc && (patch_level (dom, level) || all_sides_periodic (dom));
   const double * rhs_pack = S->rs_ready && patch_level (dom, level) ? nullptr : rhs;
   S->rs_ready = false;
+  if (rhs_pack && (r = skew_rs_join (dom, level))) return r;
   if (prolong_from && !fusedp)
     if ((r = launch_prolongate (dom, level - 1, prolong_from, u))) return r;
   if (fusedp && (r = skew_pack (dom, level, S, u, rhs_pack, dia_zero ? nullptr : dia, prolong_from))) return r;
   if (bc &&!(fusedp && prolong_images (dom, level)) && (r = launch_bc (dom, ubc, dp, level, 1))) return r;
   if (!fusedp && (r = skew_pack (dom, level, S, u, rhs_pack, dia_zero ? nullptr : dia))) return r;
+  if ((r = skew_rs_join (dom, level))) return r;
   if (!dom->no_fused_loop && skew_loop_supported (dom, level, nrelax, bc)) {
     LoopGhosts G;
     const bool defer = all_sides_periodic (dom) && !op;
@@ -581,15 +584,65 @@
   SkewPlan * S, * Sc = nullptr;
   int r;
   if ((r = skew_plan (dom, level, &S))) return r;
+  const bool warm = S->hbf && S->loop_checked;
   if ((r = skew_loop_trial (dom, level, S, 4, true))) return r;
   if (coarse_fused) {
     if ((r = skew_plan (dom, level - 1, &Sc))) return r;
     if ((r = skew_loop_trial (dom, level - 1, Sc, 4, true))) return r;
   }
   res->zero[level - 1] = false;
-  if ((r = patch_restrict_pack (dom, level, S, res->lev[level], res->lev[level - 1], Sc, dimension))) return r;
+  bool side = dom->side_stream && dom->sw.arm_ahead && warm && !S->rs_wait && dom->side_job.empty ();
+  for (int d = 0; d < 6; d++)
+    if (dom->side[d] == GFSHIP_SIDE_EXTERNAL) side = false;
+#ifdef GFSHIP_LAB_NO_SIDE_COPY
+  side = false;
+#endif
+  if ((r = patch_restrict_pack (dom, level, S, res->lev[level], res->lev[level - 1], Sc, dimension, !side,
+				dom->stream)))
+    return r;
+  if (side) {
+    S->rs_side = true;
+    S->rs_src = res->lev[level];
+  }
   S->rs_ready = true;
   if (Sc) Sc->rs_ready = true;
+  return GFSHIP_OK;
+}
+
+int skew_side_copies (gfship_domain * dom, bool * forked)
+{
+  int r;
+  for (int level = 0; level <= dom->depth; level++) {
+    SkewPlan * S = &dom->skew[level];
+    if (!S->rs_side) continue;
+    S->rs_side = false;
+    if (!S->rs_ev)
+      GFSHIP_HIP (hipEventCreateWithFlags (&S->rs_ev, hipEventDisableTiming));
+    if (!*forked) {
+      GFSHIP_HIP (hipEventRecord (dom->side_fork, dom->stream));
+      GFSHIP_HIP (hipStreamWaitEvent (dom->side_stream, dom->side_fork, 0));
+      *forked = true;
+    }
+    if ((r = patch_pack_rhs (dom, level, S, S->rs_src, dom->side_stream))) return r;
+    GFSHIP_HIP (hipEventRecord (S->rs_ev, dom->side_stream));
+    S->rs_wait = true;
+    dom->n_rhs_copy_side++;
+  }
+  return GFSHIP_OK;
+}
+
+int skew_rs_join (gfship_domain * dom, int level)
+{
+  SkewPlan * S = &dom->skew[level];
+  if (S->rs_side) {
+    S->rs_side = false;
+    int r = patch_pack_rhs (dom, level, S, S->rs_src, dom->stream);
+    if (r) return r;
+  }
+  if (S->rs_wait) {
+    GFSHIP_HIP (hipStreamWaitEvent (dom->stream, S->rs_ev, 0));
+    S->rs_wait = false;
+  }
   return GFSHIP_OK;
 }
 
diff --git a/gerris-fft-particles_amd/csrc/simulation.hip b/gerris-fft-particles_amd/csrc/simulation.hip
--- a/gerris-fft-particles_amd/csrc/simulation.hip
+++ b/gerris-fft-particles_amd/csrc/simulation.hip
@@ -976,7 +976,7 @@
   return GFSHIP_OK;
 }
 
-static int coarse_init (gfship_sim * s, bool u_done);
+static int coarse_init (gfship_sim * s, bool u_done, bool job = false);
 
 int gfship_coarse_init (gfship_sim * s)
 {
@@ -984,7 +984,7 @@
   return coarse_init (s, false);
 }
 
-static int coarse_init (gfship_sim * s, bool u_done)
+static int coarse_init (gfship_sim * s, bool u_done, bool job)
 {
   std::vector<Field *> v;
   sim_variables (s, v);
@@ -1002,11 +1002,12 @@
     }
   }
   if (vel.empty ())
-    return launch_coarse_init (s->dom, now.data (), (int) now.size ());
-  TRY (launch_coarse_init_levels (s->dom, now.data (), (int) now.size (), s->dom->depth - 1, s->dom->depth - 1));
+    return launch_coarse_init_levels (s->dom, now.data (), (int) now.size (), s->dom->depth - 1, 0, nullptr, job);
+  TRY (launch_coarse_init_levels (s->dom, now.data (), (int) now.size (), s->dom->depth - 1, s->dom->depth - 1,
+				  nullptr, job));
   now.insert (now.end (), vel.begin (), vel.end ());
   if (s->dom->depth >= 2)
-    TRY (launch_coarse_init_levels (s->dom, now.data (), (int) now.size (), s->dom->depth - 2, 0));
+    TRY (launch_coarse_init_levels (s->dom, now.data (), (int) now.size (), s->dom->depth - 2, 0, nullptr, job));
   return GFSHIP_OK;
 }
 
@@ -1088,9 +1089,14 @@
   if (!corrected)
     TRY (correct_centered_velocities (s, s->i > 0 ? gc : s->gmac, - s->advection_params.dt, &u_coarse));
 
-  TRY (coarse_init (s, u_coarse));
-
-  TRY (mac_projection (s, &s->approx_projection_params, s->advection_params.dt, s->p, s->g, true, true));
+  TRY (coarse_init (s, u_coarse, !s->has_alpha && side_window (dom, &s->approx_projection_params)));
+
+  {
+    int r = mac_projection (s, &s->approx_projection_params, s->advection_params.dt, s->p, s->g, true, true);
+    const int rf = side_job_flush (dom);
+    if (r == GFSHIP_OK) r = rf;
+    if (r != GFSHIP_OK) return r;
+  }
   s->t = s->tnext;
   s->i++;
 
diff --git a/gerris-fft-particles_amd/csrc/timestep_kernels.hip b/gerris-fft-particles_amd/csrc/timestep_kernels.hip
--- a/gerris-fft-particles_amd/csrc/timestep_kernels.hip
+++ b/gerris-fft-particles_amd/csrc/timestep_kernels.hip
@@ -2685,7 +2685,6 @@
     out[0] = fmin (fmin (sh[0], sh[1]), fmin (sh[2], sh[3]));
 }
 
-struct CoarseArgs { double * vc[8]; const double * vf[8]; int nf; };
 
 template <int DIM>
 __global__ void __launch_bounds__(256)
@@ -3227,12 +3226,33 @@
   return launch_coarse_init_levels (dom, v, nf, top, 0);
 }
 
-int launch_coarse_init_levels (gfship_domain * dom, Field * const * v, int nf, int top, int bottom)
-{
+static void coarse_init_launch (gfship_domain * dom, int l, const CoarseArgs & A, hipStream_t stream)
+{
+  const Layout & Lc = dom->lay[l], & Lf = dom->lay[l + 1];
+  dim3 grid, block;
+  cell_grid (Lc, &grid, &block);
+  if (dom->dim == 3)
+    hipLaunchKernelGGL (coarse_init_kernel<3>, grid, block, 0, stream, Lc, Lf, A);
+  else
+    hipLaunchKernelGGL (coarse_init_kernel<2>, grid, block, 0, stream, Lc, Lf, A);
+}
+
+int launch_side_job (gfship_domain * dom, hipStream_t stream)
+{
+  for (const CoarseLaunch & J : dom->side_job)
+    coarse_init_launch (dom, J.level, J.A, stream);
+  dom->side_job.clear ();
+  GFSHIP_HIP (hipGetLastError ());
+  return GFSHIP_OK;
+}
+
+int launch_coarse_init_levels (gfship_domain * dom, Field * const * v, int nf, int top, int bottom,
+			       hipStream_t stream, bool job)
+{
+  if (!stream) stream = dom->stream;
   for (int f0 = 0; f0 < nf; f0 += 8) {
     int m = nf - f0 < 8 ? nf - f0 : 8;
     for (int l = top; l >= bottom; l--) {
-      const Layout & Lc = dom->lay[l], & Lf = dom->lay[l + 1];
       CoarseArgs A;
       A.nf = m;
       for (int f = 0; f < m; f++) {
@@ -3241,9 +3261,10 @@
 	v[f0 + f]->zero[l] = false;
 	v[f0 + f]->coarse_valid = true;
       }
-      dim3 grid, block;
-      cell_grid (Lc, &grid, &block);
-      DISPATCH (dom, coarse_init_kernel, grid, block, Lc, Lf, A);
+      if (job)
+	dom->side_job.push_back (CoarseLaunch { l, A });
+      else
+	coarse_init_launch (dom, l, A, stream);
     }
   }
   return GFSHIP_OK;
diff --git a/gerris-fft-particles_amd/gfship/__init__.py b/gerris-fft-particles_amd/gfship/__init__.py
--- a/gerris-fft-particles_amd/gfship/__init__.py
+++ b/gerris-fft-particles_amd/gfship/__init__.py
@@ -123,6 +123,7 @@
     "gfship_domain_set_gather": (_i, [_vp, _vp, _vp, _i, _i, C.POINTER(C.c_int)]),
     "gfship_domain_path_counts": (_i, [_vp, C.POINTER(C.c_ulonglong), C.POINTER(C.c_ulonglong)]),
     "gfship_domain_kernel_counts": (_i, [_vp, C.POINTER(C.c_ulonglong), _i]),
+    "gfship_domain_side_counts": (_i, [_vp, C.POINTER(C.c_ulonglong), C.POINTER(C.c_ulonglong)]),
     "gfship_sim_restart": (_i, [_vp, _d, _u]),
     "gfship_snapshot_tree_bytes": (C.c_size_t, [_vp, _i]),
     "gfship_snapshot_tree_write": (_i, [_vp, _i, _pi, _vp, C.c_size_t]),
@@ -340,6 +341,11 @@
         _check(lib().gfship_domain_path_counts(self.ptr, C.byref(a), C.byref(b)))
         return int(a.value), int(b.value)
 
+    def side_counts(self):
+        a, b = C.c_ulonglong(), C.c_ulonglong()
+        _check(lib().gfship_domain_side_counts(self.ptr, C.byref(a), C.byref(b)))
+        return int(a.value), int(b.value)
+
     def kernel_counts(self):
         n = len(KERNEL_COUNT_NAMES)
         a = (C.c_ulonglong * n)()
diff --git a/include/gfship.h b/include/gfship.h
--- a/include/gfship.h
+++ b/include/gfship.h
@@ -293,6 +293,8 @@
   GFSHIP_KC_COUNT
 };
 int  gfship_domain_kernel_counts (gfship_domain * dom, unsigned long long * counts, int n);
+int  gfship_domain_side_counts (gfship_domain * dom, unsigned long long * rhs_copies,
+				unsigned long long * coarse_init_jobs);
 #define GFSHIP_UNIQUE_ID_BYTES 128
 int  gfship_comm_available (void);
 int  gfship_comm_unique_id (void * id);
```
